# febrianrachmadi/dep-gan-im

Hardware: AMD Instinct MI355X
Metric: 2D slices/sec (G+2D+GP train step), 256x256x1 fp32 (higher is better)
Workload: dtype f32; 1 GPU; DEP-GAN-IM twoCritics canonical train step (critic-Y2 + critic-DEM + G update, WGAN-GP), batch 32 per GPU, 256x256x1; per_gpu_batch=32, global_batch=32, parallelism=dp1

## Files before the change

dep_gan_im_amd/csrc/common.h:

```cpp
#pragma once
#include <hip/hip_runtime.h>
#include <stdint.h>
#include <stddef.h>

typedef float f32x2 __attribute__((ext_vector_type(2)));
typedef float f32x4 __attribute__((ext_vector_type(4)));
typedef float f32x16 __attribute__((ext_vector_type(16)));

struct TView {
  float* p;
  long sB, sY, sX;
};

static inline TView make_view(float* p, int H, int W, int C) {
  TView v;
  v.p = p;
  v.sX = C;
  v.sY = (long)W * C;
  v.sB = (long)H * W * C;
  return v;
}
static inline TView make_view_slice(float* p, int H, int W, int Ctot, int c0) {
  TView v = make_view(p, H, W, Ctot);
  v.p = p + c0;
  return v;
}
static inline TView null_view() {
  TView v;
  v.p = nullptr;
  v.sB = v.sY = v.sX = 0;
  return v;
}

struct TViewH {
  __bf16* p;
  long sB, sY, sX;
};

static inline TViewH make_view_h(__bf16* p, int H, int W, int C) {
  TViewH v;
  v.p = p;
  v.sX = C;
  v.sY = (long)W * C;
  v.sB = (long)H * W * C;
  return v;
}
static inline TViewH make_view_slice_h(__bf16* p, int H, int W, int Ctot, int c0) {
  TViewH v = make_view_h(p, H, W, Ctot);
  v.p = p + c0;
  return v;
}
static inline TViewH null_view_h() {
  TViewH v;
  v.p = nullptr;
  v.sB = v.sY = v.sX = 0;
  return v;
}

struct Epilogue {
  const float* bias;
  const float* scale;
  const float* shift;
  const float* film_mul;
  const float* film_add;
  int film_ld;
  TView out_pre;
  TView res;
  TView mask;
  int relu;
  int accumulate;
  TView pool;
  const float* head_w;
  const float* head_b;
  float* head_out;
  int head_tanh, head_skip_out;
};

struct ConvArgs {
  TView in;
  TView out;
  const float* w;
  int B, H, W, Cin, Cout;
  Epilogue ep;
  long wsT, wsI, wsO;
  int flip;
  int vec4;
  unsigned long long* dbg;
  int groups;
  int lgx, lgy;
  const float* w_group[4];
  long out_group_off[4];
  int cpt;
  long in_run_off[4];
};

struct WgradArgs {
  TView x;
  TView dy;
  float* part;
  int B, H, W, Cin, Cout;
  int nTiles, tilesPerChunk;
  float* colpart;
  int colB;
};

#ifdef __HIPCC__
static __device__ __forceinline__ float dg_vmax(float a, float b) {
  float o;
  asm("v_max_f32 %0, %1, %2" : "=v"(o) : "v"(a), "v"(b));
  return o;
}
#endif

#define DG_OK 0
#define DG_ERR_ARG 1
#define DG_ERR_HIP 2
#define DG_ERR_UNSUPPORTED 3

void dg_set_error(const char* fmt, ...);

#define HIPCHECK(expr)                                                              \
  do {                                                                              \
    hipError_t _e = (expr);                                                         \
    if (_e != hipSuccess) {                                                         \
      dg_set_error("%s:%d: %s -> %s", __FILE__, __LINE__, #expr, hipGetErrorString(_e)); \
      return DG_ERR_HIP;                                                            \
    }                                                                               \
  } while (0)
// ... 51 lines not shown
  int planes;
  int ntaps() const { return family == CONV_WINO ? 16 : KS * KS; }
  int tapg() const { return KS == 5 ? 5 : KS * KS; }
};
static inline bool dg_plan_mfma(const ConvPlan& pl) { return pl.family != CONV_DIRECT; }
static inline bool dg_plan_bf16(const ConvPlan& pl) { return pl.family == CONV_BF16; }
static inline bool dg_plan_split(const ConvPlan& pl) { return pl.family == CONV_SPLIT; }
static inline bool dg_plan_wino(const ConvPlan& pl) { return pl.family == CONV_WINO; }
static inline bool dg_plan_tile3_ck8(const ConvPlan& pl) { return pl.family == CONV_TILE && pl.KS == 3 && pl.CK == 8; }
static inline bool dg_plan_tile5(const ConvPlan& pl) { return pl.family == CONV_TILE && pl.KS == 5; }
static inline ConvPlan dg_plan_direct() {
  ConvPlan p = {};
  p.family = CONV_DIRECT;
  return p;
}
ConvPlan dg_plan_conv(int KS, int Cin, int Cout);
ConvPlan dg_plan_conv_items(int KS, int Cin, int Cout, long items);
ConvPlan dg_plan_conv_bf16(int KS, int Cin, int Cout);
ConvPlan dg_plan_conv_bf16_n16(int KS, int Cin, int Cout);
const char* dg_conv_igemm_bf16_name(const ConvPlan& pl);
ConvPlan dg_plan_conv_split(int KS, int Cin, int Cout, int planes);
int dg_conv_igemm_bf16(const ConvPlan& pl, const ConvArgs& a, hipStream_t st);
static inline size_t dg_plan_elem_bytes(const ConvPlan& pl) { return pl.planes ? 2 * (size_t)pl.planes : 4; }

struct PackJob {
  const float* src;
  float* dst;
  const float* kscale;
  int ntaps, srcI, srcO, io, transpose, flip;
  int NT, CK, nCC, Kdim, Ndim;
  int bf16;
  int tapg;
  int wino;
  unsigned total;
  unsigned per_nt;
  unsigned nt_stride;
  unsigned blk0, nblk;
};
int dg_pack_job(const ConvPlan& pl, const float* src, int srcI, int srcO, int io, int transpose, int flip,
                const float* kscale, float* dst, size_t nt_stride, PackJob* job);
unsigned dg_pack_layout(PackJob* jobs_host, int njobs);
int dg_pack_weights_batch(const PackJob* jobs_dev, int njobs, unsigned nblocks, hipStream_t st);

int dg_pack_weights(const ConvPlan& pl, const float* src, int srcI, int srcO, int io, int transpose, int flip,
                    const float* kscale, float* dst, hipStream_t st);

int dg_conv_igemm(const ConvPlan& pl, const ConvArgs& a, hipStream_t st);
int dg_conv_igemm_check(const ConvPlan& pl, const ConvArgs& a);
bool dg_conv_igemm_wp_supported(const ConvPlan& pl, const ConvArgs& a, bool force);
int dg_conv_igemm_wp(const ConvPlan& pl, const ConvArgs& a, hipStream_t st);
bool dg_conv_igemm_ws5_supported(const ConvPlan& pl, const ConvArgs& a, bool force);
int dg_conv_igemm_ws5(const ConvPlan& pl, const ConvArgs& a, hipStream_t st);
const char* dg_conv_igemm_ws5_name(const ConvPlan& pl);
int dg_conv_igemm_tile(const ConvPlan& pl, const ConvArgs& a, hipStream_t st);
bool dg_conv_igemm_head_supported(const ConvPlan& pl, const ConvArgs& a);
ConvPlan dg_plan_conv_wino(int Cin, int Cout);
bool dg_conv_wino_supported(const ConvPlan& pl, const ConvArgs& a);
const char* dg_conv_wino_name(const ConvArgs& a);
int dg_conv_wino(const ConvPlan& pl, const ConvArgs& a, hipStream_t st);
enum { DG_EPF_BIAS = 1, DG_EPF_AFFINE = 2, DG_EPF_FILM = 4, DG_EPF_RELU = 8, DG_EPF_PRE = 16, DG_EPF_RES = 32,
       DG_EPF_MASK = 64, DG_EPF_POOL = 128, DG_EPF_ACCUM = 256, DG_EPF_HEAD = 512, DG_EPF_ALL = 1023 };
unsigned dg_epilogue_flags(const Epilogue& e);
int dg_wino_epi_class(unsigned flags, int form);
void dg_set_epi_classes(int on);
int dg_get_epi_classes();
void dg_conv_igemm_name(const ConvPlan& pl, const ConvArgs& a, char* buf, size_t cap);
int dg_conv_direct(int KS, const ConvArgs& a, hipStream_t st);

int dg_wgrad(int KS, const WgradArgs& a, int* nchunks, hipStream_t st);
int dg_wgrad_finish(const float* part, int nchunks, int ntaps, int Cin, int Cout, const float* scale, float* out,
                    float* raw, int accumulate, int oi, const float* colpart, int colC, const float* colscale,
                    float* colout, float* colraw, hipStream_t st);
int dg_wgrad_finish_rows(const float* part, int nchunks, int ntaps, int Cin, int Cout, const float* scale, float* out,
                         float* raw, int accumulate, int oi, const float* colpart, int colrows, int colC,
                         const float* colscale, float* colout, float* colraw, hipStream_t st);

bool dg_wgrad_bf16_supported(int KS, int Cin, int Cout);
int dg_wgrad_bf16(int KS, const WgradArgs& a, int* nchunks, hipStream_t st);

int dg_wgrad_small(int KS, const WgradArgs& a, int* nchunks, hipStream_t st);

int dg_wgrad_plan(int KS, int B, int H, int W, int Cin, int Cout, int out[4]);
int dg_wgrad_small_plan(int KS, int B, int H, int W, int Cin, int Cout, int out[4]);
int dg_wgrad_bf16_plan(int KS, int B, int H, int W, int Cin, int Cout, int out[4]);

enum DgWgradKernel { DG_WG_F32 = 0, DG_WG_EDGE = 1, DG_WG_BF16 = 2, DG_WG_BF16S = 3, DG_WG_DECONV = 4 };
struct DgWgradChoice {
  int kernel, nchunks;
  size_t part_floats;
  int col_rows;
};
int dg_wgrad_choose(int KS, int B, int H, int W, int Cin, int Cout, bool bf16_pipe, bool x_bf16, DgWgradChoice* out);
int dg_wgrad_plan_of(int kernel, int KS, int B, int H, int W, int Cin, int Cout, int out[4]);
```

dep_gan_im_amd/csrc/direct.hip:

```cpp
#include "common.h"
#include "epilogue.h"

template <int KS, int COG, int G>
__global__ __launch_bounds__(256) void conv_direct_kernel(const ConvArgs a) {
  constexpr int PAD = KS / 2;
  constexpr int TW = 16 + KS - 1;
  constexpr int PIXT = TW * TW;
  constexpr int NTAPS = KS * KS;
  constexpr int CT = COG * G;
  constexpr int CIK = 8;
  constexpr int PPP = 256 / G;
  constexpr int NPASS = G;

  extern __shared__ __attribute__((aligned(16))) float smem[];
  float* xs = smem;
  float* ws = smem + CIK * PIXT;

  const int tid = threadIdx.x;
  const int tilesX = (a.W + 15) >> 4, tilesY = (a.H + 15) >> 4;
  int t = blockIdx.x;
  const int tx0 = (t % tilesX) * 16;
  t /= tilesX;
  const int ty0 = (t % tilesY) * 16;
  const int b = t / tilesY;
// ... 221 lines not shown
    const int iy = ty0 + ly - PAD, ix = tx0 + lx - PAD;
    float v = 0.f;
    if (lx < TWX && iy >= 0 && iy < a.H && ix >= 0 && ix < a.W) v = inb[(long)iy * a.in.sY + (long)ix * a.in.sX + c];
    xs[q] = v;
  }
  for (int q = tid; q < a.Cin * KS * KS * CT; q += 256) {
    const int n = q % CT, tap = (q / CT) % (KS * KS), c = q / (CT * KS * KS);
    const int ts = a.flip ? (KS * KS - 1 - tap) : tap;
    ws[q] = (n < a.Cout) ? a.w[(long)ts * a.wsT + (long)c * a.wsI + (long)n * a.wsO] : 0.f;
  }
  __syncthreads();

  f32x4 acc[4];
#pragma unroll
  for (int j = 0; j < 4; ++j) acc[j] = f32x4{0.f, 0.f, 0.f, 0.f};
  for (int c = 0; c < a.Cin; ++c) {
#pragma unroll
    for (int ty = 0; ty < KS; ++ty) {
      const float* row = xs + (c * TWY + py + ty) * RS + qx;
      const f32x4 x0 = *reinterpret_cast<const f32x4*>(row);
      const f32x4 x1 = *reinterpret_cast<const f32x4*>(row + 4);
      const float xv[8] = {x0[0], x0[1], x0[2], x0[3], x1[0], x1[1], x1[2], x1[3]};
#pragma unroll
      for (int tx = 0; tx < KS; ++tx) {
        const f32x4 w4 = *reinterpret_cast<const f32x4*>(ws + ((c * KS + ty) * KS + tx) * CT + 4 * g);
#pragma unroll
        for (int j = 0; j < 4; ++j)
#pragma unroll
          for (int k = 0; k < 4; ++k) acc[j][k] = fmaf(xv[j + tx], w4[k], acc[j][k]);
      }
    }
  }
  const int co = 4 * g;
  if (co < a.Cout) {
#pragma unroll
    for (int j = 0; j < 4; ++j) {
      const int oy = ty0 + py, ox = tx0 + qx + j;
      if (oy < a.H && ox < a.W) epi_store4(a, b, oy, ox, co, acc[j]);
    }
  }
}

template <int KS, int G>
static int launch_cin12(const ConvArgs& a, hipStream_t st) {
  constexpr int ROWS = 256 / G / 4;
  dim3 grid((unsigned)(cdiv(a.W, 16) * cdiv(a.H, ROWS) * a.B));
  hipLaunchKernelGGL((conv_cin12_kernel<KS, G>), grid, dim3(256), 0, st, a);
  HIPCHECK(hipGetLastError());
  return DG_OK;
}

int dg_conv_direct(int KS, const ConvArgs& a_in, hipStream_t st) {
  ConvArgs a = a_in;
  if (a.ep.pool.p || a.ep.head_out || a.ep.head_skip_out || a.groups > 1 || a.cpt > 0) {
    dg_set_error("dg_conv_direct: no fused pool, fused head, grouped launch or gathered K on the direct kernels");
    return DG_ERR_UNSUPPORTED;
  }
  auto aligned = [](const TView& v) {
    return !v.p || (!(v.sX % 4) && !(v.sY % 4) && !(v.sB % 4) && !(((uintptr_t)v.p) & 15));
  };
  a.vec4 = (a.Cout % 4 == 0) && aligned(a.out) && aligned(a.ep.res) && aligned(a.ep.mask) && aligned(a.ep.out_pre) &&
           (!a.ep.film_mul || a.ep.film_ld % 4 == 0);
  const int sel = (a.Cout == 1) ? 0 : ((a.Cout <= 16) ? 1 : 2);
  if (a.Cin <= 2 && a.vec4 && (a.Cout == 16 || a.Cout == 32) && (KS == 3 || KS == 5)) {
    if (KS == 3) return (a.Cout == 16) ? launch_cin12<3, 4>(a, st) : launch_cin12<3, 8>(a, st);
    return (a.Cout == 16) ? launch_cin12<5, 4>(a, st) : launch_cin12<5, 8>(a, st);
  }
  if (KS == 3) {
    if (sel == 0) return (a.Cin >= 4) ? launch_cout1<3>(a, st) : launch_direct<3, 1, 1>(a, st);
    if (sel == 1) return launch_direct<3, 4, 4>(a, st);
    return launch_direct<3, 4, 8>(a, st);
  }
  if (KS == 5) {
    if (sel == 0) return (a.Cin >= 4) ? launch_cout1<5>(a, st) : launch_direct<5, 1, 1>(a, st);
    if (sel == 1) return launch_direct<5, 4, 4>(a, st);
    return launch_direct<5, 4, 8>(a, st);
  }
  if (KS == 1) {
    if (sel == 0) return launch_direct<1, 1, 1>(a, st);
    if (sel == 1) return launch_direct<1, 4, 4>(a, st);
    return launch_direct<1, 4, 8>(a, st);
  }
  dg_set_error("dg_conv_direct: unsupported kernel size %d", KS);
  return DG_ERR_UNSUPPORTED;
}

template <int KS>
__global__ __launch_bounds__(256) void wgrad_small_kernel(const WgradArgs a) {
  constexpr int PAD = KS / 2;
  constexpr int TW = 16 + KS - 1;
  constexpr int PIXT = TW * TW;
  constexpr int NTAPS = KS * KS;
  constexpr int NOUT = 4;
  extern __shared__ __attribute__((aligned(16))) float smem[];
  float* xs = smem;
  float* ds = smem + a.Cin * PIXT;
  const int tid = threadIdx.x;
  const int nout = NTAPS * a.Cin * a.Cout;
  const int tilesX = (a.W + 15) >> 4, tilesY = (a.H + 15) >> 4;
  const int t0 = blockIdx.x * a.tilesPerChunk, t1 = min(t0 + a.tilesPerChunk, a.nTiles);
  float acc[NOUT];
  int xoff[NOUT], co_[NOUT];
#pragma unroll
  for (int k = 0; k < NOUT; ++k) {
    acc[k] = 0.f;
    const int o = tid + k * 256;
    const int oo = (o < nout) ? o : 0;
    const int co = oo % a.Cout, ci = (oo / a.Cout) % a.Cin, tap = oo / (a.Cout * a.Cin);
// ... 197 lines not shown
```

dep_gan_im_amd/csrc/epilogue.h:

```cpp
#pragma once
#include "common.h"

struct EpiChan {
  float bias, scale, shift, fmul, fadd;
};

__device__ __forceinline__ EpiChan epi_load_chan(const Epilogue& e, int b, int co, int Cout) {
  EpiChan c;
  c.bias = e.bias ? e.bias[co] : 0.f;
  c.scale = e.scale ? e.scale[co] : 1.f;
  c.shift = e.shift ? e.shift[co] : 0.f;
  c.fmul = e.film_mul ? e.film_mul[(long)b * e.film_ld + co] : 1.f;
  c.fadd = e.film_add ? e.film_add[(long)b * e.film_ld + co] : 0.f;
  return c;
}

__device__ __forceinline__ long view_off(const TView& v, int b, int y, int x) {
  return (long)b * v.sB + (long)y * v.sY + (long)x * v.sX;
}

__device__ __forceinline__ float film_preact(float u, float fmul, float fadd) {
#pragma clang fp contract(off)
  const float p = u * fmul;
  return p + fadd;
}

__device__ __forceinline__ void epi_store(const ConvArgs& a, const EpiChan& c, int b, int oy, int ox, int co,
                                          float acc) {
  const Epilogue& e = a.ep;
  float v = acc + c.bias;
  if (e.scale) v = __fadd_rn(__fmul_rn(v, c.scale), c.shift);
  if (e.out_pre.p) e.out_pre.p[view_off(e.out_pre, b, oy, ox) + co] = v;
  if (e.film_mul) v = film_preact(v, c.fmul, c.fadd);
  if (e.relu) v = fmaxf(v, 0.f);
  if (e.res.p) v += e.res.p[view_off(e.res, b, oy, ox) + co];
  if (e.mask.p) v = (e.mask.p[view_off(e.mask, b, oy, ox) + co] > 0.f) ? v : 0.f;
  float* o = a.out.p + view_off(a.out, b, oy, ox) + co;
  if (e.accumulate) v += *o;
  *o = v;
}

__device__ __forceinline__ void epi_store4(const ConvArgs& a, int b, int oy, int ox, int co, f32x4 v) {
  const Epilogue& e = a.ep;
  if (e.bias) {
    const f32x4 t = *reinterpret_cast<const f32x4*>(e.bias + co);
#pragma unroll
    for (int k = 0; k < 4; ++k) v[k] += t[k];
  }
  if (e.scale) {
    const f32x4 sc = *reinterpret_cast<const f32x4*>(e.scale + co);
    const f32x4 sh = *reinterpret_cast<const f32x4*>(e.shift + co);
#pragma unroll
    for (int k = 0; k < 4; ++k) v[k] = __fadd_rn(__fmul_rn(v[k], sc[k]), sh[k]);
  }
  if (e.out_pre.p) *reinterpret_cast<f32x4*>(e.out_pre.p + view_off(e.out_pre, b, oy, ox) + co) = v;
  if (e.film_mul) {
    const f32x4 fm = *reinterpret_cast<const f32x4*>(e.film_mul + (long)b * e.film_ld + co);
    const f32x4 fa = *reinterpret_cast<const f32x4*>(e.film_add + (long)b * e.film_ld + co);
#pragma unroll
    for (int k = 0; k < 4; ++k) v[k] = film_preact(v[k], fm[k], fa[k]);
  }
  if (e.relu) {
#pragma unroll
    for (int k = 0; k < 4; ++k) v[k] = fmaxf(v[k], 0.f);
  }
  if (e.res.p) {
    const f32x4 r = *reinterpret_cast<const f32x4*>(e.res.p + view_off(e.res, b, oy, ox) + co);
#pragma unroll
    for (int k = 0; k < 4; ++k) v[k] += r[k];
  }
  if (e.mask.p) {
    const f32x4 m = *reinterpret_cast<const f32x4*>(e.mask.p + view_off(e.mask, b, oy, ox) + co);
// ... 12 lines not shown
```

dep_gan_im_amd/csrc/igemm_conv.hip:

```cpp
#include <stdlib.h>

#include "common.h"
#include "epilogue.h"

__device__ __forceinline__ void store_packed(float* dst, size_t i, float v, int bf16) {
  if (bf16) reinterpret_cast<__bf16*>(dst)[i] = (__bf16)v;
  else dst[i] = v;
}
__device__ __forceinline__ void store_split(float* dst, size_t nt_base, int cc, int tap, int n, int k, float v, int planes,
                                            int tapg, int ntaps, int NT, int CK) {
  const int ng = ntaps / tapg, tg = tap / tapg, tl = tap - tg * tapg;
  __bf16* d = reinterpret_cast<__bf16*>(dst) + nt_base + ((size_t)cc * ng + tg) * (size_t)(planes * tapg * NT * CK);
  float rem = v;
  for (int p = 0; p < planes; ++p) {
    const __bf16 hb = (__bf16)rem;
    d[((size_t)p * tapg + tl) * (NT * CK) + (size_t)n * CK + k] = hb;
    rem -= (float)hb;
  }
}

template <int MF>
struct Mfma;
template <>
struct Mfma<32> {
  typedef f32x16 acc_t;
  static constexpr int NREG = 16;
  static __device__ __forceinline__ acc_t run(float a, float b, acc_t c) {
    return __builtin_amdgcn_mfma_f32_32x32x2f32(a, b, c, 0, 0, 0);
  }
  static __device__ __forceinline__ int row(int j, int h) { return (j & 3) + 8 * (j >> 2) + 4 * h; }
};
template <>
struct Mfma<16> {
  typedef f32x4 acc_t;
  static constexpr int NREG = 4;
  static __device__ __forceinline__ acc_t run(float a, float b, acc_t c) {
    return __builtin_amdgcn_mfma_f32_16x16x4f32(a, b, c, 0, 0, 0);
  }
  static __device__ __forceinline__ int row(int j, int h) { return 4 * h + j; }
};

template <int MF, int KS, int CK, int TAPG, bool PERS, bool HEAD>
static __device__ __forceinline__ void igemm_conv_body(const ConvArgs& a) {
  constexpr int NT = MF;
  constexpr int PAD = KS / 2;
  constexpr int TW = 16 + KS - 1;
  constexpr int PIXT = TW * TW;
  constexpr int CKP = CK + 4;
  constexpr int NTAPS = KS * KS;
  constexpr int NG = NTAPS / TAPG;
  constexpr int KB = 256 / MF;
  constexpr int NSUB = CK / KB;
  constexpr int MT = 64 / MF;
  constexpr int XV = CK / 4;
  constexpr int XTOT = PIXT * XV;
  constexpr int XPIECES = (XTOT + 255) / 256;
  constexpr int WTOT = TAPG * NT * XV;
  constexpr int WPIECES = (WTOT + 255) / 256;
  static_assert(NTAPS % TAPG == 0 && (TAPG == NTAPS || TAPG == KS), "tap grouping");
  static_assert(CK % KB == 0, "chunk must hold whole fragment reads");
  typedef typename Mfma<MF>::acc_t acc_t;

  extern __shared__ __attribute__((aligned(16))) float smem[];
  float* xs = smem;
  float* ws = smem + PIXT * CKP;

  const int tid = threadIdx.x;
  unsigned long long* dbg = a.dbg ? a.dbg + (size_t)blockIdx.x * 16 : nullptr;
  if (dbg && tid == 0) {
    dbg[0] = __builtin_amdgcn_s_memtime();
    dbg[6] = __builtin_amdgcn_s_memrealtime();
    dbg[7] = __builtin_amdgcn_s_getreg((4 << 0) | (0 << 6) | (31 << 11));
  }
  const int tilesX = (a.W + 15) >> 4, tilesY = (a.H + 15) >> 4;
  const unsigned nNTall = (unsigned)a.lgy, nPix = (unsigned)a.lgx;
  constexpr int XFULL = XTOT / 256, WFULL = WTOT / 256;
  constexpr bool XPART = (XTOT % 256) != 0, WPART = (WTOT % 256) != 0;
  unsigned xgb[XPIECES], xlb[XPIECES], wlb[WPIECES];
  int xyx[XPIECES];
  if (PERS) {
#pragma unroll
    for (int i = 0; i < XPIECES; ++i) {
      const int q = min(tid + i * 256, XTOT - 1);
      const int pix = q / XV, part = q - pix * XV;
      const int ly = pix / TW, lx = pix - ly * TW;
      xgb[i] = 4u * (unsigned)(ly * (int)a.in.sY + lx * (int)a.in.sX + part * 4);
      xlb[i] = 4u * (unsigned)(pix * CKP + part * 4);
      xyx[i] = (ly << 16) | (lx << 8) | (part * 4);
    }
#pragma unroll
    for (int i = 0; i < WPIECES; ++i) {
      const int q = min(tid + i * 256, WTOT - 1);
      const int row = q / XV, part = q - row * XV;
      wlb[i] = 4u * (unsigned)(row * CKP + part * 4);
    }
// ... 150 lines not shown
    if (MF == 32) {
      py = 4 * wv + 2 * mt + (r >> 4);
      px = r & 15;
    } else {
      py = 4 * wv + mt;
      px = r;
    }
    apix[mt] = (py * TW + px) * CKP + 4 * h;
  }
  const int boff = r * CKP + 4 * h;

  acc_t acc[MT];
#pragma unroll
  for (int mt = 0; mt < MT; ++mt)
#pragma unroll
    for (int j = 0; j < Mfma<MF>::NREG; ++j) acc[mt][j] = 0.f;

  prefetch(0);
  if (dbg && tid == 0) dbg[1] = __builtin_amdgcn_s_memtime();
  for (int s = 0; s < NS; ++s) {
    __syncthreads();
    commit(s);
    __syncthreads();
    if (dbg && tid == 0 && s == 0) dbg[2] = __builtin_amdgcn_s_memtime();
    if (dbg && tid == 0 && s == 1) dbg[3] = __builtin_amdgcn_s_memtime();
    if (s + 1 < NS) prefetch(s + 1);
    const int tg = s % NG;
    constexpr int NSTEP = TAPG * NSUB;
    f32x4 av[2][MT], bv[2];
    auto load_frag = [&](int q, f32x4* a_, f32x4& b_) {
      const int tl = q / NSUB, sub = q - tl * NSUB;
      const int tap = (TAPG == NTAPS) ? tl : (tg * TAPG + tl);
      const int ty = tap / KS, tx = tap - ty * KS;
      const int tapoff = (ty * TW + tx) * CKP;
#pragma unroll
      for (int mt = 0; mt < MT; ++mt) a_[mt] = *reinterpret_cast<const f32x4*>(xs + apix[mt] + tapoff + sub * KB);
      b_ = *reinterpret_cast<const f32x4*>(ws + tl * (NT * CKP) + boff + sub * KB);
    };
    load_frag(0, av[0], bv[0]);
#pragma unroll
    for (int q = 0; q < NSTEP; ++q) {
      if (q + 1 < NSTEP) load_frag(q + 1, av[(q + 1) & 1], bv[(q + 1) & 1]);
      __builtin_amdgcn_sched_barrier(0);
#pragma unroll
      for (int j = 0; j < 4; ++j)
#pragma unroll
        for (int mt = 0; mt < MT; ++mt) acc[mt] = Mfma<MF>::run(bv[q & 1][j], av[q & 1][mt][j], acc[mt]);
      __builtin_amdgcn_sched_barrier(0);
    }
  }

  if (dbg && tid == 0) dbg[4] = __builtin_amdgcn_s_memtime();
#define EPI_HEAD HEAD
#include "igemm_epilogue.inc"
#undef EPI_HEAD
  if (dbg && tid == 0) {
    dbg[5] = __builtin_amdgcn_s_memtime();
    dbg[6] = __builtin_amdgcn_s_memrealtime() - dbg[6];
  }
  dbg = nullptr;
  } while (PERS && (id += gridDim.x) < nPix * nNTall);
}

template <int MF, int KS, int CK, int TAPG, bool PERS>
__global__ __launch_bounds__(256, (PERS && KS == 3) ? (CK == 8 ? 4 : 3) : 1) void igemm_conv_kernel(const ConvArgs a) {
  igemm_conv_body<MF, KS, CK, TAPG, PERS, false>(a);
}

template <bool PERS>
__global__ __launch_bounds__(256, PERS ? 4 : 1) void igemm_conv_head_kernel(const ConvArgs a) {
  igemm_conv_body<32, 3, 8, 9, PERS, true>(a);
}

ConvPlan dg_plan_conv(int KS, int Cin, int Cout) {
  ConvPlan p = dg_plan_direct();
  p.KS = KS;
  p.Cin = Cin;
  p.Cout = Cout;
  p.MF = (Cout % 32 == 0) ? 32 : 16;
  p.NT = p.MF;
  p.CK = 16;
  if (Cin < 8 || (Cin % 4) != 0 || Cout < 8) return p;
  if (KS != 1 && KS != 3 && KS != 5) return p;
  if (p.MF == 32 && KS == 5) p.CK = 8;
  if (p.MF == 32 && KS == 1) p.CK = 32;
  p.family = CONV_TILE;
  p.nNT = cdiv(Cout, p.NT);
  p.nCC = cdiv(Cin, p.CK);
  p.packedFloats = (size_t)p.nNT * p.nCC * KS * KS * p.NT * p.CK;
  return p;
}

ConvPlan dg_plan_conv_items(int KS, int Cin, int Cout, long items) {
  ConvPlan p = dg_plan_conv(KS, Cin, Cout);
  const char* e = getenv("DEPGAN_IGEMM_CK8");
  const bool on = !(e && atoi(e) == 0);
  if (on && p.family == CONV_TILE && KS == 3 && p.MF == 32 && (Cin % 8) == 0 && items >= 1536) {
    p.CK = 8;
    p.nCC = cdiv(Cin, p.CK);
    p.packedFloats = (size_t)p.nNT * p.nCC * KS * KS * p.NT * p.CK;
  }
  return p;
}

ConvPlan dg_plan_conv_wino(int Cin, int Cout) {
  ConvPlan p = dg_plan_conv(3, Cin, Cout);
  if (p.family != CONV_TILE || (Cin % 8) != 0 || (Cout % 32) != 0) { p.family = CONV_DIRECT; return p; }
  p.family = CONV_WINO;
  p.CK = 8;
  p.nCC = Cin / 8;
  p.packedFloats = (size_t)p.nNT * p.nCC * 16 * p.NT * p.CK;
  return p;
}

static long igemm_grid(int KS, int CK, size_t lds, long total) {
  const char* e = getenv("DEPGAN_IGEMM_PERSIST");
  int per_cu = (int)((160 * 1024) / lds);
  if (per_cu > (KS == 3 ? (CK == 8 ? 4 : 3) : 2)) per_cu = (KS == 3 ? (CK == 8 ? 4 : 3) : 2);
  if (KS == 1) per_cu = 0;
  if (e) per_cu = atoi(e) < per_cu ? atoi(e) : per_cu;
  const long cap = 256L * per_cu;
  return (per_cu > 0 && total > cap) ? cap : total;
}

template <int MF, int KS, int CK, int TAPG>
static int launch_tile(const ConvArgs& a, hipStream_t st, char* name_out = nullptr, size_t name_cap = 0) {
  constexpr int TW = 16 + KS - 1;
  constexpr size_t lds_k = (size_t)(TW * TW * (CK + 4) + TAPG * MF * (CK + 4)) * sizeof(float);
  constexpr size_t lds_e = (size_t)4 * 64 * (MF + 4) * sizeof(float);
  constexpr size_t lds = lds_k > lds_e ? lds_k : lds_e;
  ConvArgs b = a;
  b.lgx = cdiv(a.W, 16) * cdiv(a.H, 16) * a.B;
  b.lgy = cdiv(a.Cout, MF) * (a.groups > 1 ? a.groups : 1);
  const long total = (long)b.lgx * b.lgy;
  const long G = igemm_grid(KS, CK, lds, total);
  constexpr bool CAN_HEAD = (MF == 32 && KS == 3 && CK == 8 && TAPG == 9);
  const bool head = a.ep.head_out != nullptr;
  if (head && (!CAN_HEAD || a.Cout != 32 || a.groups > 1 || a.ep.pool.p != nullptr)) {
    dg_set_error("dg_conv_igemm: the fused head needs the 8-channel-chunk 3x3 kernel and 32 output channels");
    return DG_ERR_ARG;
  }
  if (name_out) {
    if (head) snprintf(name_out, name_cap, "igemm_conv_head_kernel<%s>", G < total ? "true" : "false");
    else snprintf(name_out, name_cap, "igemm_conv_kernel<%d,%d,%d,%d,%s>", MF, KS, CK, TAPG, G < total ? "true" : "false");
    return DG_OK;
  }
  if constexpr (CAN_HEAD) {
    if (head) {
      static DgOncePerDevice once_h;
      if (once_h.need()) {
        HIPCHECK(hipFuncSetAttribute(reinterpret_cast<const void*>(&igemm_conv_head_kernel<false>),
                                     hipFuncAttributeMaxDynamicSharedMemorySize, (int)lds));
        HIPCHECK(hipFuncSetAttribute(reinterpret_cast<const void*>(&igemm_conv_head_kernel<true>),
                                     hipFuncAttributeMaxDynamicSharedMemorySize, (int)lds));
      }
      if (G < total) hipLaunchKernelGGL((igemm_conv_head_kernel<true>), dim3((unsigned)G), dim3(256), lds, st, b);
      else hipLaunchKernelGGL((igemm_conv_head_kernel<false>), dim3((unsigned)G), dim3(256), lds, st, b);
      HIPCHECK(hipGetLastError());
      return DG_OK;
    }
  }
  static DgOncePerDevice once;
  if (once.need()) {
    HIPCHECK(hipFuncSetAttribute(reinterpret_cast<const void*>(&igemm_conv_kernel<MF, KS, CK, TAPG, false>),
                                 hipFuncAttributeMaxDynamicSharedMemorySize, (int)lds));
    HIPCHECK(hipFuncSetAttribute(reinterpret_cast<const void*>(&igemm_conv_kernel<MF, KS, CK, TAPG, true>),
                                 hipFuncAttributeMaxDynamicSharedMemorySize, (int)lds));
  }
  if (G < total)
    hipLaunchKernelGGL((igemm_conv_kernel<MF, KS, CK, TAPG, true>), dim3((unsigned)G), dim3(256), lds, st, b);
  else
    hipLaunchKernelGGL((igemm_conv_kernel<MF, KS, CK, TAPG, false>), dim3((unsigned)G), dim3(256), lds, st, b);
  HIPCHECK(hipGetLastError());
  return DG_OK;
}

static int dispatch_tile(const ConvPlan& pl, const ConvArgs& a, hipStream_t st, char* name_out, size_t name_cap) {
  const bool wide = pl.MF == 32;
  if (pl.family == CONV_TILE && pl.KS == 3 && !dg_plan_tile3_ck8(pl))
    return wide ? launch_tile<32, 3, 16, 9>(a, st, name_out, name_cap) : launch_tile<16, 3, 16, 9>(a, st, name_out, name_cap);
  if (pl.family == CONV_TILE && pl.KS == 5)
    return wide ? launch_tile<32, 5, 8, 25>(a, st, name_out, name_cap) : launch_tile<16, 5, 16, 25>(a, st, name_out, name_cap);
  if (pl.family == CONV_TILE && pl.KS == 1)
    return wide ? launch_tile<32, 1, 32, 1>(a, st, name_out, name_cap) : launch_tile<16, 1, 16, 1>(a, st, name_out, name_cap);
  if (dg_plan_tile3_ck8(pl)) return launch_tile<32, 3, 8, 9>(a, st, name_out, name_cap);
  dg_set_error("dg_conv_igemm: no tile kernel for family %d MF=%d KS=%d CK=%d", (int)pl.family, pl.MF, pl.KS, pl.CK);
  return DG_ERR_ARG;
}

bool dg_conv_igemm_head_supported(const ConvPlan& pl, const ConvArgs& a) {
  return (dg_plan_tile3_ck8(pl) || dg_plan_wino(pl)) && a.Cout == 32 && a.groups <= 1 && a.ep.pool.p == nullptr && a.cpt <= 0 &&
         !a.ep.accumulate;
}

void dg_conv_igemm_name(const ConvPlan& pl, const ConvArgs& a, char* buf, size_t cap) {
  if (cap) buf[0] = 0;
  if (!dg_plan_mfma(pl)) { snprintf(buf, cap, "conv_direct"); return; }
  if (dg_plan_split(pl)) { snprintf(buf, cap, "igemm_split_kernel"); return; }
  if (dg_plan_bf16(pl)) { snprintf(buf, cap, "%s", dg_conv_igemm_bf16_name(pl)); return; }
  if (dg_plan_wino(pl)) { snprintf(buf, cap, "%s", dg_conv_wino_name(a)); return; }
  if (dg_conv_igemm_wp_supported(pl, a, false)) { snprintf(buf, cap, "igemm_wp_kernel<0>"); return; }
  if (dg_conv_igemm_ws5_supported(pl, a, false)) { snprintf(buf, cap, "%s", dg_conv_igemm_ws5_name(pl)); return; }
  dispatch_tile(pl, a, nullptr, buf, cap);
}

int dg_conv_igemm_check(const ConvPlan& pl, const ConvArgs& a) {
  if (!dg_plan_mfma(pl)) {
    dg_set_error("dg_conv_igemm: no MFMA variant for KS=%d Cin=%d Cout=%d", pl.KS, pl.Cin, pl.Cout);
    return DG_ERR_UNSUPPORTED;
  }
  auto misaligned = [](const TView& v) {
    return v.p && ((v.sX % 4) || (v.sY % 4) || (v.sB % 4) || (((uintptr_t)v.p) & 15));
  };
  if (misaligned(a.in) || misaligned(a.out) || misaligned(a.ep.res) || misaligned(a.ep.mask) ||
      misaligned(a.ep.out_pre) || (a.Cout % 4) || (a.ep.film_mul && (a.ep.film_ld % 4))) {
    dg_set_error("dg_conv_igemm: views must be 16-byte aligned (pointers, strides and Cout multiples of 4 floats)");
    return DG_ERR_ARG;
  }
  if (a.ep.pool.p && ((a.H | a.W) & 1 || misaligned(a.ep.pool) || a.groups > 1)) {
    dg_set_error("dg_conv_igemm: fused max-pool needs even H, W and a 16-byte aligned pooled view");
    return DG_ERR_ARG;
  }
  if (a.cpt > 0) {
    const int run = a.cpt * pl.CK;
    bool bad = a.groups > 1 || (a.Cin % run) != 0 || a.Cin / run > 4;
    for (int r = 0; !bad && r < a.Cin / run; ++r) bad = (a.in_run_off[r] % 4) != 0;
    if (bad) {
      dg_set_error("dg_conv_igemm: gathered K needs Cin = runs (<= 4) x cpt x %d channels and 16-byte run offsets", pl.CK);
      return DG_ERR_ARG;
    }
  }
  if (a.ep.head_out && !dg_conv_igemm_head_supported(pl, a)) {
    dg_set_error("dg_conv_igemm: the fused head needs the fp32 8-channel-chunk 3x3 kernel, 32 output channels, no pool");
    return DG_ERR_ARG;
  }
  return DG_OK;
}

static int conv_igemm_impl(const ConvPlan& pl, const ConvArgs& a_in, hipStream_t st, bool allow_wp) {
  ConvArgs a = a_in;
  DGCHECK(dg_conv_igemm_check(pl, a));
  if (dg_plan_bf16(pl) || dg_plan_split(pl)) return dg_conv_igemm_bf16(pl, a, st);
  if (dg_plan_wino(pl)) return dg_conv_wino(pl, a, st);
  if (allow_wp && dg_conv_igemm_wp_supported(pl, a, false)) return dg_conv_igemm_wp(pl, a, st);
  if (allow_wp && dg_conv_igemm_ws5_supported(pl, a, false)) return dg_conv_igemm_ws5(pl, a, st);
  return dispatch_tile(pl, a, st, nullptr, 0);
}

int dg_conv_igemm(const ConvPlan& pl, const ConvArgs& a, hipStream_t st) { return conv_igemm_impl(pl, a, st, true); }
int dg_conv_igemm_tile(const ConvPlan& pl, const ConvArgs& a, hipStream_t st) { return conv_igemm_impl(pl, a, st, false); }

__global__ __launch_bounds__(256) void pack_weights_batch_kernel(const PackJob* __restrict__ jobs, int njobs) {
  int lo = 0, hi = njobs - 1;
  while (lo < hi) {
    const int mid = (lo + hi + 1) >> 1;
    if (jobs[mid].blk0 <= blockIdx.x) lo = mid; else hi = mid - 1;
  }
  const PackJob J = jobs[lo];
  const unsigned b = blockIdx.x - J.blk0;
  if (J.wino) {
    const unsigned cols = J.total / 16u, plane = (unsigned)(J.NT * J.CK);
    for (unsigned i = b * 256u + threadIdx.x; i < cols; i += J.nblk * 256u) {
      unsigned q = i;
      const int k = (int)(q % J.CK);
      q /= J.CK;
      const int n = (int)(q % J.NT);
      q /= J.NT;
      const int cc = (int)(q % J.nCC);
      const int nt = (int)(q / J.nCC);
      const int kk = cc * J.CK + k, nn = nt * J.NT + n;
      double g[3][3];
#pragma unroll
      for (int t = 0; t < 9; ++t) g[t / 3][t % 3] = 0.0;
      if (kk < J.Kdim && nn < J.Ndim) {
        const int ci = J.transpose ? nn : kk;
        const int co = J.transpose ? kk : nn;
        const float* e0 = J.src + (J.io ? ((size_t)co * J.srcI + ci) : ((size_t)ci * J.srcO + co));
        const size_t ts_stride = (size_t)J.srcI * J.srcO;
        const float ks = J.kscale ? J.kscale[kk] : 1.f;
#pragma unroll
        for (int t = 0; t < 9; ++t) {
          float v = e0[(size_t)(J.flip ? 8 - t : t) * ts_stride];
// ... 110 lines not shown
```

dep_gan_im_amd/csrc/igemm_epilogue.inc:

```
#ifndef EPI_PRE_SYNC
#define EPI_PRE_SYNC __syncthreads()
#define EPI_PRE_SYNC_DEFAULTED
#endif
  EPI_PRE_SYNC;
  constexpr int CP = NT + 4;
#ifdef EPI_ES_BASE
  float* es = EPI_ES_BASE;
#else
  float* es = smem + wv * (64 * CP);
#endif
  constexpr int NQ = (MF == 32) ? 4 : 1, CSTEP = (MF == 32) ? 8 : 4;
#if defined(EPI_STAGE)
  EPI_STAGE;
  (void)es;
#elif !defined(EPI_PHASED)
#pragma unroll
  for (int mt = 0; mt < MT; ++mt)
#pragma unroll
    for (int g = 0; g < NQ; ++g) {
      f32x4 q4;
#pragma unroll
      for (int k = 0; k < 4; ++k) q4[k] = acc[mt][4 * g + k];
      *reinterpret_cast<f32x4*>(es + (MF * mt + r) * CP + CSTEP * g + 4 * h) = q4;
    }
#endif
  constexpr int LPP = NT / 4;
  constexpr int PPP = 64 / LPP;
#ifdef EPI_NPASS
  constexpr int NPASS = EPI_NPASS;
#else
  constexpr int NPASS = 64 / PPP;
#endif
  const int c4 = (lane % LPP) * 4, pl0 = lane / LPP;
  const int co = n0 + c4;
#ifndef EPI_OYW
  const int wvu = __builtin_amdgcn_readfirstlane(wv);
#endif
  const Epilogue& e = a.ep;
#ifdef EPI_CLASS
  typedef EPI_CLASS EpiC;
  constexpr bool EPI_CT = EpiC::fixed;
  const bool affine = EPI_CT ? EpiC::affine : (e.scale != nullptr), film = EPI_CT ? EpiC::film : (e.film_mul != nullptr),
             relu = EPI_CT ? EpiC::relu : (e.relu != 0), accum = EPI_CT ? false : (e.accumulate != 0);
  const bool has_bias = EPI_CT ? EpiC::bias : (e.bias != nullptr), has_pre = EPI_CT ? EpiC::pre : (e.out_pre.p != nullptr),
             has_res = EPI_CT ? EpiC::res : (e.res.p != nullptr), has_msk = EPI_CT ? EpiC::msk : (e.mask.p != nullptr),
             has_pool = EPI_CT ? EpiC::pool : (e.pool.p != nullptr);
#else
  const bool affine = e.scale != nullptr, film = e.film_mul != nullptr, relu = e.relu != 0, accum = e.accumulate != 0;
  const bool has_bias = e.bias != nullptr, has_pre = e.out_pre.p != nullptr, has_res = e.res.p != nullptr,
             has_msk = e.mask.p != nullptr, has_pool = e.pool.p != nullptr;
#endif
#ifdef EPI_OYW
  const int oyw = EPI_OYW;
#else
  const int oyw = ty0 + 4 * wvu;
#endif
#ifdef EPI_HEAD
  float hkeep_out = 0.f;
#endif
#ifdef EPI_FULL
  const bool full = EPI_FULL;
#else
  const bool full = (ty0 + 16 <= a.H) && (tx0 + 16 <= a.W);
#endif
  if (co < a.Cout) {
    f32x4 bias4 = {0.f, 0.f, 0.f, 0.f}, sc4 = {1.f, 1.f, 1.f, 1.f}, sh4 = {0.f, 0.f, 0.f, 0.f};
    f32x4 fm4 = {1.f, 1.f, 1.f, 1.f}, fa4 = {0.f, 0.f, 0.f, 0.f};
    if (has_bias) bias4 = *reinterpret_cast<const f32x4*>(e.bias + co);
    if (affine) {
      sc4 = *reinterpret_cast<const f32x4*>(e.scale + co);
      sh4 = *reinterpret_cast<const f32x4*>(e.shift + co);
    }
#pragma unroll
    for (int k = 0; k < 4; ++k) sh4[k] = fmaf(bias4[k], sc4[k], sh4[k]);
    if (film) {
      fm4 = *reinterpret_cast<const f32x4*>(e.film_mul + (long)b * e.film_ld + co);
      fa4 = *reinterpret_cast<const f32x4*>(e.film_add + (long)b * e.film_ld + co);
    }
    auto mk = [&](const float* p) {
      const unsigned long long u = (unsigned long long)p;
      const unsigned lo = __builtin_amdgcn_readfirstlane((unsigned)u), hi = __builtin_amdgcn_readfirstlane((unsigned)(u >> 32));
      return __builtin_amdgcn_make_buffer_rsrc((void*)(((unsigned long long)hi << 32) | lo), 0, 0x7FFFFFFF, 0x00020000);
    };
    const int lo_out = 4 * (pl0 * (int)a.out.sX + co);
    const int lo_pre = has_pre ? 4 * (pl0 * (int)e.out_pre.sX + co) : 0;
    const int lo_res = has_res ? 4 * (pl0 * (int)e.res.sX + co) : 0;
    const int lo_msk = has_msk ? 4 * (pl0 * (int)e.mask.sX + co) : 0;
    const __amdgpu_buffer_rsrc_t r_out = mk(a.out.p + out_goff + view_off(a.out, b, oyw, tx0));
    const __amdgpu_buffer_rsrc_t r_pre = mk(has_pre ? e.out_pre.p + view_off(e.out_pre, b, oyw, tx0) : a.out.p);
    const __amdgpu_buffer_rsrc_t r_res = mk(has_res ? e.res.p + view_off(e.res, b, oyw, tx0) : a.out.p);
    const __amdgpu_buffer_rsrc_t r_msk = mk(has_msk ? e.mask.p + view_off(e.mask, b, oyw, tx0) : a.out.p);
    const __amdgpu_buffer_rsrc_t r_pool =
        mk(has_pool ? e.pool.p + view_off(e.pool, b, oyw >> 1, tx0 >> 1) : a.out.p);
    const int lo_pool = has_pool ? 4 * ((pl0 >> 1) * (int)e.pool.sX + co) : 0;
    const int sY_pool = 4 * (int)e.pool.sY, sX_pool = 4 * (int)e.pool.sX;
    f32x4 vrow = {0.f, 0.f, 0.f, 0.f};
#ifdef EPI_HEAD
#ifdef EPI_CLASS
    const bool has_head = EPI_HEAD && (EPI_CT ? EpiC::head : (e.head_out != nullptr));
#else
    const bool has_head = EPI_HEAD && e.head_out != nullptr;
#endif
    f32x4 hw4 = {0.f, 0.f, 0.f, 0.f};
    if (has_head) hw4 = *reinterpret_cast<const f32x4*>(e.head_w + co);
    const bool skip_out = has_head && e.head_skip_out != 0;
#else
    constexpr bool has_head = false, skip_out = false;
#endif
    typedef int i32x4 __attribute__((ext_vector_type(4)));
    auto ld = [&](const __amdgpu_buffer_rsrc_t& r, int voff, int soff) {
      const i32x4 t = __builtin_amdgcn_raw_buffer_load_b128(r, voff, soff, 0);
      return __builtin_bit_cast(f32x4, t);
    };
    auto st = [&](const __amdgpu_buffer_rsrc_t& r, int voff, int soff, f32x4 v) {
      __builtin_amdgcn_raw_buffer_store_b128(__builtin_bit_cast(i32x4, v), r, voff, soff, 0);
    };
    const int sY_out = 4 * (int)a.out.sY, sX_out = 4 * (int)a.out.sX;
    const int sY_pre = 4 * (int)e.out_pre.sY, sX_pre = 4 * (int)e.out_pre.sX;
    const int sY_res = 4 * (int)e.res.sY, sX_res = 4 * (int)e.res.sX;
    const int sY_msk = 4 * (int)e.mask.sY, sX_msk = 4 * (int)e.mask.sX;
#ifdef EPI_STAGE_LATE
    EPI_STAGE_LATE;
#endif
#pragma unroll
    for (int p = 0; p < NPASS; ++p) {
      constexpr int RP = 16 / PPP;
      const int py = (p & 1) + 2 * (p / (2 * RP)), px0 = ((p >> 1) % RP) * PPP;
      const bool ok = full || (oyw + py < a.H && tx0 + px0 + pl0 < a.W);
#if defined(EPI_FETCH)
      f32x4 v;
      EPI_FETCH(v, py, (px0 + pl0));
#elif defined(EPI_PHASED)
      static_assert(MF == 32, "phased epilogue: 32-pixel tiles");
      if (p % (NPASS / MT) == 0) {
        const int mtp = p / (NPASS / MT);
#pragma unroll
        for (int g = 0; g < NQ; ++g) {
          f32x4 q4;
#pragma unroll
          for (int k = 0; k < 4; ++k) q4[k] = acc[mtp][4 * g + k];
          *reinterpret_cast<f32x4*>(es + r * CP + CSTEP * g + 4 * h) = q4;
        }
      }
      f32x4 v = *reinterpret_cast<const f32x4*>(es + ((py & 1) * 16 + px0 + pl0) * CP + c4);
#else
      f32x4 v = *reinterpret_cast<const f32x4*>(es + (py * 16 + px0 + pl0) * CP + c4);
#endif
#pragma unroll
      for (int k = 0; k < 4; ++k) v[k] = fmaf(v[k], sc4[k], sh4[k]);
      if (has_pre) {
        if (ok) st(r_pre, lo_pre, py * sY_pre + px0 * sX_pre, v);
      }
      if (film) {
#pragma unroll
        for (int k = 0; k < 4; ++k) v[k] = film_preact(v[k], fm4[k], fa4[k]);
      }
      if (relu) {
#pragma unroll
        for (int k = 0; k < 4; ++k) v[k] = dg_vmax(v[k], 0.f);
      }
      if (has_res) {
        f32x4 rr = {0.f, 0.f, 0.f, 0.f};
        if (ok) rr = ld(r_res, lo_res, py * sY_res + px0 * sX_res);
#pragma unroll
        for (int k = 0; k < 4; ++k) v[k] += rr[k];
      }
      if (has_msk) {
        f32x4 mm = {1.f, 1.f, 1.f, 1.f};
        if (ok) mm = ld(r_msk, lo_msk, py * sY_msk + px0 * sX_msk);
#pragma unroll
        for (int k = 0; k < 4; ++k) v[k] = (mm[k] > 0.f) ? v[k] : 0.f;
      }
      const int so = py * sY_out + px0 * sX_out;
      if (accum) {
        f32x4 old = {0.f, 0.f, 0.f, 0.f};
        if (ok) old = ld(r_out, lo_out, so);
#pragma unroll
        for (int k = 0; k < 4; ++k) v[k] += old[k];
      }
      if (ok && !skip_out) st(r_out, lo_out, so, v);
#ifdef EPI_HEAD
      if (has_head) {
        static_assert(!EPI_HEAD || (NT == 32 && NPASS == 8), "fused head: 32-channel tiles, eight passes");
        float d = v[0] * hw4[0];
        d = fmaf(v[1], hw4[1], d);
        d = fmaf(v[2], hw4[2], d);
        d = fmaf(v[3], hw4[3], d);
#define EPI_DPP(x, ctrl) \
  __builtin_bit_cast(float, __builtin_amdgcn_update_dpp(0, __builtin_bit_cast(int, (x)), (ctrl), 0xF, 0xF, false))
        d += EPI_DPP(d, 0xB1);
        d += EPI_DPP(d, 0x4E);
        d += EPI_DPP(d, 0x141);
#undef EPI_DPP
        hkeep_out = ((lane & 7) == p) ? d : hkeep_out;
      }
#endif
      if (has_pool) {
        if ((py & 1) == 0) {
          vrow = v;
        } else {
          f32x4 m;
#pragma unroll
          for (int k = 0; k < 4; ++k) {
            const float t = dg_vmax(vrow[k], v[k]);
            m[k] = dg_vmax(t, __shfl_xor(t, LPP, 64));
          }
          if (ok && (pl0 & 1) == 0) st(r_pool, lo_pool, (py >> 1) * sY_pool + (px0 >> 1) * sX_pool, m);
        }
      }
    }
  }
#ifdef EPI_HEAD
  if (EPI_HEAD && a.ep.head_out != nullptr && n0 < a.Cout) {
    const int ph = lane & 7, plh = lane >> 3;
    const int pyh = (ph & 1) + 2 * (ph >> 2), pxh = ((ph >> 1) & 1) * 8 + plh;
    const int yh = oyw + pyh, xh = tx0 + pxh;
    if (yh < a.H && xh < a.W) {
      const float t = hkeep_out + a.ep.head_b[0];
      a.ep.head_out[((long)b * a.H + yh) * a.W + xh] = a.ep.head_tanh ? tanhf(t) : t;
    }
  }
#endif
#ifdef EPI_PRE_SYNC_DEFAULTED
#undef EPI_PRE_SYNC
#undef EPI_PRE_SYNC_DEFAULTED
#endif
```

dep_gan_im_amd/csrc/igemm_wino.hip:

```cpp
#include <stdlib.h>

#include <type_traits>

#include "common.h"
#include "epilogue.h"

namespace {

constexpr int WN_CK = 8;
constexpr int WN_TW = 18;
constexpr int WN_CP = 36;
constexpr int WN_XV = WN_CK / 4;

template <int MT>
struct WnCfg {
  static constexpr int TH = 8 * MT;
  static constexpr int NTILE = 32 * MT;
  static constexpr int PIXT = (TH + 2) * WN_TW;
  static constexpr int XTOT = PIXT * WN_XV;
  static constexpr int NXP = (XTOT + 255) / 256;
  static constexpr int RAW = NXP * 256 * 4;
  static_assert(XTOT % 4 == 0 && WN_TW % 2 == 0, "rslot permutes inside aligned groups of four slots: halo and padding stay apart");
  static constexpr int ZPLANE = NTILE * WN_CP + 32;
  static constexpr int Z = 8 * ZPLANE;
  static constexpr int NBUF = 2;
  static_assert(NBUF >= 2 && NBUF * RAW <= Z, "the raw ring must fit under the Z exchange: LDS and workgroups per CU unchanged");
  static_assert((NBUF - 1) * NXP + 4 < 64, "counted waits: vmcnt is a 6-bit field");
  static constexpr size_t LDS = sizeof(float) * (size_t)Z;
  static constexpr int WGS_PER_CU = (MT == 2) ? 2 : 3;
};

template <int N>
static __device__ __forceinline__ void wn_wait_vm() {
  asm volatile("s_waitcnt vmcnt(%0)" ::"n"(N) : "memory");
}
template <int S>
using WnSlot = std::integral_constant<int, S>;

static __device__ __forceinline__ int rslot(int pix, int half) { return (2 * pix + half) ^ (((pix % WN_TW) >> 2) & 3); }
static __device__ __forceinline__ int rslot_inv(int q) { return q ^ ((((q >> 1) % WN_TW) >> 2) & 3); }

constexpr unsigned WN_BAR = DG_EPF_BIAS | DG_EPF_AFFINE | DG_EPF_RELU;
constexpr unsigned WN_FILM = WN_BAR | DG_EPF_FILM | DG_EPF_RES;
constexpr int WN_NCLASS = 11, WN_HEAD_CLASS = 10;
constexpr unsigned kWnClassMask[WN_NCLASS] = {
    0,
    WN_BAR,
    WN_BAR | DG_EPF_POOL,
    WN_FILM,
    WN_FILM | DG_EPF_PRE,
    DG_EPF_RES | DG_EPF_MASK,
    DG_EPF_MASK,
    0,
    DG_EPF_BIAS | DG_EPF_RELU,
    DG_EPF_BIAS | DG_EPF_RELU | DG_EPF_POOL,
    WN_BAR | DG_EPF_HEAD,
};
#define WN_CLASSES8(X) X(1) X(2) X(3) X(4) X(5) X(6) X(7) X(8) X(9)
template <int EC>
struct WnEpi {
  static_assert(EC >= 0 && EC < WN_NCLASS, "epilogue class");
  static constexpr unsigned M = kWnClassMask[EC];
  static constexpr bool fixed = EC != 0;
  static constexpr bool bias = M & DG_EPF_BIAS, affine = M & DG_EPF_AFFINE, film = M & DG_EPF_FILM, relu = M & DG_EPF_RELU,
                        pre = M & DG_EPF_PRE, res = M & DG_EPF_RES, msk = M & DG_EPF_MASK, pool = M & DG_EPF_POOL,
                        head = M & DG_EPF_HEAD;
};

template <int MT, bool PERS, bool HEAD, bool GATH = false, int ABL = 0, int EC = 0>
static __device__ __forceinline__ void wino_body(const ConvArgs& a) {
  typedef WnCfg<MT> C;
  constexpr int MF = 32, NT = 32;
  constexpr int WN_RAW = C::RAW, WN_ZPLANE = C::ZPLANE, WN_XTOT = C::XTOT, NXP = C::NXP, NBUF = C::NBUF;
  constexpr int NXI = (ABL & 8) ? 0 : NXP;
  typedef f32x16 acc_t;
  extern __shared__ __attribute__((aligned(16))) float smem[];

  const int tid = threadIdx.x;
  const int lane = tid & 63, wv = tid >> 6;
  const int r = lane & 31, h = lane >> 5;
  const int tilesX = (a.W + 15) >> 4, tilesY = (a.H + C::TH - 1) / C::TH;
  const unsigned nNTall = (unsigned)a.lgy, nPix = (unsigned)a.lgx;
  const int nCC = a.Cin / WN_CK;

  constexpr int SENT = (int)0x80000000;
  int xvo[NXP], xyx[NXP];
#pragma unroll
  for (int i = 0; i < NXP; ++i) {
    const int q = tid + i * 256;
    const int lq = rslot_inv(q);
    const int pix = lq >> 1, part = lq & 1;
    const int ly = pix / WN_TW, lx = pix - ly * WN_TW;
    xvo[i] = (q < WN_XTOT) ? 4 * (ly * (int)a.in.sY + lx * (int)a.in.sX + part * 4) : SENT;
    xyx[i] = (ly << 8) | lx;
  }
  int tA[MT][4], tB[MT][4];
  float tS[MT];
#pragma unroll
  for (int i = 0; i < MT; ++i) {
    const int cg = h, aa = wv, T = 32 * i + r;
    const int tyi = T >> 3, txi = T & 7;
    const int rA = (aa == 0) ? 0 : (aa == 2 ? 2 : 1), rB = (aa == 3) ? 3 : (aa == 2 ? 1 : 2);
#pragma unroll
    for (int j = 0; j < 4; ++j) {
      tA[i][j] = 16 * rslot((2 * tyi + rA) * WN_TW + 2 * txi + j, cg);
      tB[i][j] = 16 * rslot((2 * tyi + rB) * WN_TW + 2 * txi + j, cg);
    }
    tS[i] = (aa == 1) ? 1.f : -1.f;
  }
  const int wbase = __builtin_amdgcn_readfirstlane(wv * 256);
  const int wvo = 4 * ((4 * wv * 32 + r) * WN_CK + 4 * h);

  unsigned id = blockIdx.x;
  do {
    int t, ntile;
    if ((nPix & 7u) == 0) {
      const unsigned x = id & 7u, sl = id >> 3;
      ntile = (int)(sl % nNTall);
      t = (int)(x * (nPix >> 3) + sl / nNTall);
// ... 166 lines not shown
        chunk(no, rt, last);
      }
    }

    if (ABL & 1) {
      float sacc = 0.f;
#pragma unroll
      for (int f = 0; f < 4; ++f)
#pragma unroll
        for (int mt = 0; mt < MT; ++mt)
#pragma unroll
          for (int j = 0; j < 16; ++j) sacc += acc[f][mt][j];
      if (sacc == 12345.678f) a.out.p[tid] = sacc;
      __syncthreads();
      continue;
    }
    auto zstage = [&]() {
      __syncthreads();
      float* zw = smem + (2 * wv) * WN_ZPLANE + r * WN_CP + 4 * h;
#pragma unroll
      for (int mt = 0; mt < MT; ++mt)
#pragma unroll
        for (int g = 0; g < 4; ++g) {
          f32x4 z0, z1;
#pragma unroll
          for (int k = 0; k < 4; ++k) {
            const float m0 = acc[0][mt][4 * g + k], m1 = acc[1][mt][4 * g + k], m2 = acc[2][mt][4 * g + k],
                        m3 = acc[3][mt][4 * g + k];
            z0[k] = (m0 + m1) + m2;
            z1[k] = (m1 - m2) - m3;
          }
          *reinterpret_cast<f32x4*>(zw + mt * (32 * WN_CP) + 8 * g) = z0;
          *reinterpret_cast<f32x4*>(zw + WN_ZPLANE + mt * (32 * WN_CP) + 8 * g) = z1;
        }
      __syncthreads();
    };
#define EPI_PRE_SYNC
#define EPI_STAGE
#define EPI_STAGE_LATE zstage()
#define EPI_NPASS (4 * MT)
#define EPI_OYW (ty0 + 2 * MT * __builtin_amdgcn_readfirstlane(wv))
#define EPI_FULL ((ty0 + C::TH <= a.H) && (tx0 + 16 <= a.W))
#define EPI_FETCH(v, py, px)                                                                                         \
  {                                                                                                                  \
    const float* zb = smem + ((px)&1) * WN_ZPLANE +                                                                  \
                      ((MT * __builtin_amdgcn_readfirstlane(wv) + ((py) >> 1)) * 8 + ((px) >> 1)) * WN_CP + c4;       \
    const f32x4 za = *reinterpret_cast<const f32x4*>(zb + (((py)&1) ? 2 : 0) * WN_ZPLANE);                           \
    const f32x4 zb1 = *reinterpret_cast<const f32x4*>(zb + (((py)&1) ? 4 : 2) * WN_ZPLANE);                          \
    const f32x4 zc = *reinterpret_cast<const f32x4*>(zb + (((py)&1) ? 6 : 4) * WN_ZPLANE);                           \
    _Pragma("unroll") for (int k_ = 0; k_ < 4; ++k_) v[k_] = ((py)&1) ? (za[k_] - zb1[k_]) - zc[k_] : (za[k_] + zb1[k_]) + zc[k_]; \
  }
#define EPI_HEAD HEAD
#define EPI_CLASS WnEpi<EC>
#include "igemm_epilogue.inc"
#undef EPI_CLASS
#undef EPI_HEAD
#undef EPI_FETCH
#undef EPI_FULL
#undef EPI_OYW
#undef EPI_NPASS
#undef EPI_STAGE_LATE
#undef EPI_STAGE
#undef EPI_PRE_SYNC
    if (PERS) __syncthreads();
  } while (PERS && (id += gridDim.x) < nPix * nNTall);
}

template <int MT, bool PERS, int EC>
__global__ __launch_bounds__(256, WnCfg<MT>::WGS_PER_CU) void wino_conv_kernel(const ConvArgs a) {
  wino_body<MT, PERS, false, false, 0, EC>(a);
}
template <bool PERS, int EC>
__global__ __launch_bounds__(256, 2) void wino_conv_head_kernel(const ConvArgs a) {
  wino_body<2, PERS, true, false, 0, EC>(a);
}
template <int MT, bool PERS>
__global__ __launch_bounds__(256, WnCfg<MT>::WGS_PER_CU) void wino_conv_gathered_kernel(const ConvArgs a) {
  wino_body<MT, PERS, false, true>(a);
}
#ifdef DEPGAN_WINO_ABLATIONS
template <int MT, int ABL>
__global__ __launch_bounds__(256, WnCfg<MT>::WGS_PER_CU) void wino_conv_abl_kernel(const ConvArgs a) {
  wino_body<MT, true, false, false, ABL>(a);
}
#endif

struct WnKern {
  const void* fn;
  const char* name;
};
#define WN_K8(EC)                                                                                       \
  {{reinterpret_cast<const void*>(&wino_conv_kernel<1, false, EC>), "wino_conv_kernel<1,false," #EC ">"}, \
   {reinterpret_cast<const void*>(&wino_conv_kernel<1, true, EC>), "wino_conv_kernel<1,true," #EC ">"}},
const WnKern kWn8[WN_HEAD_CLASS][2] = {WN_K8(0) WN_CLASSES8(WN_K8)};
#undef WN_K8
const WnKern kWn16[2] = {{reinterpret_cast<const void*>(&wino_conv_kernel<2, false, 0>), "wino_conv_kernel<2,false,0>"},
                         {reinterpret_cast<const void*>(&wino_conv_kernel<2, true, 0>), "wino_conv_kernel<2,true,0>"}};
const WnKern kWnHead[2][2] = {
    {{reinterpret_cast<const void*>(&wino_conv_head_kernel<false, 0>), "wino_conv_head_kernel<false,0>"},
     {reinterpret_cast<const void*>(&wino_conv_head_kernel<true, 0>), "wino_conv_head_kernel<true,0>"}},
    {{reinterpret_cast<const void*>(&wino_conv_head_kernel<false, WN_HEAD_CLASS>), "wino_conv_head_kernel<false,10>"},
     {reinterpret_cast<const void*>(&wino_conv_head_kernel<true, WN_HEAD_CLASS>), "wino_conv_head_kernel<true,10>"}}};
static_assert(WN_HEAD_CLASS == 10, "the names above");
const WnKern kWnGath[2][2] = {
    {{reinterpret_cast<const void*>(&wino_conv_gathered_kernel<1, false>), "wino_conv_gathered_kernel<1,false>"},
     {reinterpret_cast<const void*>(&wino_conv_gathered_kernel<1, true>), "wino_conv_gathered_kernel<1,true>"}},
    {{reinterpret_cast<const void*>(&wino_conv_gathered_kernel<2, false>), "wino_conv_gathered_kernel<2,false>"},
     {reinterpret_cast<const void*>(&wino_conv_gathered_kernel<2, true>), "wino_conv_gathered_kernel<2,true>"}}};

int g_epi_classes = -1;

}

void dg_set_epi_classes(int on) { g_epi_classes = on ? 1 : 0; }
int dg_get_epi_classes() {
  if (g_epi_classes < 0) {
    const char* e = getenv("DEPGAN_EPI_CLASSES");
    g_epi_classes = (e && atoi(e) == 0) ? 0 : 1;
  }
  return g_epi_classes;
}

unsigned dg_epilogue_flags(const Epilogue& e) {
  return (e.bias ? DG_EPF_BIAS : 0u) | (e.scale ? DG_EPF_AFFINE : 0u) | (e.film_mul ? DG_EPF_FILM : 0u) |
         (e.relu ? DG_EPF_RELU : 0u) | (e.out_pre.p ? DG_EPF_PRE : 0u) | (e.res.p ? DG_EPF_RES : 0u) |
         (e.mask.p ? DG_EPF_MASK : 0u) | (e.pool.p ? DG_EPF_POOL : 0u) | (e.accumulate ? DG_EPF_ACCUM : 0u) |
         (e.head_out ? DG_EPF_HEAD : 0u);
}

int dg_wino_epi_class(unsigned flags, int form) {
  if (!dg_get_epi_classes()) return 0;
  if (form == 1) return flags == kWnClassMask[WN_HEAD_CLASS] ? WN_HEAD_CLASS : 0;
  if (form != 0) return 0;
  for (int i = 1; i < WN_HEAD_CLASS; ++i)
    if (kWnClassMask[i] == flags) return i;
  return 0;
}

bool dg_conv_wino_supported(const ConvPlan& pl, const ConvArgs& a) {
  if (!dg_plan_wino(pl)) return false;
  if (a.Cin != pl.Cin || (a.Cin % WN_CK) || (a.Cout % 32) || a.groups > 1 || a.dbg || ((a.H | a.W) & 1)) return false;
  if (a.cpt > 0 && ((a.Cin % (a.cpt * WN_CK)) != 0 || a.Cin / (a.cpt * WN_CK) > 4)) return false;
  long run = 0;
  for (int t = 0; a.cpt > 0 && t < a.Cin / (a.cpt * WN_CK); ++t) {
    if (a.in_run_off[t] < 0) return false;
    run = a.in_run_off[t] > run ? a.in_run_off[t] : run;
  }
  constexpr long lim = 1L << 29;
  if (a.in.sY < 0 || a.in.sX < 0 || a.in.sY >= lim || a.in.sX >= lim || run >= lim) return false;
  if ((WnCfg<2>::TH + 2) * a.in.sY + WN_TW * a.in.sX + a.Cin + run >= lim) return false;
  return true;
}

static int wino_mt(const ConvArgs& a) {
  static int forced = -1;
  if (forced < 0) {
    const char* e = getenv("DEPGAN_WINO_MT");
    forced = e ? atoi(e) : 0;
  }
  if (a.ep.head_out) return 2;
  if (forced == 1 || forced == 2) return forced;
  return 1;
}

template <int MT>
static void wino_geometry(ConvArgs& a, long* total, long* G, bool* pers) {
  a.lgx = cdiv(a.W, 16) * cdiv(a.H, WnCfg<MT>::TH) * a.B;
  a.lgy = a.Cout / 32;
  *total = (long)a.lgx * a.lgy;
  const long cap = (long)WnCfg<MT>::WGS_PER_CU * dg_cu_count();
  *pers = *total > cap;
  *G = *pers ? cap : *total;
}

static const WnKern* wino_pick(const ConvArgs& a, int mt, bool pers) {
  const int form = a.ep.head_out ? 1 : (a.cpt > 0 ? 3 : (mt == 2 ? 2 : 0));
  const int ec = dg_wino_epi_class(dg_epilogue_flags(a.ep), form);
  if (form == 1) return &kWnHead[ec ? 1 : 0][pers];
  if (form == 3) return &kWnGath[mt - 1][pers];
  if (form == 2) return &kWn16[pers];
  return &kWn8[ec][pers];
}

const char* dg_conv_wino_name(const ConvArgs& a_in) {
  ConvArgs a = a_in;
  long total, G;
  bool pers;
  const int mt = wino_mt(a);
  if (mt == 2) wino_geometry<2>(a, &total, &G, &pers); else wino_geometry<1>(a, &total, &G, &pers);
  return wino_pick(a, mt, pers)->name;
}

template <int MT>
static int wino_launch(ConvArgs a, hipStream_t st) {
  long total, G;
  bool pers;
  wino_geometry<MT>(a, &total, &G, &pers);
  constexpr size_t LDS = WnCfg<MT>::LDS;
  static DgOncePerDevice once;
  if (once.need()) {
    const WnKern* const own = (MT == 2) ? &kWn16[0] : &kWn8[0][0];
    const int nown = (MT == 2) ? 2 : 2 * WN_HEAD_CLASS;
    for (int i = 0; i < nown; ++i)
      HIPCHECK(hipFuncSetAttribute(own[i].fn, hipFuncAttributeMaxDynamicSharedMemorySize, (int)LDS));
    for (int i = 0; i < 2; ++i)
      HIPCHECK(hipFuncSetAttribute(kWnGath[MT - 1][i].fn, hipFuncAttributeMaxDynamicSharedMemorySize, (int)LDS));
    for (int i = 0; MT == 2 && i < 4; ++i)
      HIPCHECK(hipFuncSetAttribute(kWnHead[i >> 1][i & 1].fn, hipFuncAttributeMaxDynamicSharedMemorySize, (int)LDS));
  }
#ifdef DEPGAN_WINO_ABLATIONS
  if (const char* e = getenv("DEPGAN_WINO_ABL")) {
    const int abl = atoi(e);
    if (abl && pers && !a.ep.head_out && a.cpt <= 0) {
#define WN_ABL_CASE(N)                                                                                              \
  case N:                                                                                                           \
    HIPCHECK(hipFuncSetAttribute(reinterpret_cast<const void*>(&wino_conv_abl_kernel<MT, N>),                       \
                                 hipFuncAttributeMaxDynamicSharedMemorySize, (int)LDS));                            \
    hipLaunchKernelGGL((wino_conv_abl_kernel<MT, N>), dim3((unsigned)G), dim3(256), LDS, st, a);                    \
    break;
      switch (abl) {
        WN_ABL_CASE(1) WN_ABL_CASE(2) WN_ABL_CASE(3) WN_ABL_CASE(4) WN_ABL_CASE(8) WN_ABL_CASE(10) WN_ABL_CASE(11)
        default: dg_set_error("DEPGAN_WINO_ABL=%d not instantiated", abl); return DG_ERR_ARG;
      }
      HIPCHECK(hipGetLastError());
      return DG_OK;
    }
  }
#endif
  if (a.ep.head_out) {
    if (MT != 2 || a.Cout != 32 || a.ep.pool.p || a.cpt > 0) {
      dg_set_error("dg_conv_wino: the fused head needs 32 output channels, no fused pool and no gathered K");
      return DG_ERR_ARG;
    }
  }
  void* kargs[] = {&a};
  HIPCHECK(hipLaunchKernel(wino_pick(a, MT, pers)->fn, dim3((unsigned)G), dim3(256), kargs, LDS, st));
  HIPCHECK(hipGetLastError());
  return DG_OK;
}

int dg_conv_wino(const ConvPlan& pl, const ConvArgs& a, hipStream_t st) {
  if (!dg_conv_wino_supported(pl, a)) {
    dg_set_error("dg_conv_wino: shape not covered (3x3, Cin %% 8, Cout %% 32, even H and W, no groups, a halo tile of the input view within 2 GiB)");
    return DG_ERR_UNSUPPORTED;
  }
  return wino_mt(a) == 2 ? wino_launch<2>(a, st) : wino_launch<1>(a, st);
}
```

dep_gan_im_amd/csrc/igemm_wp.hip:

```cpp
#include <stdlib.h>

#include "common.h"
#include "epilogue.h"

namespace {

constexpr int WP_NW = 16;

template <int MF, int KS, int CK>
struct WpGeo {
  static constexpr int NT = MF, MT = 64 / MF, PAD = KS / 2, NTAPS = KS * KS;
  static constexpr int TWX = 16 + KS - 1, TWY = 4 + KS - 1;
  static constexpr int PIX = TWX * TWY;
  static constexpr int XV = CK / 4;
  static constexpr int CKP = (KS == 3) ? CK + 4 : CK;
  static constexpr int EPI_FLOATS = (MF == 32 ? 32 : 64) * (NT + 4);
  static constexpr int WAVE_FLOATS = PIX * CKP > EPI_FLOATS ? PIX * CKP : EPI_FLOATS;
  static constexpr int SLOTS = PIX * XV;
  static constexpr int PIECES = (SLOTS + 63) / 64;
  static __device__ __forceinline__ int panel_sw(int n) {
    if (MF == 32) return (n >> (KS == 3 ? 2 : 4)) & 1;
    return (0x78 >> (2 * (n >> 2))) & 3;
  }
  static __device__ __forceinline__ int halo_off(int pix, int part) {
    if (CK == 16) return pix * CKP + 4 * (part ^ (((pix >> 2) & 1) << 1));
    return pix * CKP + 4 * part;
  }
};

template <int MF> struct WpMfma;
template <> struct WpMfma<32> {
  typedef f32x16 acc_t;
  static constexpr int NREG = 16;
  static __device__ __forceinline__ acc_t run(float w, float x, acc_t c) { return __builtin_amdgcn_mfma_f32_32x32x2f32(w, x, c, 0, 0, 0); }
};
template <> struct WpMfma<16> {
  typedef f32x4 acc_t;
  static constexpr int NREG = 4;
  static __device__ __forceinline__ acc_t run(float w, float x, acc_t c) { return __builtin_amdgcn_mfma_f32_16x16x4f32(w, x, c, 0, 0, 0); }
};

template <int MF, int KS, int CK, int ABL>
static __device__ __forceinline__ void igemm_wp_body(const ConvArgs& a) {
  typedef WpGeo<MF, KS, CK> G;
  constexpr int NT = G::NT, MT = G::MT, TW = G::TWX, PAD = G::PAD, NTAPS = G::NTAPS, CKP = G::CKP;
  constexpr int PIECES = G::PIECES, SLOTS = G::SLOTS, XV = G::XV;
  typedef typename WpMfma<MF>::acc_t acc_t;
  extern __shared__ __attribute__((aligned(16))) float smem[];
  const int tid = threadIdx.x;
  const int lane = tid & 63, wv = tid >> 6;
  const int NW = (int)(blockDim.x >> 6);
  const int r = lane % MF, h = lane / MF;
  const int nCC = a.Cin / CK;
  const int panelFloats = nCC * NTAPS * NT * CK;
  float* panel = smem;
  float* wbuf = smem + panelFloats + wv * G::WAVE_FLOATS;

  const unsigned nNT = (unsigned)a.lgy, nSup = (unsigned)a.lgx;
  const int bxN = (a.W + 15) >> 4, bandsY = (a.H + 15) >> 4;
  const int nItems = a.B * bandsY * bxN * 4;
  unsigned id = blockIdx.x;
  auto decode = [&](unsigned i, int& st, int& nt) {
    if ((nSup & 7u) == 0) {
      const unsigned x = i & 7u, sl = i >> 3;
      nt = (int)(sl % nNT);
      st = (int)(x * (nSup >> 3) + sl / nNT);
    } else {
      st = (int)(i % nSup);
      nt = (int)(i / nSup);
    }
  };
  int st0, ntile;
  decode(id, st0, ntile);

  {
    const float* src = a.w + (size_t)ntile * panelFloats;
    const int nq = panelFloats / 4;
    for (int q = tid; q < nq; q += (int)blockDim.x) {
      const int row = q / XV, part = q % XV;
      const f32x4 v = *reinterpret_cast<const f32x4*>(src + (size_t)q * 4);
      *reinterpret_cast<f32x4*>(panel + row * CK + 4 * (part ^ G::panel_sw(row % NT))) = v;
    }
  }
  __syncthreads();

  unsigned xgb[PIECES];
  constexpr int PSTEP = 64 / XV;
  static_assert(PSTEP % 8 == 0, "the halo swizzle must repeat from piece to piece");
  const int xpart = lane % XV, xpix0 = lane / XV;
#pragma unroll
  for (int i = 0; i < PIECES; ++i) {
    const int pix = min(xpix0 + PSTEP * i, G::PIX - 1);
    const int ly = pix / TW, lx = pix - ly * TW;
    xgb[i] = 4u * (unsigned)(ly * (int)a.in.sY + lx * (int)a.in.sX + xpart * 4);
  }
// ... 64 lines not shown
        for (int i = 0; i < PIECES - 1; ++i)
          *reinterpret_cast<__attribute__((address_space(3))) f32x4*>((size_t)(wb0 + xlb0 + 4u * PSTEP * CKP * i)) = xr[i];
        if (in_last)
          *reinterpret_cast<__attribute__((address_space(3))) f32x4*>((size_t)(wb0 + xlb0 + 4u * PSTEP * CKP * (PIECES - 1))) =
              xr[PIECES - 1];
      };

      acc_t acc[MT];
#pragma unroll
      for (int mt = 0; mt < MT; ++mt)
#pragma unroll
        for (int j = 0; j < WpMfma<MF>::NREG; ++j) acc[mt][j] = 0.f;

      prefetch(0);
      commit();
      for (int cc = 0; cc < nCC; ++cc) {
        if (!(ABL & 2) && cc + 1 < nCC) prefetch(cc + 1);
        const float* wp = panel + (size_t)cc * (NTAPS * NT * CK) + boff;
        f32x4 av[2][MT], bv[2];
        auto load_frag = [&](int tap, f32x4* a_, f32x4& b_) {
          const int ty = tap / KS, tx = tap - ty * KS;
#pragma unroll
          for (int mt = 0; mt < MT; ++mt) {
            if (CK == 16) a_[mt] = *reinterpret_cast<const f32x4*>(wbuf + asw[tx][(mt + ty) & 1] + (mt + ty) * TW * CKP);
            else a_[mt] = *reinterpret_cast<const f32x4*>(wbuf + apix[mt] + (ty * TW + tx) * CKP);
          }
          b_ = *reinterpret_cast<const f32x4*>(wp + tap * (NT * CK));
        };
        load_frag(0, av[0], bv[0]);
#pragma unroll
        for (int q = 0; q < NTAPS; ++q) {
          if (q + 1 < NTAPS) load_frag(q + 1, av[(q + 1) & 1], bv[(q + 1) & 1]);
          __builtin_amdgcn_sched_barrier(0);
#pragma unroll
          for (int j = 0; j < 4; ++j)
#pragma unroll
            for (int mt = 0; mt < MT; ++mt) {
              if (ABL & 4) acc[mt][j] += bv[q & 1][j] * av[q & 1][mt][j];
              else acc[mt] = WpMfma<MF>::run(bv[q & 1][j], av[q & 1][mt][j], acc[mt]);
            }
          __builtin_amdgcn_sched_barrier(0);
        }
        if (!(ABL & 2) && cc + 1 < nCC) commit();
      }

      const long out_goff = 0;
      if (ABL & 1) {
        if (acc[0][0] + acc[1][0] == 123.456f) a.out.p[0] = 1.f;
      } else {
#define EPI_PRE_SYNC ((void)0)
#define EPI_ES_BASE wbuf
#define EPI_OYW ty0
#define EPI_FULL ((ty0 + 4 <= a.H) && (tx0 + 16 <= a.W))
        if constexpr (MF == 32) {
#define EPI_PHASED
#include "igemm_epilogue.inc"
#undef EPI_PHASED
        } else {
#include "igemm_epilogue.inc"
        }
#undef EPI_PRE_SYNC
#undef EPI_ES_BASE
#undef EPI_OYW
#undef EPI_FULL
      }
    }
    id += gridDim.x;
    if (id >= nSup * nNT) break;
  }
}

template <int ABL>
__global__ __launch_bounds__(WP_NW * 64, 1) void igemm_wp_kernel(const ConvArgs a) {
  igemm_wp_body<32, 3, 8, ABL>(a);
}

constexpr int ws5_nwmax(int MF) { return MF == 32 ? 16 : 12; }
template <int MF, int CK>
__global__ __launch_bounds__(ws5_nwmax(MF) * 64, 1) void igemm_ws5_kernel(const ConvArgs a) {
  igemm_wp_body<MF, 5, CK, 0>(a);
}

}

typedef WpGeo<32, 3, 8> Wp3;
static long wp_groups(const ConvArgs& a, int nw) { return cdiv((long)a.B * cdiv(a.H, 16) * cdiv(a.W, 16) * 4, nw); }

bool dg_conv_igemm_wp_supported(const ConvPlan& pl, const ConvArgs& a, bool force) {
  if (!dg_plan_tile3_ck8(pl)) return false;
  if (a.Cin != pl.Cin || (a.Cin % 8) || a.Cin > 64 || (a.Cout % 32) || a.groups > 1 || a.cpt > 0 || a.dbg) return false;
  if (a.ep.head_out) return false;
  const size_t lds = ((size_t)a.Cin * 9 * 32 + (size_t)WP_NW * Wp3::WAVE_FLOATS) * sizeof(float);
  if (lds > 160 * 1024) return false;
  if (force) return true;
  static int on = -1;
  if (on < 0) {
    const char* e = getenv("DEPGAN_IGEMM_WP");
    on = (e && atoi(e) != 0) ? 1 : 0;
  }
  if (!on) return false;
  const long sup = wp_groups(a, WP_NW);
  return (sup & 7) == 0 && sup * (a.Cout / 32) >= 256;
}

int dg_conv_igemm_wp(const ConvPlan& pl, const ConvArgs& a_in, hipStream_t st) {
  ConvArgs a = a_in;
  DGCHECK(dg_conv_igemm_check(pl, a));
  const size_t lds = ((size_t)a.Cin * 9 * 32 + (size_t)WP_NW * Wp3::WAVE_FLOATS) * sizeof(float);
  static DgOncePerDevice once;
  if (once.need())
    HIPCHECK(hipFuncSetAttribute(reinterpret_cast<const void*>(&igemm_wp_kernel<0>),
                                 hipFuncAttributeMaxDynamicSharedMemorySize, 160 * 1024));
  const int nNT = a.Cout / 32;
  a.lgx = (int)wp_groups(a, WP_NW);
  a.lgy = nNT;
  const long total = (long)a.lgx * nNT;
  long G = dg_cu_count();
  G -= G % (8L * nNT);
  if (G < 8L * nNT) G = 8L * nNT;
  if (G > total || (a.lgx & 7) != 0) G = total;
#ifdef DEPGAN_WP_ABLATIONS
  static int abl = -1;
  if (abl < 0) {
    const char* e = getenv("DEPGAN_WP_ABL");
    abl = e ? atoi(e) : 0;
  }
  if (abl) {
    static DgOncePerDevice once2;
    if (once2.need()) {
      HIPCHECK(hipFuncSetAttribute(reinterpret_cast<const void*>(&igemm_wp_kernel<1>), hipFuncAttributeMaxDynamicSharedMemorySize, 160 * 1024));
      HIPCHECK(hipFuncSetAttribute(reinterpret_cast<const void*>(&igemm_wp_kernel<2>), hipFuncAttributeMaxDynamicSharedMemorySize, 160 * 1024));
      HIPCHECK(hipFuncSetAttribute(reinterpret_cast<const void*>(&igemm_wp_kernel<3>), hipFuncAttributeMaxDynamicSharedMemorySize, 160 * 1024));
      HIPCHECK(hipFuncSetAttribute(reinterpret_cast<const void*>(&igemm_wp_kernel<4>), hipFuncAttributeMaxDynamicSharedMemorySize, 160 * 1024));
    }
    switch (abl) {
      case 1: hipLaunchKernelGGL((igemm_wp_kernel<1>), dim3((unsigned)G), dim3(WP_NW * 64), lds, st, a); break;
      case 2: hipLaunchKernelGGL((igemm_wp_kernel<2>), dim3((unsigned)G), dim3(WP_NW * 64), lds, st, a); break;
      case 3: hipLaunchKernelGGL((igemm_wp_kernel<3>), dim3((unsigned)G), dim3(WP_NW * 64), lds, st, a); break;
      default: hipLaunchKernelGGL((igemm_wp_kernel<4>), dim3((unsigned)G), dim3(WP_NW * 64), lds, st, a); break;
    }
    HIPCHECK(hipGetLastError());
    return DG_OK;
  }
#endif
  hipLaunchKernelGGL((igemm_wp_kernel<0>), dim3((unsigned)G), dim3(WP_NW * 64), lds, st, a);
  HIPCHECK(hipGetLastError());
  return DG_OK;
}

template <int MF, int CK>
static int ws5_waves(int Cin) {
  const long panel = (long)Cin * 25 * MF, wave = WpGeo<MF, 5, CK>::WAVE_FLOATS;
  long nw = (160L * 1024 / 4 - panel) / wave;
  static int cap = -1;
  if (cap < 0) {
    const char* e = getenv("DEPGAN_IGEMM_WS5_WAVES");
    cap = (e && atoi(e) >= 4) ? atoi(e) : 16;
  }
  if (nw > cap) nw = cap;
  return (int)(nw < ws5_nwmax(MF) ? nw : ws5_nwmax(MF));
}
static int ws5_waves_of(const ConvPlan& pl, int Cin) { return pl.MF == 32 ? ws5_waves<32, 8>(Cin) : ws5_waves<16, 16>(Cin); }

bool dg_conv_igemm_ws5_supported(const ConvPlan& pl, const ConvArgs& a, bool force) {
  if (!dg_plan_tile5(pl)) return false;
  if (pl.CK != (pl.MF == 32 ? 8 : 16)) return false;
  if (a.Cin != pl.Cin || a.Cout != pl.Cout || a.Cout != pl.MF || (a.Cin != 16 && a.Cin != 32)) return false;
  if (a.groups > 1 || a.cpt > 0 || a.dbg || a.ep.head_out) return false;
  if (force) return true;
  static int mode = -2;
  if (mode == -2) {
    const char* e = getenv("DEPGAN_IGEMM_WS5");
    mode = e ? (atoi(e) != 0 ? 1 : 0) : -1;
  }
  if (mode == 0) return false;
  const long items = (long)a.B * cdiv(a.H, 4) * cdiv(a.W, 16);
  const long slots = (long)dg_cu_count() * ws5_waves_of(pl, a.Cin);
  if (items < 2 * slots) return false;
  if (mode == 1) return true;
  if (a.Cin == 32 && a.Cout == 16) return false;
  if (a.Cin == 32 && a.Cout == 32) return items >= 4 * slots;
  return true;
}

const char* dg_conv_igemm_ws5_name(const ConvPlan& pl) { return pl.MF == 32 ? "igemm_ws5_kernel<32,8>" : "igemm_ws5_kernel<16,16>"; }

template <int MF, int CK>
static int ws5_launch(ConvArgs& a, hipStream_t st) {
  const int nw = ws5_waves<MF, CK>(a.Cin);
  const size_t lds = ((size_t)a.Cin * 25 * MF + (size_t)nw * WpGeo<MF, 5, CK>::WAVE_FLOATS) * sizeof(float);
  static DgOncePerDevice once;
  if (once.need())
    HIPCHECK(hipFuncSetAttribute(reinterpret_cast<const void*>(&igemm_ws5_kernel<MF, CK>),
                                 hipFuncAttributeMaxDynamicSharedMemorySize, 160 * 1024));
  a.lgx = (int)wp_groups(a, nw);
  a.lgy = 1;
  long G = dg_cu_count();
  if ((a.lgx & 7) == 0) G -= G % 8;
  if (G > a.lgx || G < 1) G = a.lgx;
  hipLaunchKernelGGL((igemm_ws5_kernel<MF, CK>), dim3((unsigned)G), dim3(nw * 64), lds, st, a);
  HIPCHECK(hipGetLastError());
  return DG_OK;
}

int dg_conv_igemm_ws5(const ConvPlan& pl, const ConvArgs& a_in, hipStream_t st) {
  ConvArgs a = a_in;
  DGCHECK(dg_conv_igemm_check(pl, a));
  return pl.MF == 32 ? ws5_launch<32, 8>(a, st) : ws5_launch<16, 16>(a, st);
}
```

dep_gan_im_amd/csrc/model.h:

```cpp
#pragma once
#include <string.h>

#include <map>
#include <string>
#include <type_traits>
#include <vector>

#include "../../include/depgan.h"
#include "common.h"
#include "bf16s.h"
#include "bf16s_train.h"
#include "deconv_fwd.h"
#include "noise.h"
#include "ops.h"
#include "train_ops.h"

struct PInfo {
  std::string name;
  int shape[4];
  int ndim;
  size_t off, size;
  bool trainable;
};

// ... 83 lines not shown
  double flops;
  double bytes;
  char label[56];
  char kernel[48];
};

struct depgan_ctx {
  depgan_config cfg;
  hipStream_t st = nullptr;
  std::vector<void*> allocs;

  Net g;
  std::vector<GLayer> gl;
  NoiseParams np;
  NoiseGrads ng;
  NoiseActs na;
  float* derived = nullptr;
  PackJob* g_pack_jobs = nullptr;
  int g_n_pack = 0;
  unsigned g_pack_blocks = 0;
  BnJob* g_bn_jobs = nullptr;
  int g_n_bn = 0;
  float* raw_all = nullptr;
  GammaJob* g_gamma_jobs = nullptr;
  int g_n_gamma = 0, g_gamma_blocks = 0;
  float* heads_mean = nullptr;
  float* dheads = nullptr;
  Tn attr;
  Tn du_tmp;
  float* dpre = nullptr;
  float* zbuf = nullptr;

  DNet d[2];
  std::vector<DLayer> dl;
  int NB3 = 0;
  float* d_in = nullptr;
  Tn d_act[11];
  Tn d_pool[11];
  Tn d_dz[11];
  Tn d_dpool[11];
  Tn d_ufull;
  float *d_t9 = nullptr, *d_out = nullptr;
  float* g0 = nullptr;
  float* coefs = nullptr;
  float *norms = nullptr, *gp = nullptr;

  depgan_allreduce_fn ar_fn = nullptr;
  void* ar_user = nullptr;
  int world = 1;
  void* rccl_comm = nullptr;
  long rccl_issued = 0;
  int device = 0;
  bool winograd = true;
  bool head_fused = true;
  bool wgrad_bf16 = true;
  float* host_stats = nullptr;
  int* best_dev = nullptr;
  int* best_host = nullptr;
  float* z_best = nullptr;

  float* part = nullptr;
  size_t partFloats = 0;
  float* raw = nullptr;
  float* Sraw = nullptr;
  float* scratch = nullptr;
  size_t scratchFloats = 0;
  float* scal = nullptr;
  float* scal_multi = nullptr;
  float* fake_y2 = nullptr;
  float last_sums[8];

  bool infer_only = false;

  bool train_bn = false;
  unsigned last_drop_seed = 0;
  Tn draw_tmp;
  float *logits = nullptr, *dz = nullptr, *loss_dev = nullptr;
  struct {
    DgCeSetting ce;
    DgDiceSetting dice;
    DgBoundarySetting boundary;
  } loss;
  float* bl_phi = nullptr;
  void* bl_rows = nullptr;
  size_t bl_rows_bytes = 0;
  double* bl_part = nullptr;
  struct {
    bool census_valid = false, counts_valid = false, dice_valid = false;
    long long census[DEPGAN_MAX_HEAD_CLASSES * DEPGAN_MAX_HEAD_CLASSES];
    long long counts[DEPGAN_LABEL_NCOUNT];
    double dice_sums[3 * DEPGAN_MAX_HEAD_CLASSES];
    float dice_loss = 0.f;
    bool boundary_valid = false;
    double boundary_loss = 0.0, boundary_M = 0.0;
  } last;
  float *ones1k = nullptr, *zeros1k = nullptr;
  float *n_mean0 = nullptr, *n_rstd0 = nullptr, *n_mean1 = nullptr, *n_rstd1 = nullptr, *n_meanh = nullptr,
        *n_rstdh = nullptr;
  float *n_dl = nullptr, *n_dflat = nullptr, *n_dl1 = nullptr, *n_da0 = nullptr, *n_dl0 = nullptr;

  bool dbg_capture = false;
  float* dbg_mixed[11] = {nullptr, nullptr, nullptr, nullptr, nullptr, nullptr, nullptr, nullptr, nullptr, nullptr, nullptr};
  bool dbg_mixed_valid = false;

  bool h_ready = false, h_valid = false;
  bool fwd_only_bf16 = false;
// ... 206 lines not shown
```

dep_gan_im_amd/csrc/model.hip:

```cpp
#include "model.h"

#include <dlfcn.h>
#include <float.h>
#include <math.h>
#include <stdlib.h>
#include <stdarg.h>
#include <stdio.h>
#include <string.h>

static thread_local char g_err[1024] = "";
void dg_set_error(const char* fmt, ...) {
  va_list ap;
  va_start(ap, fmt);
  vsnprintf(g_err, sizeof(g_err), fmt, ap);
  va_end(ap);
}
const char* dg_get_error() { return g_err; }

void Net::add(const std::string& name, std::vector<int> shape, bool trainable) {
  PInfo pi;
  pi.name = name;
  pi.ndim = (int)shape.size();
  pi.size = 1;
  for (int i = 0; i < 4; ++i) {
// ... 39 lines not shown
}
#define STATS_TAIL 8
static int net_alloc(depgan_ctx* c, Net* n) {
  DGCHECK(dmalloc(c, &n->P, n->nTrain));
  DGCHECK(dmalloc(c, &n->G, n->nTrain + STATS_TAIL));
  DGCHECK(dmalloc(c, &n->M, n->nTrain));
  DGCHECK(dmalloc(c, &n->V, n->nTrain));
  DGCHECK(dmalloc(c, &n->NT, n->nNon));
  if (c->cfg.bf16_weights) {
    DGCHECK(dmalloc(c, &n->Pq, n->nTrain));
    std::vector<unsigned char> m(n->nTrain ? n->nTrain : 4, 0);
    for (const PInfo& pi : n->params) {
      const std::string& nm = pi.name;
      if (pi.trainable && nm.size() > 7 && nm.compare(nm.size() - 7, 7, "/kernel") == 0)
        for (size_t i = 0; i < pi.size; ++i) m[pi.off + i] = 1;
    }
    void* q = nullptr;
    HIPCHECK(hipMalloc(&q, m.size()));
    c->allocs.push_back(q);
    HIPCHECK(hipMemcpy(q, m.data(), m.size(), hipMemcpyHostToDevice));
    n->qmask = (unsigned char*)q;
  }
  return DG_OK;
}

static int net_requantize(depgan_ctx* c, Net& n) {
  if (!n.Pq || n.nTrain == 0) return DG_OK;
  ProfScope ps(c, 2, 0.0, "bf16 round");
  return dg_round_bf16_masked(n.P, n.qmask, n.Pq, n.nTrain, c->st);
}

static ConvPlan plan_conv(const depgan_ctx* c, int KS, int Cin, int Cout, int N = 0, int H = 0, int W = 0) {
  if (c->cfg.f32_split) return dg_plan_conv_split(KS, Cin, Cout, c->cfg.f32_split == 6 ? 3 : 2);
  if (c->cfg.bf16_mfma) return dg_plan_conv_bf16(KS, Cin, Cout);
  const long items = (long)N * cdiv(H, 16) * cdiv(W, 16) * cdiv(Cout, 32);
  if (c->winograd && KS == 3 && H > 0 && W > 0 && !((H | W) & 1)) {
    const ConvPlan w = dg_plan_conv_wino(Cin, Cout);
    if (dg_plan_wino(w)) return w;
  }
  return dg_plan_conv_items(KS, Cin, Cout, items);
}


int conv_launch(depgan_ctx* c, const ConvPlan& pl, const ConvArgs& a, int KS) {
  const int ng = a.groups > 1 ? a.groups : 1;
  const double fl = 2.0 * a.B * a.H * a.W * (double)a.Cin * a.Cout * KS * KS * ng;
  char lb[56], pipe[12] = "";
  if (dg_plan_split(pl)) snprintf(pipe, sizeof(pipe), "(bf16x%d)", pl.planes * (pl.planes + 1) / 2);
  else if (dg_plan_bf16(pl)) snprintf(pipe, sizeof(pipe), "(bf16)");
  snprintf(lb, sizeof(lb), "conv%s k%d b%d %dx%d %d->%d%s", pipe, KS, a.B, a.H, a.W, a.Cin, a.Cout, ng > 1 ? " x4" : "");
  const double px = 4.0 * a.B * a.H * a.W;
  const double by = px * a.Cin + ng * (px * a.Cout * (1 + (a.ep.res.p ? 1 : 0) + (a.ep.mask.p ? 1 : 0) +
                                                      (a.ep.out_pre.p ? 1 : 0) + (a.ep.accumulate ? 1 : 0) +
                                                      (a.ep.pool.p ? 0.25 : 0) - (a.ep.head_skip_out ? 1 : 0)) +
                                          4.0 * KS * KS * a.Cin * a.Cout) +
                    (a.ep.head_out ? px + 4.0 * a.Cout : 0.0);
  if (dg_plan_mfma(pl)) {
    char kn[48] = "";
    if (c->prof_on) dg_conv_igemm_name(pl, a, kn, sizeof(kn));
    ProfScope ps(c, 0, fl, lb, by, kn);
    return dg_conv_igemm(pl, a, c->st);
  }
  ProfScope ps(c, 2, fl, lb);
  return dg_conv_direct(KS, a, c->st);
}

bool deconv_fused(const depgan_ctx* c, const GLayer& L, int n) {
  if (c->cfg.bf16_mfma || c->cfg.f32_split) return false;
  return dg_deconv_fwd_supported(n, L.H, L.W, L.Cin, L.Cout, L.in, L.out);
}
int deconv_fwd_launch(depgan_ctx* c, const GLayer& L, TView out, const float* bias, const float* scale,
                      const float* shift, int relu, int n) {
  DeconvArgs d;
  memset(&d, 0, sizeof(d));
  d.in = L.in.p;
  d.w = L.Wt;
  d.out = out;
  d.bias = bias; d.scale = scale; d.shift = shift; d.relu = relu;
  d.H = L.H; d.W = L.W; d.Cin = L.Cin; d.Cout = L.Cout;
  char lb[56];
  snprintf(lb, sizeof(lb), "conv k1 b%d %dx%d %d->%d x4", n, L.H, L.W, L.Cin, L.Cout);
  const double px = 4.0 * n * L.H * L.W;
  ProfScope ps(c, 0, 2.0 * n * L.H * L.W * (double)L.Cin * L.Cout * 4, lb,
               px * L.Cin + 4 * (px * L.Cout + 4.0 * L.Cin * L.Cout), "deconv_fwd_kernel");
  return dg_deconv_fwd(d, n, c->st);
}

template <typename XV>
int deconv_wgrad_all(depgan_ctx* c, const GLayer& L, XV x, TView dsrc, int n, const float* scale, float* raw,
                     const float* colscale, float* colout, float* colraw) {
  if constexpr (std::is_same<XV, TView>::value) {
    if (!c->cfg.bf16_mfma && !c->cfg.f32_split && dg_deconv_wgrad_supported(n, L.H, L.W, L.Cin, L.Cout, x, dsrc) &&
        dg_deconv_wgrad_part_floats(n, L.H, L.W, L.Cin, L.Cout) <= c->partFloats) {
      DeconvWgradArgs d;
      memset(&d, 0, sizeof(d));
      d.in = x.p;
      d.dout = dsrc;
      d.part = c->part;
      d.colpart = c->scratch;
      d.H = L.H; d.W = L.W; d.Cin = L.Cin; d.Cout = L.Cout;
      int nch = 0;
      {
        char lb[56];
        snprintf(lb, sizeof(lb), "wgrad k1 b%d %dx%d %d->%d x4", n, L.H, L.W, L.Cin, L.Cout);
        ProfScope ps(c, 1, 2.0 * n * L.H * L.W * (double)L.Cin * L.Cout * 4, lb);
        DGCHECK(dg_deconv_wgrad(d, n, &nch, c->st));
      }
      ProfScope ps(c, 2, 0.0, "slab reduce");
      return dg_wgrad_finish_rows(c->part, nch, 4, L.Cin, L.Cout, scale, L.dW, raw, 0, 1, c->scratch, 4 * nch, L.Cout,
                                  colscale, colout, colraw, c->st);
    }
  }
  {
    ProfScope ps(c, 2, 0.0, "colsum");
    DGCHECK(dg_colsum(dsrc, n, 2 * L.H, 2 * L.W, L.Cout, colscale, colout, colraw, 0, c->scratch, c->scratchFloats,
                      c->st));
  }
  for (int t = 0; t < 4; ++t) {
    const size_t o = (size_t)t * L.Cout * L.Cin;
    DGCHECK(wgrad_full(c, 1, x, strided2(dsrc, t / 2, t % 2), n, L.H, L.W, L.Cin, L.Cout, scale, L.dW + o,
                       raw ? raw + o : nullptr, 0, 1));
  }
  return DG_OK;
}
template int deconv_wgrad_all<TView>(depgan_ctx*, const GLayer&, TView, TView, int, const float*, float*, const float*,
                                     float*, float*);
template int deconv_wgrad_all<TViewH>(depgan_ctx*, const GLayer&, TViewH, TView, int, const float*, float*,
                                      const float*, float*, float*);

int deconv_bwd_data(depgan_ctx* c, GLayer& L, TView dsrc, int n) {
  ConvArgs a = conv_args(null_view(), L.din, n, L.H, L.W, L.Cout, L.Cin);
  a.ep.mask = L.in_mask;
  if (L.wpb_all) {
    deconv_gather_k(&a, dsrc, L.Cout, L.pb.CK);
    a.w = L.wpb_all;
    return conv_launch(c, L.pbf, a, 1);
  }
  for (int t = 0; t < 4; ++t) {
    a.in = strided2(dsrc, t / 2, t % 2);
    a.w = L.wpb[t];
    a.ep.accumulate = (t > 0);
    DGCHECK(conv_launch(c, L.pb, a, 1));
  }
  return DG_OK;
}

void zero_ep(Epilogue* e) {
  memset(e, 0, sizeof(*e));
  e->out_pre = e->res = e->mask = e->pool = null_view();
}

TView view_offset(TView v, long samples) {
  v.p += samples * v.sB;
  return v;
}
void deconv_gather_k(ConvArgs* a, TView d, int Cout, int CK) {
  a->in = strided2(d, 0, 0);
  a->Cin = 4 * Cout;
  a->cpt = Cout / CK;
  for (int t = 0; t < 4; ++t) a->in_run_off[t] = (long)(t / 2) * d.sY + (long)(t % 2) * d.sX;
}

static int wgrad_launch(int kernel, int KS, const WgradArgs& a, int* nch, hipStream_t st) {
  if (kernel == DG_WG_F32) return dg_wgrad(KS, a, nch, st);
  if (kernel == DG_WG_EDGE) return dg_wgrad_small(KS, a, nch, st);
  return dg_wgrad_bf16(KS, a, nch, st);
}
static int wgrad_launch(int, int KS, const WgradArgsH& a, int* nch, hipStream_t st) { return dg_wgrad_bf16s(KS, a, nch, st); }

template <typename XV>
int wgrad_run(const WgradWs& ws, int KS, XV x, TView dy, int N, int H, int W, int Cin, int Cout, const float* scale,
              float* out, float* raw, int accumulate, int oi, const ColSum* cs) {
  constexpr bool x_bf16 = std::is_same<XV, TViewH>::value;
  typedef typename std::conditional<x_bf16, WgradArgsH, WgradArgs>::type Args;
  depgan_ctx* c = ws.prof;
  float* const scratch = ws.scratch;
  const size_t cap = ws.scratchFloats;
  DgWgradChoice ch;
  DGCHECK(dg_wgrad_choose(KS, N, H, W, Cin, Cout, ws.bf16, x_bf16, &ch));
  if (ch.part_floats > ws.partFloats) {
    dg_set_error("wgrad slab workspace too small");
    return DG_ERR_ARG;
  }
  const bool rows = cs && ch.col_rows;
  if (rows && (size_t)ch.col_rows * Cout > cap) {
    dg_set_error("wgrad column-sum workspace too small (%d rows of %d floats, capacity %zu)", ch.col_rows, Cout, cap);
    return DG_ERR_ARG;
  }
  if (cs && !rows) {
    ProfScope ps(c, 2, 0.0, "colsum");
    DGCHECK(dg_colsum(dy, cs->B, H, W, Cout, cs->scale, cs->out, cs->raw, 0, scratch, cap, ws.st));
  }
  Args a = wgrad_args_of<Args>(x, dy, ws.part, N, H, W, Cin, Cout);
  if (rows) {
    a.colpart = scratch;
    a.colB = cs->B;
  }
  int nch = 0;
  {
    static const char* const tag[] = {"wgrad", "wgrad", "wgrad(bf16)", "wgrad(bf16s)"};
    char lb[56];
    snprintf(lb, sizeof(lb), "%s k%d b%d %dx%d %d->%d", tag[ch.kernel], KS, N, H, W, Cin, Cout);
// ... 462 lines not shown
  }
  ProfScope ps(c, 2, 0.0, "pack weights");
  return dg_pack_weights_batch(D.pack_jobs, D.n_pack, D.pack_blocks, c->st);
}

int g_forward(depgan_ctx* c, const float* x, const float* z, int n, bool store_u) {
  {
    ProfScope ps(c, 2, 0.0, "noise mlp fwd");
    DGCHECK(dg_noise_fwd(c->np, z, c->na, n, c->st));
  }
  bool pooled_by_conv = false, head_by_conv = false;
  for (size_t i = 0; i < c->gl.size(); ++i) {
    GLayer& L = c->gl[i];
    if (L.kind == G_CONV || L.kind == G_FILM) {
      ConvArgs a = conv_args((i == 0) ? make_view(const_cast<float*>(x), L.H, L.W, L.Cin) : L.in, L.out,
                             n, L.H, L.W, L.Cin, L.Cout);
      g_layer_epilogue(&a.ep, L, c->na.heads, L.in);
      if (L.kind == G_FILM && store_u) a.ep.out_pre = L.u.view();
      conv_set_weights(&a, L.pf, L.wpf[0], L.Wt, L.Cin, L.Cout);
      if (dg_plan_mfma(L.pf) && g_pool_follows(c->gl, i)) a.ep.pool = c->gl[i + 1].out;
      pooled_by_conv = a.ep.pool.p != nullptr;
      head_by_conv = false;
      if (L.kind == G_CONV && i + 1 < c->gl.size() && c->gl[i + 1].kind == G_HEAD && c->cfg.nc_out == 1 &&
          c->head_fused && dg_conv_igemm_head_supported(L.pf, a)) {
        const GLayer& Hd = c->gl[i + 1];
        a.ep.head_w = Hd.Wt; a.ep.head_b = Hd.b; a.ep.head_out = c->attr.p;
        a.ep.head_tanh = 1;
        a.ep.head_skip_out = (!store_u && !c->dbg_capture) ? 1 : 0;
        head_by_conv = true;
      }
      DGCHECK(conv_launch(c, L.pf, a, 3));
    } else if (L.kind == G_POOL) {
      if (pooled_by_conv && L.skip_of == (int)i - 1) continue;
      ProfScope ps(c, 2, 0.0, "maxpool");
      DGCHECK(dg_maxpool(c->gl[L.skip_of].out, L.out, n, L.H / 2, L.W / 2, L.Cout, c->st));
    } else if (L.kind == G_DECONV) {
      if (deconv_fused(c, L, n)) {
        DGCHECK(deconv_fwd_launch(c, L, L.out, L.b, L.s, L.t, 1, n));
        continue;
      }
      ConvArgs a = conv_args(L.in, L.out, n, L.H, L.W, L.Cin, L.Cout);
      g_layer_epilogue(&a.ep, L, c->na.heads, L.in);
      deconv_groups(&a, L.out, L.wpf);
      DGCHECK(conv_launch(c, L.pf, a, 1));
    } else if (L.kind == G_HEAD && c->cfg.nc_out == 1) {
      if (head_by_conv) continue;
      ProfScope ps(c, 2, 0.0, "head fwd");
      DGCHECK(dg_head_fwd(L.in.p, L.Wt, L.b, c->attr.p, (long)n * L.H * L.W, L.Cin, 1, c->st));
    }
  }
  return DG_OK;
}

static int g_conv_bn_bwd(depgan_ctx* c, GLayer& L, size_t li, const float* x_user, TView dy, TView res, int n) {
  TView xin = (li == 0) ? make_view(const_cast<float*>(x_user), L.H, L.W, L.Cin) : L.in;
  const ColSum cs = {n, L.s, L.db, L.dbeta};
  DGCHECK(wgrad_full(c, 3, xin, dy, n, L.H, L.W, L.Cin, L.Cout, L.s, L.dW, c->raw_all + (L.dW - c->g.G), 0, 0, &cs));
  if (li == 0) return DG_OK;
  ConvArgs a = conv_args(dy, L.din, n, L.H, L.W, L.Cout, L.Cin);
  a.w = L.wpb[0];
  a.ep.res = res;
  a.ep.mask = L.in_mask;
  return conv_launch(c, L.pb, a, 3);
}

int g_backward(depgan_ctx* c, const float* x, const float* z, int n) {
  for (int i = (int)c->gl.size() - 1; i >= 0; --i) {
    GLayer& L = c->gl[i];
    if (L.kind == G_HEAD) {
      ProfScope ps(c, 2, 0.0, "head bwd");
      const long P = (long)n * L.H * L.W;
      DGCHECK(dg_colsum_rowmul(L.in, n, L.H, L.W, L.Cin, c->dpre, L.dW, c->scratch, c->scratchFloats, c->st));
      DGCHECK(dg_sum(c->dpre, (size_t)P, L.db, c->scratch, c->scratchFloats, c->st));
      DGCHECK(dg_head_bwd(c->dpre, L.Wt, L.in.p, L.din.p, P, L.Cin, c->st));
    } else if (L.kind == G_CONV) {
      DGCHECK(g_conv_bn_bwd(c, L, (size_t)i, x, L.dout, null_view(), n));
    } else if (L.kind == G_FILM) {
      TView du = make_view(c->du_tmp.p, L.H, L.W, L.Cout);
      {
        ProfScope ps(c, 2, 0.0, "film bwd");
        DGCHECK(dg_film_bwd(L.dout.p, L.u.p, c->na.heads + L.col_mul, c->na.heads + L.col_add, 1024, du.p,
                            c->dheads + L.col_mul, c->dheads + L.col_add, n, (long)L.H * L.W, L.Cout, c->scratch,
                            c->scratchFloats, c->st));
      }
      DGCHECK(g_conv_bn_bwd(c, L, (size_t)i, x, du, L.dout, n));
    } else if (L.kind == G_POOL) {
      ProfScope ps(c, 2, 0.0, "unpool+mask");
      DGCHECK(dg_unpool_mask(L.pool_dsrc, c->gl[L.skip_of].out, L.pool_skipgrad, L.pool_dst, n, L.H / 2, L.W / 2,
                             L.Cout, c->st));
    } else if (L.kind == G_DECONV) {
      DGCHECK(deconv_wgrad_all(c, L, L.in, L.dout, n, L.s, c->raw_all + (L.dW - c->g.G), L.s, L.db, L.dbeta));
      DGCHECK(deconv_bwd_data(c, L, L.dout, n));
    }
  }
  return g_backward_finish(c, z, n);
}

int g_backward_finish(depgan_ctx* c, const float* z, int n) {
  {
    if (!c->g_gamma_jobs) {
      std::vector<GammaJob> jobs;
      int blk = 0;
      for (size_t i = 0; i < c->gl.size(); ++i) {
        const GLayer& L = c->gl[i];
        if (L.kind != G_CONV && L.kind != G_FILM && L.kind != G_DECONV) continue;
        const bool de = L.kind == G_DECONV;
        jobs.push_back({L.Wt, c->raw_all + (L.dW - c->g.G), L.b, L.mean, L.rstd, L.dbeta, L.dgamma,
                        (de ? 4 : 9) * L.Cin, L.Cout, de ? 1 : 0, L.Cin, blk});
        blk += L.Cout;
      }
      c->g_n_gamma = (int)jobs.size();
      c->g_gamma_blocks = blk;
      DGCHECK(upload_table(c, jobs, &c->g_gamma_jobs));
    }
    ProfScope ps(c, 2, 0.0, "bn gamma grad");
    DGCHECK(dg_bn_gamma_grad_batch(c->g_gamma_jobs, c->g_n_gamma, c->g_gamma_blocks, c->st));
  }
  ProfScope ps(c, 2, 0.0, "noise mlp bwd");
  return dg_noise_bwd(c->np, c->ng, z, c->na, c->dheads, c->scratch, c->scratchFloats, n, c->st);
}

static TView d_in_view(depgan_ctx* c, int l, long s0) {
  const Tn& t = c->dl[l - 1].pool ? c->d_pool[l - 1] : c->d_act[l - 1];
  return view_offset(t.view(), s0);
}

static const ConvPlan& d_plan_f(const depgan_ctx* c, int l) {
  return (c->critic16_bf16 && c->dl[l].has16f) ? c->dl[l].pf16 : c->dl[l].pf;
}
static const float* d_panel_f(const depgan_ctx* c, const DNet& D, int l) {
  return (c->critic16_bf16 && c->dl[l].has16f) ? D.wpf16[l] : D.wpf[l];
}
static const ConvPlan& d_plan_b(const depgan_ctx* c, int l) {
  return (c->critic16_bf16 && c->dl[l].has16b) ? c->dl[l].pb16 : c->dl[l].pb;
}
static const float* d_panel_b(const depgan_ctx* c, const DNet& D, int l) {
  return (c->critic16_bf16 && c->dl[l].has16b) ? D.wpb16[l] : D.wpb[l];
}

static int d_forward(depgan_ctx* c, DNet& D, const float* img, long s0, int N) {
  const int H0 = c->cfg.height, W0 = c->cfg.width;
  for (int l = 0; l < 11; ++l) {
    const DLayer& L = c->dl[l];
    ConvArgs a = conv_args((l == 0) ? make_view(const_cast<float*>(img), H0, W0, 1) : d_in_view(c, l, s0),
                           view_offset(c->d_act[l].view(), s0), N, L.H, L.W, L.Cin, L.Cout);
    a.ep.bias = D.b[l];
    a.ep.relu = 1;
    const ConvPlan& pf = d_plan_f(c, l);
    conv_set_weights(&a, pf, d_panel_f(c, D, l), D.W[l], L.Cin, L.Cout);
    if (dg_plan_mfma(pf) && L.pool && !((L.H | L.W) & 1))
      a.ep.pool = view_offset(c->d_pool[l].view(), s0);
    DGCHECK(conv_launch(c, pf, a, L.KS));
    if (L.pool && !a.ep.pool.p) {
      ProfScope ps(c, 2, 0.0, "maxpool");
      DGCHECK(dg_maxpool(a.out, view_offset(c->d_pool[l].view(), s0), N, L.H / 2, L.W / 2, L.Cout, c->st));
    }
  }
  const DLayer& T = c->dl[10];
  const int HW = T.H * T.W;
  ProfScope ps(c, 2, 0.0, "critic tail fwd");
  return dg_critic_tail_fwd(c->d_act[10].p + s0 * c->d_act[10].per_sample(), D.w9, D.b9, D.wd, D.bd,
                            c->d_t9 + s0 * HW, c->d_out + s0, N, HW, 256, c->st);
}

static int d_backward_chain(depgan_ctx* c, DNet& D, long s0, int N, const float* coefs, int per, long img_s0,
                            int img_n, float* g0_out) {
  const DLayer& T = c->dl[10];
  const int HW = T.H * T.W;
  {
    ProfScope ps(c, 2, 0.0, "critic tail bwd");
    DGCHECK(dg_critic_tail_bwd(c->d_act[10].p + s0 * c->d_act[10].per_sample(), D.w9, D.wd, coefs, per,
                               c->d_dz[10].p + s0 * c->d_dz[10].per_sample(), N, HW, 256, c->st));
  }
  for (int l = 10; l >= 1; --l) {
    const DLayer& L = c->dl[l];
    const DLayer& Pv = c->dl[l - 1];
    ConvArgs a = conv_args(view_offset(c->d_dz[l].view(), s0), null_view(), N, L.H, L.W, L.Cout, L.Cin);
    a.w = d_panel_b(c, D, l);
    if (Pv.pool) {
      a.out = view_offset(c->d_dpool[l - 1].view(), s0);
    } else {
      a.out = view_offset(c->d_dz[l - 1].view(), s0);
      a.ep.mask = view_offset(c->d_act[l - 1].view(), s0);
    }
    DGCHECK(conv_launch(c, d_plan_b(c, l), a, L.KS));
    if (Pv.pool) {
      ProfScope ps(c, 2, 0.0, "unpool+mask");
      DGCHECK(dg_unpool_mask(a.out, view_offset(c->d_act[l - 1].view(), s0), null_view(),
                             view_offset(c->d_dz[l - 1].view(), s0), N, Pv.H / 2, Pv.W / 2, Pv.Cout, c->st));
    }
  }
  if (img_n > 0) {
    const DLayer& L = c->dl[0];
    ConvArgs a = conv_args(view_offset(c->d_dz[0].view(), s0 + img_s0), make_view(g0_out, L.H, L.W, 1),
                           img_n, L.H, L.W, L.Cout, 1);
    conv_set_weights_bwd(&a, dg_plan_direct(), nullptr, D.W[0], L.Cin, L.Cout);
    DGCHECK(conv_launch(c, dg_plan_direct(), a, L.KS));
  }
  return DG_OK;
}

int net_adam(depgan_ctx* c, Net& n, float gscale) {
  n.adam_t += 1;
  const double b1 = c->cfg.beta1, b2 = c->cfg.beta2;
  const double t = (double)n.adam_t;
  const double lr_t = n.lr * sqrt(1.0 - pow(b2, t)) / (1.0 - pow(b1, t));
  if (n.clipnorm == 0.f && n.clipvalue == 0.f && n.weight_decay == 0.f) {
    ProfScope ps(c, 2, 0.0, "adam");
    return dg_adam(n.P, n.G, n.M, n.V, n.nTrain, (float)lr_t, (float)b1, (float)b2, c->cfg.adam_eps, gscale, c->st);
  }
  if (n.clipnorm > 0.f) {
    ProfScope ps(c, 2, 0.0, "grad sqnorm");
    DGCHECK(dg_grad_sqnorm(n.G, n.nTrain, gscale, c->scratch, c->scratchFloats, n.gnorm, c->st));
    n.gnorm_valid = true;
  }
  ProfScope ps(c, 2, 0.0, "adam opts");
  return dg_adam_opts(n.P, n.G, n.M, n.V, n.nTrain, (float)lr_t, n.lr, (float)b1, (float)b2, c->cfg.adam_eps, gscale,
                      n.clipnorm, n.clipvalue, n.weight_decay, n.decay_bits, n.gnorm, c->st);
}

static int net_opt_alloc(depgan_ctx* c, Net& n) {
  if (n.gnorm) return DG_OK;
  const size_t words = (n.nTrain + 31) / 32 + 1;
  std::vector<unsigned> bits(words, 0u);
  for (const PInfo& pi : n.params) {
    const std::string& nm = pi.name;
    if (pi.trainable && nm.size() > 7 && nm.compare(nm.size() - 7, 7, "/kernel") == 0)
      for (size_t i = pi.off; i < pi.off + pi.size; ++i) bits[i >> 5] |= 1u << (i & 31);
  }
  void* b = nullptr;
  HIPCHECK(dalloc_bytes(c, &b, words * sizeof(unsigned)));
  HIPCHECK(hipMemcpy(b, bits.data(), words * sizeof(unsigned), hipMemcpyHostToDevice));
  void* g = nullptr;
  HIPCHECK(dalloc_bytes(c, &g, 4 * sizeof(double)));
  n.decay_bits = (unsigned*)b;
  n.gnorm = (double*)g;
  return dalloc_fills_done();
}

// ... 224 lines not shown
  return DG_OK;
}

static Net* pick_net(depgan_ctx* c, int net) {
  if (net == DEPGAN_NET_G) return &c->g;
  if (net == DEPGAN_NET_D_Y2) return &c->d[0].net;
  if (net == DEPGAN_NET_D_DEM) return &c->d[1].net;
  dg_set_error("unknown net id %d", net);
  return nullptr;
}

extern "C" {

const char* depgan_last_error(void) { return dg_get_error(); }

int depgan_abi_version(void) { return DEPGAN_ABI_VERSION; }
size_t depgan_config_size(void) { return sizeof(depgan_config); }

int depgan_create(const depgan_config* cfg, depgan_ctx** out) {
  if (!cfg || !out) { dg_set_error("depgan_create: null argument"); return DG_ERR_ARG; }
  if (cfg->struct_size != (int)sizeof(depgan_config)) {
    dg_set_error("depgan_create: depgan_config.struct_size is %d, this library (ABI %d) expects %d -- the caller was "
                 "built against another include/depgan.h", cfg->struct_size, DEPGAN_ABI_VERSION,
                 (int)sizeof(depgan_config));
    return DG_ERR_ARG;
  }
  if (cfg->f32_split != 0 && ((cfg->f32_split != 3 && cfg->f32_split != 6) || cfg->bf16_weights || cfg->bf16_mfma ||
                               (cfg->nc_out != 0 && cfg->nc_out != 1))) {
    dg_set_error("depgan_create: f32_split must be 0, 3 or 6, without bf16_weights / bf16_mfma, nc_out = 1");
    return DG_ERR_ARG;
  }
  if (cfg->bf16_mfma && !cfg->bf16_weights) {
    dg_set_error("depgan_create: bf16_mfma needs bf16_weights = 1 and nc_out = 1 (the DEP-GAN generator) or nc_out in "
                 "[2, %d] (the DEP-UResNet as a predict-only inference context)", DEPGAN_MAX_HEAD_CLASSES);
    return DG_ERR_ARG;
  }
  if (cfg->batch < 1 || cfg->height % 16 || cfg->width % 16 || cfg->height < 16 || cfg->width < 16 || cfg->nicg < 1 ||
      cfg->nicg > 2) {
    dg_set_error("depgan_create: need batch >= 1, height/width multiples of 16, nicg in {1,2}");
    return DG_ERR_ARG;
  }
  depgan_ctx* c = new depgan_ctx();
  c->cfg = *cfg;
  if (hipGetDevice(&c->device) != hipSuccess) c->device = 0;
  {
    const char* e = getenv("DEPGAN_WGRAD_BF16");
    c->wgrad_bf16 = !(e && atoi(e) == 0);
    const char* hf = getenv("DEPGAN_HEAD_FUSED");
    c->head_fused = !(hf && atoi(hf) == 0);
    const char* hfs = getenv("DEPGAN_BF16S_HEAD_FUSED");
    c->bf16s_head_fused = !(hfs && atoi(hfs) == 0);
    const char* wn = getenv("DEPGAN_WINOGRAD");
    c->winograd = !(wn && atoi(wn) == 0);
  }
  if (c->cfg.nc_out == 0) c->cfg.nc_out = 1;
  if (c->cfg.nc_out < 1 || c->cfg.nc_out > DEPGAN_MAX_HEAD_CLASSES) {
    dg_set_error("depgan_create: nc_out must be 1 (DEP-GAN) or in [2, %d] (DEP-UResNet classes), not %d",
                 DEPGAN_MAX_HEAD_CLASSES, c->cfg.nc_out);
    delete c;
    return DG_ERR_ARG;
  }
  c->infer_only = c->cfg.bf16_mfma && c->cfg.nc_out >= 2;
  c->train_bn = c->cfg.nc_out != 1 && !c->infer_only;
  memset(c->last_sums, 0, sizeof(c->last_sums));
  int rc = build_generator(c);
  if (rc == DG_OK && !c->train_bn && !c->infer_only) rc = build_critics(c);
  if (rc == DG_OK && c->train_bn) rc = uresnet_build(c);
  if (rc == DG_OK && c->infer_only)
    rc = dmalloc(c, &c->logits, (size_t)cfg->batch * cfg->height * cfg->width * c->cfg.nc_out);
  if (rc == DG_OK && !c->infer_only) {
    size_t mx = 0;
    const int B = cfg->batch;
    const bool pipe = cfg->bf16_mfma != 0, store = pipe && c->cfg.nc_out == 1;
    auto call = [&](int KS, int N, const auto& L, bool x_bf16) {
      auto form = [&](bool bf16_pipe, bool xh) {
        DgWgradChoice ch;
        if (dg_wgrad_choose(KS, N, L.H, L.W, L.Cin, L.Cout, bf16_pipe, xh, &ch) == DG_OK && ch.part_floats > mx)
          mx = ch.part_floats;
      };
      form(false, false);
      if (pipe) form(true, false);
      if (x_bf16) form(false, true);
    };
    for (size_t i = 0; i < c->gl.size(); ++i) {
      const GLayer& L = c->gl[i];
      if (L.kind == G_CONV || L.kind == G_FILM) call(3, B, L, store && i > 0);
      else if (L.kind == G_DECONV) call(1, B, L, store);
      else if (L.kind == G_HEAD && c->train_bn && L.Cout == 4) call(1, B, L, false);
      if (L.kind == G_DECONV && dg_deconv_wgrad_supported(B, L.H, L.W, L.Cin, L.Cout, L.in, L.dout)) {
        const size_t f4 = dg_deconv_wgrad_part_floats(B, L.H, L.W, L.Cin, L.Cout);
        if (f4 > mx) mx = f4;
      }
    }
    for (const DLayer& L : c->dl) call(L.KS, 3 * B, L, false);
    c->partFloats = mx;
    rc = dmalloc(c, &c->part, mx);
  }
  if (rc == DG_OK && !c->infer_only) rc = dmalloc(c, &c->raw, (size_t)9 * 256 * 256);
  if (rc == DG_OK && !c->train_bn && !c->infer_only) rc = dmalloc(c, &c->raw_all, c->g.nTrain);
  if (rc == DG_OK) rc = dmalloc(c, &c->Sraw, 256);
  c->scratchFloats = (size_t)(1 << 20) + (size_t)cfg->batch * 20000;
  if (rc == DG_OK) rc = dmalloc(c, &c->scratch, c->scratchFloats);
  if (rc == DG_OK) rc = dmalloc(c, &c->scal, 16);
  if (rc == DG_OK) rc = dmalloc(c, &c->scal_multi, 8 * DEPGAN_MAX_MULTI);
  if (rc == DG_OK) rc = dmalloc(c, &c->z_best, (size_t)cfg->batch * 32);
  if (rc == DG_OK) {
// ... 500 lines not shown
```

dep_gan_im_amd/csrc/op_entries.hip:

```cpp
#include "model.h"

#include <math.h>
#include <stdlib.h>
#include <stdio.h>
#include <string.h>

int op_pack_jobs(PackJob* jobs, int n, hipStream_t st) {
  const unsigned nb = dg_pack_layout(jobs, n);
  DevTmp jd(st);
  DGCHECK(jd.alloc(n * sizeof(PackJob)));
  hipError_t e = hipMemcpyAsync(jd.p, jobs, n * sizeof(PackJob), hipMemcpyHostToDevice, st);
  if (e != hipSuccess) { dg_set_error("op_pack_jobs: upload failed: %s", hipGetErrorString(e)); return DG_ERR_HIP; }
  return dg_pack_weights_batch(jd.as<PackJob>(), n, nb, st);
}

static int op_alloc(DevTmp* t, size_t floats, const char* who) {
  if (t->alloc((floats ? floats : 1) * sizeof(float)) != DG_OK) {
    dg_set_error("%s: out of device memory (%zu floats)", who, floats);
    return DG_ERR_HIP;
  }
  return DG_OK;
}

template <typename XV>
int op_wgrad(const char* who, int KS, XV x, TView dy, int B, int H, int W, int Cin, int Cout, bool bf16,
             const float* scale, float* dw, float* raw, int accumulate, int oi, const ColSum* cs, hipStream_t st) {
  DgWgradChoice ch;
  DGCHECK(dg_wgrad_choose(KS, B, H, W, Cin, Cout, bf16, std::is_same<XV, TViewH>::value, &ch));
  WgradWs ws;
  memset(&ws, 0, sizeof(ws));
  ws.partFloats = ch.part_floats;
  ws.scratchFloats = !cs ? 0 : ch.col_rows ? (size_t)ch.col_rows * Cout : dg_colsum_scratch(cs->B, H, W, Cout);
  ws.bf16 = bf16;
  ws.st = st;
  DevTmp part(st), scratch(st);
  DGCHECK(op_alloc(&part, ws.partFloats, who));
  DGCHECK(op_alloc(&scratch, ws.scratchFloats, who));
  ws.part = part.as<float>();
  ws.scratch = scratch.as<float>();
  return wgrad_run(ws, KS, x, dy, B, H, W, Cin, Cout, scale, dw, raw, accumulate, oi, cs);
}
template int op_wgrad<TViewH>(const char*, int, TViewH, TView, int, int, int, int, int, bool, const float*, float*, float*,
                              int, int, const ColSum*, hipStream_t);

extern "C" {

static int op_conv_run(ConvArgs a, const float* w_hwio, int Cin, int Cout, int KS, int path, int bwd, hipStream_t st) {
  const int ci = a.Cin, co = a.Cout;
  ConvPlan pl = (path == 3) ? dg_plan_conv_bf16(KS, ci, co)
                : (path == 4 || path == 5) ? dg_plan_conv_split(KS, ci, co, path == 5 ? 3 : 2)
                : (path == 6) ? dg_plan_conv_items(KS, ci, co, 1L << 30) : dg_plan_conv(KS, ci, co);
  if (path == 7) pl = dg_plan_conv_items(KS, ci, co, 1L << 30);
  if (path == 10) {
    if (KS != 5) { dg_set_error("op_conv: path 10 is the 16-channel 5x5 bf16 kernel, KS must be 5"); return DG_ERR_ARG; }
    if (!a.in.p || !a.out.p || !w_hwio) { dg_set_error("op_conv: null operand"); return DG_ERR_ARG; }
    if (a.ep.head_w || a.ep.head_b || a.ep.head_out) { dg_set_error("op_conv: path 10 has no fused head"); return DG_ERR_ARG; }
    pl = dg_plan_conv_bf16_n16(KS, ci, co);
    if (!dg_plan_bf16(pl) || pl.MF != 16) { dg_set_error("op_conv: the 16-channel bf16 kernel does not cover a launch of %d -> %d channels", ci, co); return DG_ERR_UNSUPPORTED; }
  }
  if (path == 8) {
    pl = (KS == 3) ? dg_plan_conv_wino(ci, co) : pl;
    if (!dg_plan_wino(pl) || !dg_conv_wino_supported(pl, a)) { dg_set_error("op_conv: the Winograd kernel does not cover this shape"); return DG_ERR_UNSUPPORTED; }
  }
  if ((path == 6 || path == 7) && pl.CK != 8) { dg_set_error("op_conv: the 8-channel-chunk variant does not cover this shape"); return DG_ERR_UNSUPPORTED; }
  if (path >= 3 && path <= 5 && !pl.planes) { dg_set_error("op_conv: the bf16 MFMA kernel does not cover this shape"); return DG_ERR_UNSUPPORTED; }
  if (path == 9 && KS != 5) { dg_set_error("op_conv: path 9 is the weight-stationary 5x5 kernel, KS must be 5"); return DG_ERR_ARG; }
  if (path == 9 && !dg_conv_igemm_ws5_supported(pl, a, true)) { dg_set_error("op_conv: the weight-stationary 5x5 kernel does not cover this shape"); return DG_ERR_UNSUPPORTED; }
  if (path == 1 && !dg_plan_mfma(pl)) { dg_set_error("op_conv: MFMA path not available for this shape"); return DG_ERR_UNSUPPORTED; }
  if (path != 2 && dg_plan_mfma(pl)) {
    DevTmp wp(st);
    DGCHECK(wp.alloc(pl.packedFloats * sizeof(float)));
    DGCHECK(dg_pack_weights(pl, w_hwio, Cin, Cout, 0, bwd, bwd, nullptr, wp.as<float>(), st));
    a.w = wp.as<float>();
    if (path == 7) {
      if (dg_conv_igemm_wp_supported(pl, a, true)) return dg_conv_igemm_wp(pl, a, st);
      dg_set_error("op_conv: the wave-private kernel does not cover this shape");
      return DG_ERR_UNSUPPORTED;
    }
    if (path == 9) return dg_conv_igemm_ws5(pl, a, st);
    if (path == 6 || path == 1) return dg_conv_igemm_tile(pl, a, st);
    return dg_conv_igemm(pl, a, st);
  }
  if (!bwd) conv_set_weights(&a, dg_plan_direct(), nullptr, w_hwio, Cin, Cout);
  else conv_set_weights_bwd(&a, dg_plan_direct(), nullptr, w_hwio, Cin, Cout);
  return dg_conv_direct(KS, a, st);
}

static int op_conv(const float* in, const float* w_hwio, const float* bias, float* out, int B, int H, int W, int Cin,
                   int Cout, int KS, int relu, int path, int bwd, hipStream_t st) {
  const int ci = bwd ? Cout : Cin, co = bwd ? Cin : Cout;
  ConvArgs a = conv_args(make_view(const_cast<float*>(in), H, W, ci), make_view(out, H, W, co), B, H, W, ci, co);
  a.ep.bias = bias;
  a.ep.relu = relu;
  return op_conv_run(a, w_hwio, Cin, Cout, KS, path, bwd, st);
}

int depgan_op_conv2d_stamps(const float* in, const float* w_hwio, float* out, int B, int H, int W, int Cin, int Cout,
                            int KS, unsigned long long* stamps, int reps, void* stream) {
  hipStream_t st = (hipStream_t)stream;
  ConvArgs a = conv_args(make_view(const_cast<float*>(in), H, W, Cin), make_view(out, H, W, Cout), B, H, W, Cin, Cout);
  a.ep.relu = 1;
  ConvPlan pl = dg_plan_conv(KS, Cin, Cout);
  if (!dg_plan_mfma(pl)) { dg_set_error("no MFMA variant"); return DG_ERR_UNSUPPORTED; }
  DevTmp wp(st);
  DGCHECK(wp.alloc(pl.packedFloats * sizeof(float)));
  DGCHECK(dg_pack_weights(pl, w_hwio, Cin, Cout, 0, 0, 0, nullptr, wp.as<float>(), st));
  a.w = wp.as<float>();
  for (int i = 0; i < reps; ++i) {
    a.dbg = (i == reps - 1) ? stamps : nullptr;
    DGCHECK(dg_conv_igemm(pl, a, st));
  }
  return DG_OK;
}

int depgan_op_conv2d(const float* in, const float* w_hwio, const float* bias, float* out, int B, int H, int W,
                     int Cin, int Cout, int KS, int relu, int path, void* stream) {
  return op_conv(in, w_hwio, bias, out, B, H, W, Cin, Cout, KS, relu, path, 0, (hipStream_t)stream);
}
int depgan_op_conv2d_bwd_data(const float* dy, const float* w_hwio, float* dx, int B, int H, int W, int Cin,
                              int Cout, int KS, int path, void* stream) {
  return op_conv(dy, w_hwio, nullptr, dx, B, H, W, Cin, Cout, KS, 0, path, 1, (hipStream_t)stream);
// ... 73 lines not shown
  DGCHECK(dev.alloc(DEPGAN_EVAL_NCOUNT * sizeof(unsigned long long)));
  DGCHECK(dg_eval_counts(x, nicg, pred, code_real, mask1, wmh1, mask2, wmh2, prob2, (size_t)npix, thr,
                         dev.as<unsigned long long>(), st));
  unsigned long long h[DEPGAN_EVAL_NCOUNT];
  if (hipMemcpyAsync(h, dev.p, sizeof(h), hipMemcpyDeviceToHost, st) != hipSuccess ||
      hipStreamSynchronize(st) != hipSuccess) {
    dg_set_error("eval_counts: copy back failed");
    return DG_ERR_HIP;
  }
  for (int k = 0; k < DEPGAN_EVAL_NCOUNT; ++k) out_host[k] = (long long)h[k];
  return DG_OK;
}


static size_t op_scratch(long scratch_floats, size_t need) { return scratch_floats > 0 ? (size_t)scratch_floats : need; }


int depgan_op_conv2d_fused(const float* in, long isB, long isY, long isX, const float* w_hwio, const float* bias,
                           const float* scale, const float* shift, const float* film_mul, const float* film_add,
                           int film_ld, float* out, long osB, long osY, long osX, float* out_pre, long psB, long psY,
                           long psX, const float* res, long rsB, long rsY, long rsX, const float* mask, long msB,
                           long msY, long msX, float* pool, long qsB, long qsY, long qsX, const float* head_w,
                           const float* head_b, float* head_out, int head_tanh, int head_skip_out, int B, int H, int W,
                           int Cin, int Cout, int KS, int relu, int accumulate, int path, int bwd, void* stream) {
  if (op_view_bad_batched(in, isB, isY, isX) || op_view_bad_batched(out, osB, osY, osX) || !w_hwio || B < 1 || H < 1 || W < 1 || Cin < 1 ||
      Cout < 1 || (KS != 1 && KS != 3 && KS != 5) || (out_pre && op_view_bad_batched(out_pre, psB, psY, psX)) ||
      (res && op_view_bad_batched(res, rsB, rsY, rsX)) || (mask && op_view_bad_batched(mask, msB, msY, msX)) ||
      (pool && op_view_bad_batched(pool, qsB, qsY, qsX))) {
    dg_set_error("op_conv2d_fused: null or non-positive argument");
    return DG_ERR_ARG;
  }
  const int co = bwd ? Cin : Cout;
  if (!scale != !shift || !film_mul != !film_add || (film_mul && film_ld < co)) {
    dg_set_error("op_conv2d_fused: scale / shift and film_mul / film_add come in pairs, film_ld >= output channels");
    return DG_ERR_ARG;
  }
  if ((head_w || head_b || head_out) && !(head_w && head_b && head_out)) { dg_set_error("op_conv2d_fused: null head argument"); return DG_ERR_ARG; }
  if (head_skip_out && !head_out) { dg_set_error("op_conv2d_fused: head_skip_out without a head"); return DG_ERR_ARG; }
  if (path < 1 || path > 10) { dg_set_error("op_conv2d_fused: path must be 1 ... 10"); return DG_ERR_ARG; }
  ConvArgs a = conv_args(op_view(in, isB, isY, isX), op_view(out, osB, osY, osX), B, H, W, bwd ? Cout : Cin, co);
  Epilogue& e = a.ep;
  e.bias = bias; e.scale = scale; e.shift = shift;
  e.film_mul = film_mul; e.film_add = film_add; e.film_ld = film_ld;
  e.out_pre = op_view_or_null(out_pre, psB, psY, psX);
  e.res = op_view_or_null(res, rsB, rsY, rsX);
  e.mask = op_view_or_null(mask, msB, msY, msX);
  e.pool = op_view_or_null(pool, qsB, qsY, qsX);
  e.relu = relu; e.accumulate = accumulate;
  e.head_w = head_w; e.head_b = head_b; e.head_out = head_out;
  e.head_tanh = head_tanh; e.head_skip_out = head_skip_out;
  return op_conv_run(a, w_hwio, Cin, Cout, KS, path, bwd ? 1 : 0, (hipStream_t)stream);
}


int depgan_op_conv3x3_wino_gathered(const float* in, long isB, long isY, long isX, const long* run_off, int runs,
                                    const float* w_hwio, const float* bias, float* out, long osB, long osY, long osX,
                                    int B, int H, int W, int Cin, int Cout, void* stream) {
  if (op_view_bad_batched(in, isB, isY, isX) || op_view_bad_batched(out, osB, osY, osX) || !w_hwio || !run_off || B < 1 || H < 1 ||
      W < 1 || Cin < 1 || Cout < 1 || runs < 1 || runs > 4) {
    dg_set_error("op_conv3x3_wino_gathered: null or non-positive argument, or not 1 ... 4 runs");
    return DG_ERR_ARG;
  }
  if (Cin % (runs * 8)) {
    dg_set_error("op_conv3x3_wino_gathered: %d channels are not %d runs of whole 8-channel chunks", Cin, runs);
    return DG_ERR_UNSUPPORTED;
  }
  ConvArgs a = conv_args(op_view(in, isB, isY, isX), op_view(out, osB, osY, osX), B, H, W, Cin, Cout);
  a.ep.bias = bias;
  a.cpt = Cin / (runs * 8);
  for (int t = 0; t < runs; ++t) a.in_run_off[t] = run_off[t];
  return op_conv_run(a, w_hwio, Cin, Cout, 3, 8, 0, (hipStream_t)stream);
}


static_assert(DEPGAN_EPF_BIAS == DG_EPF_BIAS && DEPGAN_EPF_AFFINE == DG_EPF_AFFINE && DEPGAN_EPF_FILM == DG_EPF_FILM &&
              DEPGAN_EPF_RELU == DG_EPF_RELU && DEPGAN_EPF_PRE == DG_EPF_PRE && DEPGAN_EPF_RES == DG_EPF_RES &&
              DEPGAN_EPF_MASK == DG_EPF_MASK && DEPGAN_EPF_POOL == DG_EPF_POOL && DEPGAN_EPF_ACCUM == DG_EPF_ACCUM &&
              DEPGAN_EPF_HEAD == DG_EPF_HEAD && DEPGAN_EPF_ALL == DG_EPF_ALL, "include/depgan.h and common.h");
int depgan_set_epilogue_classes(int on) {
  if (on != 0 && on != 1) { dg_set_error("set_epilogue_classes: 0 or 1, not %d", on); return DG_ERR_ARG; }
  dg_set_epi_classes(on);
  return DG_OK;
}
int depgan_get_epilogue_classes(void) { return dg_get_epi_classes(); }
int depgan_wino_epilogue_class(unsigned flags, int form) {
  if ((flags & ~(unsigned)DG_EPF_ALL) || form < 0 || form > 3) {
    dg_set_error("wino_epilogue_class: flags 0x%x outside DEPGAN_EPF_ALL or form %d outside 0 ... 3", flags, form);
    return -1;
  }
  return dg_wino_epi_class(flags, form);
}
int depgan_op_conv3x3_wino_kernel_name(unsigned flags, int B, int H, int W, int Cin, int Cout, char* buf, int cap) {
  if ((flags & ~(unsigned)DG_EPF_ALL) || B < 1 || H < 1 || W < 1 || Cin < 1 || Cout < 1 || !buf || cap < 1) {
    dg_set_error("op_conv3x3_wino_kernel_name: null or non-positive argument, or flags outside DEPGAN_EPF_ALL");
    return DG_ERR_ARG;
  }
  static float present;
  const TView pv = make_view(&present, H, W, Cout);
  ConvArgs a = conv_args(make_view(&present, H, W, Cin), pv, B, H, W, Cin, Cout);
  Epilogue& e = a.ep;
  if (flags & DG_EPF_BIAS) e.bias = &present;
  if (flags & DG_EPF_AFFINE) e.scale = e.shift = &present;
  if (flags & DG_EPF_FILM) { e.film_mul = e.film_add = &present; e.film_ld = Cout; }
  e.relu = (flags & DG_EPF_RELU) ? 1 : 0;
  if (flags & DG_EPF_PRE) e.out_pre = pv;
  if (flags & DG_EPF_RES) e.res = pv;
// ... 752 lines not shown
```

dep_gan_im_amd/csrc/ops.hip:

```cpp
#include "ops.h"
#include <float.h>
#include <hip/hip_bf16.h>
#include "epilogue.h"

__device__ __forceinline__ float wave_sum(float v) {
#pragma unroll
  for (int o = 32; o > 0; o >>= 1) v += __shfl_down(v, o, 64);
  return v;
}
__device__ __forceinline__ float block_sum(float v, float* sh4) {
  v = wave_sum(v);
  __syncthreads();
  if ((threadIdx.x & 63) == 0) sh4[threadIdx.x >> 6] = v;
  __syncthreads();
  return (sh4[0] + sh4[1]) + (sh4[2] + sh4[3]);
}

static inline int nblk(size_t n, int cap = 2048) {
  size_t b = (n + 255) / 256;
  return (int)(b > (size_t)cap ? cap : (b < 1 ? 1 : b));
}

static int scratch_ok(const char* who, size_t need, size_t have) {
  if (need <= have) return 1;
  dg_set_error("%s: scratch holds %zu floats, the launch needs %zu", who, have, need);
  return 0;
}

__device__ __forceinline__ int first_argmax4(float a0, float a1, float a2, float a3) {
  int k = 0;
  float m = a0;
  if (a1 > m) { m = a1; k = 1; }
  if (a2 > m) { m = a2; k = 2; }
  if (a3 > m) { m = a3; k = 3; }
  return k;
}

__global__ void maxpool_kernel(TView in, TView out, int B, int Ho, int Wo, int C4) {
  const size_t total = (size_t)B * Ho * Wo * C4;
  for (size_t i = blockIdx.x * (size_t)blockDim.x + threadIdx.x; i < total; i += (size_t)gridDim.x * blockDim.x) {
    size_t q = i;
    const int c = (int)(q % C4) * 4;
    q /= C4;
    const int x = (int)(q % Wo);
    q /= Wo;
    const int y = (int)(q % Ho);
    const int b = (int)(q / Ho);
    const float* p = in.p + view_off(in, b, 2 * y, 2 * x) + c;
    const f32x4 a0 = *reinterpret_cast<const f32x4*>(p);
    const f32x4 a1 = *reinterpret_cast<const f32x4*>(p + in.sX);
    const f32x4 a2 = *reinterpret_cast<const f32x4*>(p + in.sY);
    const f32x4 a3 = *reinterpret_cast<const f32x4*>(p + in.sY + in.sX);
    f32x4 m;
#pragma unroll
    for (int k = 0; k < 4; ++k) m[k] = fmaxf(fmaxf(a0[k], a1[k]), fmaxf(a2[k], a3[k]));
    *reinterpret_cast<f32x4*>(out.p + view_off(out, b, y, x) + c) = m;
  }
}

int dg_maxpool(TView in, TView out, int B, int Ho, int Wo, int C, hipStream_t st) {
  if (C % 4) { dg_set_error("dg_maxpool: C %% 4 != 0"); return DG_ERR_ARG; }
  const size_t total = (size_t)B * Ho * Wo * (C / 4);
  hipLaunchKernelGGL(maxpool_kernel, dim3(nblk(total, 8192)), dim3(256), 0, st, in, out, B, Ho, Wo, C / 4);
  HIPCHECK(hipGetLastError());
  return DG_OK;
}

template <int MODE>
__global__ void pool_bwd_kernel(TView d, TView a, TView skip, TView out, int B, int Ho, int Wo, int C4) {
  const size_t total = (size_t)B * Ho * Wo * C4;
  for (size_t i = blockIdx.x * (size_t)blockDim.x + threadIdx.x; i < total; i += (size_t)gridDim.x * blockDim.x) {
    size_t q = i;
    const int c = (int)(q % C4) * 4;
    q /= C4;
    const int x = (int)(q % Wo);
    q /= Wo;
    const int y = (int)(q % Ho);
    const int b = (int)(q / Ho);
    const float* pa = a.p + view_off(a, b, 2 * y, 2 * x) + c;
    f32x4 av[4];
    av[0] = *reinterpret_cast<const f32x4*>(pa);
    av[1] = *reinterpret_cast<const f32x4*>(pa + a.sX);
    av[2] = *reinterpret_cast<const f32x4*>(pa + a.sY);
    av[3] = *reinterpret_cast<const f32x4*>(pa + a.sY + a.sX);
    if (MODE == 0) {
      const f32x4 dv = *reinterpret_cast<const f32x4*>(d.p + view_off(d, b, y, x) + c);
      f32x4 o[4];
#pragma unroll
// ... 1029 lines not shown
```

include/depgan.h:

```cpp
#ifndef DEPGAN_H
#define DEPGAN_H
#include <stddef.h>
#ifdef __cplusplus
extern "C" {
#endif

typedef struct depgan_ctx depgan_ctx;

#define DEPGAN_ABI_VERSION 3
int depgan_abi_version(void);
size_t depgan_config_size(void);
const char* depgan_source_hash(void);

typedef struct depgan_config {
  int struct_size;
  int batch;
  int height;
  int width;
  int nicg;
  int first_fm;
  float im_thresh;
  float delta;
  float lrD, lrG;
  float beta1, beta2, adam_eps;
// ... 202 lines not shown
int depgan_op_head_bwd_bf16s(int backward, const void* a, long ld, const float* w, const float* dpre, float* out, long P,
                             int C, void* hip_stream);

int depgan_op_conv2d_bf16s(const void* in, long isB, long isY, long isX, const float* w_hwio, const float* bias,
                           const float* scale, const float* shift, const float* film_mul, const float* film_add,
                           int film_ld, const void* res, long rsB, long rsY, long rsX, void* out, long osB, long osY,
                           long osX, void* pool, int B, int H, int W, int Cin, int Cout, int KS, int relu,
                           void* hip_stream);
int depgan_op_conv2d_head_bf16s(const void* in, long isB, long isY, long isX, const float* w_hwio, const float* bias,
                                const float* scale, const float* shift, const float* film_mul, const float* film_add,
                                int film_ld, const void* res, long rsB, long rsY, long rsX, void* out, long osB,
                                long osY, long osX, void* pool, int B, int H, int W, int Cin, int Cout, int KS, int relu,
                                const float* head_w, const float* head_b, float* head_out, int tanh_act, int skip_out,
                                void* hip_stream);
int depgan_op_deconv2x2_bf16s(const void* in, long isB, long isY, long isX, const float* w_hwoi, const float* bias,
                              const float* scale, const float* shift, void* out, long osB, long osY, long osX, int B,
                              int H, int W, int Cin, int Cout, int relu, void* hip_stream);
int depgan_op_edge_conv_bf16s(const float* in, const float* w_hwio, const float* bias, const float* scale,
                              const float* shift, void* out, long osB, long osY, long osX, int B, int H, int W, int Cin,
                              int Cout, int relu, void* hip_stream);
int depgan_op_head_bf16s(const void* a, const float* w, const float* b, float* out, long P, int C, int tanh_act,
                         void* hip_stream);
int depgan_op_head_softmax_bf16s(const void* a, long ld, const float* w, const float* b, float* probs,
                                 float* logits_or_null, long P, int C, void* hip_stream);
int depgan_op_head_softmax_k_bf16s(const void* a, long ld, const float* w, const float* b, float* probs,
                                   float* logits_or_null, long P, int C, int K, void* hip_stream);

int depgan_op_conv2d(const float* in, const float* w_hwio, const float* bias, float* out, int B, int H, int W,
                     int Cin, int Cout, int KS, int relu, int path, void* hip_stream);
int depgan_op_conv2d_bwd_data(const float* dy, const float* w_hwio, float* dx, int B, int H, int W, int Cin,
                              int Cout, int KS, int path, void* hip_stream);
int depgan_op_conv2d_wgrad(const float* x, const float* dy, float* dw_hwio, int B, int H, int W, int Cin, int Cout,
                           int KS, void* hip_stream);
int depgan_op_conv2d_wgrad_bf16(const float* x, const float* dy, float* dw_hwio, int B, int H, int W, int Cin,
                                int Cout, int KS, void* hip_stream);

int depgan_op_conv2d_stamps(const float* in, const float* w_hwio, float* out, int B, int H, int W, int Cin, int Cout,
                            int KS, unsigned long long* stamps, int reps, void* hip_stream);
int depgan_op_maxpool(const float* in, float* out, int B, int Ho, int Wo, int C, void* hip_stream);
int depgan_op_deconv2x2(const float* in, const float* w_hwoi, const float* bias, const float* scale,
                        const float* shift, float* out, int B, int H, int W, int Cin, int Cout, int relu,
                        void* hip_stream);

int depgan_op_deconv2x2_wgrad(const float* in, const float* dout, float* dw_hwoi, float* colsum, int B, int H, int W,
                              int Cin, int Cout, void* hip_stream);

int depgan_op_conv2d_fused(const float* in, long isB, long isY, long isX, const float* w_hwio, const float* bias,
                           const float* scale, const float* shift, const float* film_mul, const float* film_add,
                           int film_ld, float* out, long osB, long osY, long osX, float* out_pre, long psB, long psY,
                           long psX, const float* res, long rsB, long rsY, long rsX, const float* mask, long msB,
                           long msY, long msX, float* pool, long qsB, long qsY, long qsX, const float* head_w,
                           const float* head_b, float* head_out, int head_tanh, int head_skip_out, int B, int H, int W,
                           int Cin, int Cout, int KS, int relu, int accumulate, int path, int bwd, void* hip_stream);
int depgan_op_conv3x3_wino_gathered(const float* in, long isB, long isY, long isX, const long* run_off, int runs,
                                    const float* w_hwio, const float* bias, float* out, long osB, long osY, long osX,
                                    int B, int H, int W, int Cin, int Cout, void* hip_stream);
#define DEPGAN_EPF_BIAS 1
#define DEPGAN_EPF_AFFINE 2
#define DEPGAN_EPF_FILM 4
#define DEPGAN_EPF_RELU 8
#define DEPGAN_EPF_PRE 16
#define DEPGAN_EPF_RES 32
#define DEPGAN_EPF_MASK 64
#define DEPGAN_EPF_POOL 128
#define DEPGAN_EPF_ACCUM 256
#define DEPGAN_EPF_HEAD 512
#define DEPGAN_EPF_ALL 1023
int depgan_set_epilogue_classes(int on);
int depgan_get_epilogue_classes(void);
int depgan_wino_epilogue_class(unsigned flags, int form);
int depgan_op_conv3x3_wino_kernel_name(unsigned flags, int B, int H, int W, int Cin, int Cout, char* buf, int cap);
int depgan_op_deconv2x2_igemm(int form, const float* in, long isB, long isY, long isX, const float* w_hwoi,
                              const float* bias, const float* scale, const float* shift, float* out, long osB, long osY,
                              long osX, const float* mask, long msB, long msY, long msX, int B, int H, int W, int Cin,
                              int Cout, int relu, int path, void* hip_stream);
int depgan_op_conv2d_wgrad_ex(const float* x, long xsB, long xsY, long xsX, const float* dy, long dsB, long dsY,
                              long dsX, const float* scale, float* dw, float* raw, int accumulate, int oi, int colB,
                              const float* colscale, float* colout, float* colraw, int B, int H, int W, int Cin,
                              int Cout, int KS, int bf16, void* hip_stream);
int depgan_debug_wgrad_plan(int kernel, int KS, int B, int H, int W, int Cin, int Cout, int out[4]);
int depgan_debug_wgrad_choice(int KS, int B, int H, int W, int Cin, int Cout, int bf16_pipe, int x_bf16, long out[4]);

int depgan_op_bn_moments(const float* x, long sB, long sY, long sX, int B, int H, int W, int C, float* mean, float* var,
                         long scratch_floats, void* hip_stream);
int depgan_op_bn_backward(const float* dy, const float* raw, float* draw, long sB, long sY, long sX, int B, int H, int W,
                          int C, const float* gamma, const float* mean, const float* var, float eps, float invN,
                          float dyscale, float* dgamma, float* dbeta, long scratch_floats, void* hip_stream);
int depgan_op_affine_act(const float* in, float* out, float* out_pre, const float* res, long sB, long sY, long sX,
                         const float* s, const float* t, const float* film_mul, const float* film_add, int film_ld,
                         int relu, int B, int H, int W, int C, unsigned drop_seed, float drop_rate, void* hip_stream);
int depgan_op_softmax_ce4(const float* logits, const float* onehot, float* probs, float* dz, float* loss_sum, long P,
                          void* hip_stream);
int depgan_op_softmax_ce(const float* logits, const float* onehot, const unsigned char* codes, float* probs, float* dz,
                         float* loss_sum, long P, int C, void* hip_stream);
int depgan_op_softmax_ce_census(const float* logits, const float* onehot, const unsigned char* codes, float* probs,
                                float* dz, float* loss_sum, long long* census_host, long P, int C, void* hip_stream);
int depgan_op_softmax_ce_weighted(const float* logits, const float* onehot, const unsigned char* codes,
                                  const float* w_host, int n, int ignore_code, float* probs, float* dz, float* loss_sum,
                                  long long* census_host, long long* counts_host, long P, int C, void* hip_stream);
int depgan_op_softmax_ce_focal(const float* logits, const float* onehot, const unsigned char* codes, const float* w_host,
                               int n, int ignore_code, float gamma, float label_smoothing, float* probs, float* dz,
                               float* loss_sum, long long* census_host, long long* counts_host, long P, int C,
                               void* hip_stream);
int depgan_op_label_counts(const float* onehot, const unsigned char* codes, long P, int C, int ignore_code,
                           long long* out_host, void* hip_stream);
int depgan_op_dice_loss(const float* probs, const float* onehot, const unsigned char* codes, int ignore_code, int form,
// ... 72 lines not shown
```

Baseline: 712.9 slices/s.

## Fuse max-unpool and mask into backward conv epilogues for generator and critics

```diff
diff --git a/dep_gan_im_amd/csrc/common.h b/dep_gan_im_amd/csrc/common.h
--- a/dep_gan_im_amd/csrc/common.h
+++ b/dep_gan_im_amd/csrc/common.h
@@ -74,6 +74,9 @@
   const float* head_b;
   float* head_out;
   int head_tanh, head_skip_out;
+  TView unpool_act;
+  TView unpool_out;
+  TView unpool_skip;
 };
 
 struct ConvArgs {
@@ -231,8 +234,11 @@
 bool dg_conv_igemm_ws5_supported(const ConvPlan& pl, const ConvArgs& a, bool force);
 int dg_conv_igemm_ws5(const ConvPlan& pl, const ConvArgs& a, hipStream_t st);
 const char* dg_conv_igemm_ws5_name(const ConvPlan& pl);
+const char* dg_conv_igemm_ws5_unpool_name(const ConvPlan& pl);
 int dg_conv_igemm_tile(const ConvPlan& pl, const ConvArgs& a, hipStream_t st);
 bool dg_conv_igemm_head_supported(const ConvPlan& pl, const ConvArgs& a);
+bool dg_conv_igemm_unpool_supported(const ConvPlan& pl, const ConvArgs& a);
+bool dg_conv_wino_unpool_supported(const ConvArgs& a);
 ConvPlan dg_plan_conv_wino(int Cin, int Cout);
 bool dg_conv_wino_supported(const ConvPlan& pl, const ConvArgs& a);
 const char* dg_conv_wino_name(const ConvArgs& a);
diff --git a/dep_gan_im_amd/csrc/direct.hip b/dep_gan_im_amd/csrc/direct.hip
--- a/dep_gan_im_amd/csrc/direct.hip
+++ b/dep_gan_im_amd/csrc/direct.hip
@@ -297,8 +297,8 @@
 
 int dg_conv_direct(int KS, const ConvArgs& a_in, hipStream_t st) {
   ConvArgs a = a_in;
-  if (a.ep.pool.p || a.ep.head_out || a.ep.head_skip_out || a.groups > 1 || a.cpt > 0) {
-    dg_set_error("dg_conv_direct: no fused pool, fused head, grouped launch or gathered K on the direct kernels");
+  if (a.ep.pool.p || a.ep.head_out || a.ep.head_skip_out || a.groups > 1 || a.cpt > 0 || a.ep.unpool_out.p) {
+    dg_set_error("dg_conv_direct: no fused pool, un-pool or head, grouped launch or gathered K on the direct kernels");
     return DG_ERR_UNSUPPORTED;
   }
   auto aligned = [](const TView& v) {
diff --git a/dep_gan_im_amd/csrc/epilogue.h b/dep_gan_im_amd/csrc/epilogue.h
--- a/dep_gan_im_amd/csrc/epilogue.h
+++ b/dep_gan_im_amd/csrc/epilogue.h
@@ -18,6 +18,26 @@
 __device__ __forceinline__ long view_off(const TView& v, int b, int y, int x) {
   return (long)b * v.sB + (long)y * v.sY + (long)x * v.sX;
 }
+
+__device__ __forceinline__ int first_argmax4(float a0, float a1, float a2, float a3) {
+  int k = 0;
+  float m = a0;
+  if (a1 > m) { m = a1; k = 1; }
+  if (a2 > m) { m = a2; k = 2; }
+  if (a3 > m) { m = a3; k = 3; }
+  return k;
+}
+
+struct EpiRunTime {
+  static constexpr bool fixed = false, bias = false, affine = false, film = false, relu = false, pre = false, res = false,
+                        msk = false, pool = false, head = false, unpool = false;
+  static constexpr int uskip = -1;
+};
+struct EpiUnpoolOnly {
+  static constexpr bool fixed = true, bias = false, affine = false, film = false, relu = false, pre = false, res = false,
+                        msk = false, pool = false, head = false, unpool = true;
+  static constexpr int uskip = -1;
+};
 
 __device__ __forceinline__ float film_preact(float u, float fmul, float fadd) {
 #pragma clang fp contract(off)
diff --git a/dep_gan_im_amd/csrc/igemm_conv.hip b/dep_gan_im_amd/csrc/igemm_conv.hip
--- a/dep_gan_im_amd/csrc/igemm_conv.hip
+++ b/dep_gan_im_amd/csrc/igemm_conv.hip
@@ -1,4 +1,6 @@
 #include <stdlib.h>
+
+#include <type_traits>
 
 #include "common.h"
 #include "epilogue.h"
@@ -40,7 +42,7 @@
   static __device__ __forceinline__ int row(int j, int h) { return 4 * h + j; }
 };
 
-template <int MF, int KS, int CK, int TAPG, bool PERS, bool HEAD>
+template <int MF, int KS, int CK, int TAPG, bool PERS, bool HEAD, bool UNP = false>
 static __device__ __forceinline__ void igemm_conv_body(const ConvArgs& a) {
   constexpr int NT = MF;
   constexpr int PAD = KS / 2;
@@ -297,7 +299,11 @@
 
   if (dbg && tid == 0) dbg[4] = __builtin_amdgcn_s_memtime();
 #define EPI_HEAD HEAD
+#define EPI_UNPOOL UNP
+#define EPI_CLASS std::conditional_t<UNP, EpiUnpoolOnly, EpiRunTime>
 #include "igemm_epilogue.inc"
+#undef EPI_CLASS
+#undef EPI_UNPOOL
 #undef EPI_HEAD
   if (dbg && tid == 0) {
     dbg[5] = __builtin_amdgcn_s_memtime();
@@ -310,6 +316,11 @@
 template <int MF, int KS, int CK, int TAPG, bool PERS>
 __global__ __launch_bounds__(256, (PERS && KS == 3) ? (CK == 8 ? 4 : 3) : 1) void igemm_conv_kernel(const ConvArgs a) {
   igemm_conv_body<MF, KS, CK, TAPG, PERS, false>(a);
+}
+
+template <int MF, int CK, bool PERS>
+__global__ __launch_bounds__(256, 1) void igemm_conv5_unpool_kernel(const ConvArgs a) {
+  igemm_conv_body<MF, 5, CK, 25, PERS, false, true>(a);
 }
 
 template <bool PERS>
@@ -385,8 +396,15 @@
     dg_set_error("dg_conv_igemm: the fused head needs the 8-channel-chunk 3x3 kernel and 32 output channels");
     return DG_ERR_ARG;
   }
+  constexpr bool CAN_UNPOOL = (KS == 5 && TAPG == 25);
+  const bool unp = a.ep.unpool_out.p != nullptr;
+  if (unp && !CAN_UNPOOL) {
+    dg_set_error("dg_conv_igemm: among the tile kernels the fused un-pool rides on the 5x5 forms only");
+    return DG_ERR_UNSUPPORTED;
+  }
   if (name_out) {
-    if (head) snprintf(name_out, name_cap, "igemm_conv_head_kernel<%s>", G < total ? "true" : "false");
+    if (unp) snprintf(name_out, name_cap, "igemm_conv5_unpool_kernel<%d,%d,%s>", MF, CK, G < total ? "true" : "false");
+    else if (head) snprintf(name_out, name_cap, "igemm_conv_head_kernel<%s>", G < total ? "true" : "false");
     else snprintf(name_out, name_cap, "igemm_conv_kernel<%d,%d,%d,%d,%s>", MF, KS, CK, TAPG, G < total ? "true" : "false");
     return DG_OK;
   }
@@ -401,6 +419,21 @@
       }
       if (G < total) hipLaunchKernelGGL((igemm_conv_head_kernel<true>), dim3((unsigned)G), dim3(256), lds, st, b);
       else hipLaunchKernelGGL((igemm_conv_head_kernel<false>), dim3((unsigned)G), dim3(256), lds, st, b);
+      HIPCHECK(hipGetLastError());
+      return DG_OK;
+    }
+  }
+  if constexpr (CAN_UNPOOL) {
+    if (unp) {
+      static DgOncePerDevice once_u;
+      if (once_u.need()) {
+        HIPCHECK(hipFuncSetAttribute(reinterpret_cast<const void*>(&igemm_conv5_unpool_kernel<MF, CK, false>),
+                                     hipFuncAttributeMaxDynamicSharedMemorySize, (int)lds));
+        HIPCHECK(hipFuncSetAttribute(reinterpret_cast<const void*>(&igemm_conv5_unpool_kernel<MF, CK, true>),
+                                     hipFuncAttributeMaxDynamicSharedMemorySize, (int)lds));
+      }
+      if (G < total) hipLaunchKernelGGL((igemm_conv5_unpool_kernel<MF, CK, true>), dim3((unsigned)G), dim3(256), lds, st, b);
+      else hipLaunchKernelGGL((igemm_conv5_unpool_kernel<MF, CK, false>), dim3((unsigned)G), dim3(256), lds, st, b);
       HIPCHECK(hipGetLastError());
       return DG_OK;
     }
@@ -438,6 +471,13 @@
          !a.ep.accumulate;
 }
 
+bool dg_conv_igemm_unpool_supported(const ConvPlan& pl, const ConvArgs& a) {
+  if (!dg_plan_mfma(pl) || dg_plan_bf16(pl) || dg_plan_split(pl) || a.groups > 1 || a.cpt > 0 || a.dbg) return false;
+  if (dg_epilogue_flags(a.ep) != 0) return false;
+  if (dg_plan_wino(pl)) return dg_conv_wino_unpool_supported(a);
+  return dg_plan_tile5(pl);
+}
+
 void dg_conv_igemm_name(const ConvPlan& pl, const ConvArgs& a, char* buf, size_t cap) {
   if (cap) buf[0] = 0;
   if (!dg_plan_mfma(pl)) { snprintf(buf, cap, "conv_direct"); return; }
@@ -445,7 +485,10 @@
   if (dg_plan_bf16(pl)) { snprintf(buf, cap, "%s", dg_conv_igemm_bf16_name(pl)); return; }
   if (dg_plan_wino(pl)) { snprintf(buf, cap, "%s", dg_conv_wino_name(a)); return; }
   if (dg_conv_igemm_wp_supported(pl, a, false)) { snprintf(buf, cap, "igemm_wp_kernel<0>"); return; }
-  if (dg_conv_igemm_ws5_supported(pl, a, false)) { snprintf(buf, cap, "%s", dg_conv_igemm_ws5_name(pl)); return; }
+  if (dg_conv_igemm_ws5_supported(pl, a, false)) {
+    snprintf(buf, cap, "%s", a.ep.unpool_out.p ? dg_conv_igemm_ws5_unpool_name(pl) : dg_conv_igemm_ws5_name(pl));
+    return;
+  }
   dispatch_tile(pl, a, nullptr, buf, cap);
 }
 
@@ -473,6 +516,25 @@
     if (bad) {
       dg_set_error("dg_conv_igemm: gathered K needs Cin = runs (<= 4) x cpt x %d channels and 16-byte run offsets", pl.CK);
       return DG_ERR_ARG;
+    }
+  }
+  if (a.ep.unpool_out.p || a.ep.unpool_act.p || a.ep.unpool_skip.p) {
+    const Epilogue& e = a.ep;
+    if (!e.unpool_out.p || !e.unpool_act.p) {
+      dg_set_error("dg_conv_igemm: the fused un-pool needs its destination and its activation view");
+      return DG_ERR_ARG;
+    }
+    if (e.pool.p || e.head_out || e.accumulate || e.out_pre.p || a.groups > 1) {
+      dg_set_error("dg_conv_igemm: the fused un-pool excludes pool, head, accumulate, out_pre and grouped launches");
+      return DG_ERR_ARG;
+    }
+    if (misaligned(e.unpool_out) || misaligned(e.unpool_act) || misaligned(e.unpool_skip)) {
+      dg_set_error("dg_conv_igemm: the un-pool views must be 16-byte aligned");
+      return DG_ERR_ARG;
+    }
+    if (!dg_conv_igemm_unpool_supported(pl, a)) {
+      dg_set_error("dg_conv_igemm: no kernel of this plan carries the fused un-pool (plain launches on the fp32 5x5 tile and weight-stationary kernels and the Winograd 8-row kernel)");
+      return DG_ERR_UNSUPPORTED;
     }
   }
   if (a.ep.head_out && !dg_conv_igemm_head_supported(pl, a)) {
diff --git a/dep_gan_im_amd/csrc/igemm_epilogue.inc b/dep_gan_im_amd/csrc/igemm_epilogue.inc
--- a/dep_gan_im_amd/csrc/igemm_epilogue.inc
+++ b/dep_gan_im_amd/csrc/igemm_epilogue.inc
@@ -49,6 +49,17 @@
   const bool affine = e.scale != nullptr, film = e.film_mul != nullptr, relu = e.relu != 0, accum = e.accumulate != 0;
   const bool has_bias = e.bias != nullptr, has_pre = e.out_pre.p != nullptr, has_res = e.res.p != nullptr,
              has_msk = e.mask.p != nullptr, has_pool = e.pool.p != nullptr;
+#endif
+#ifdef EPI_UNPOOL
+#ifdef EPI_CLASS
+  const bool has_unp = EPI_UNPOOL && (EPI_CT ? EpiC::unpool : (e.unpool_out.p != nullptr));
+  const bool has_uskip = has_unp && ((EPI_CT && EpiC::uskip >= 0) ? EpiC::uskip != 0 : (e.unpool_skip.p != nullptr));
+#else
+  const bool has_unp = EPI_UNPOOL && e.unpool_out.p != nullptr;
+  const bool has_uskip = has_unp && e.unpool_skip.p != nullptr;
+#endif
+#else
+  constexpr bool has_unp = false;
 #endif
 #ifdef EPI_OYW
   const int oyw = EPI_OYW;
@@ -95,6 +106,20 @@
     const int lo_pool = has_pool ? 4 * ((pl0 >> 1) * (int)e.pool.sX + co) : 0;
     const int sY_pool = 4 * (int)e.pool.sY, sX_pool = 4 * (int)e.pool.sX;
     f32x4 vrow = {0.f, 0.f, 0.f, 0.f};
+#ifdef EPI_UNPOOL
+    const __amdgpu_buffer_rsrc_t r_ua =
+        mk(has_unp ? e.unpool_act.p + view_off(e.unpool_act, b, 2 * oyw, 2 * tx0) : a.out.p);
+    const __amdgpu_buffer_rsrc_t r_uo =
+        mk(has_unp ? e.unpool_out.p + view_off(e.unpool_out, b, 2 * oyw, 2 * tx0) : a.out.p);
+    const __amdgpu_buffer_rsrc_t r_us =
+        mk(has_uskip ? e.unpool_skip.p + view_off(e.unpool_skip, b, 2 * oyw, 2 * tx0) : a.out.p);
+    const int lo_ua = has_unp ? 4 * (2 * pl0 * (int)e.unpool_act.sX + co) : 0;
+    const int lo_uo = has_unp ? 4 * (2 * pl0 * (int)e.unpool_out.sX + co) : 0;
+    const int lo_us = has_uskip ? 4 * (2 * pl0 * (int)e.unpool_skip.sX + co) : 0;
+    const int sY_ua = 4 * (int)e.unpool_act.sY, sX_ua = 4 * (int)e.unpool_act.sX;
+    const int sY_uo = 4 * (int)e.unpool_out.sY, sX_uo = 4 * (int)e.unpool_out.sX;
+    const int sY_us = 4 * (int)e.unpool_skip.sY, sX_us = 4 * (int)e.unpool_skip.sX;
+#endif
 #ifdef EPI_HEAD
 #ifdef EPI_CLASS
     const bool has_head = EPI_HEAD && (EPI_CT ? EpiC::head : (e.head_out != nullptr));
@@ -119,6 +144,24 @@
     const int sY_pre = 4 * (int)e.out_pre.sY, sX_pre = 4 * (int)e.out_pre.sX;
     const int sY_res = 4 * (int)e.res.sY, sX_res = 4 * (int)e.res.sX;
     const int sY_msk = 4 * (int)e.mask.sY, sX_msk = 4 * (int)e.mask.sX;
+#ifdef EPI_UNPOOL
+    f32x4 ua[4];
+    auto unp_fetch = [&](int q) {
+      constexpr int RPq = 16 / PPP;
+      const int qy = (q & 1) + 2 * (q / (2 * RPq)), qx0 = ((q >> 1) % RPq) * PPP;
+      const bool okq = full || (oyw + qy < a.H && tx0 + qx0 + pl0 < a.W);
+      const int su_a = 2 * (qy * sY_ua + qx0 * sX_ua);
+#pragma unroll
+      for (int w = 0; w < 4; ++w) ua[w] = (f32x4){0.f, 0.f, 0.f, 0.f};
+      if (okq) {
+        ua[0] = ld(r_ua, lo_ua, su_a);
+        ua[1] = ld(r_ua, lo_ua, su_a + sX_ua);
+        ua[2] = ld(r_ua, lo_ua, su_a + sY_ua);
+        ua[3] = ld(r_ua, lo_ua, su_a + sY_ua + sX_ua);
+      }
+    };
+    if (has_unp) unp_fetch(0);
+#endif
 #ifdef EPI_STAGE_LATE
     EPI_STAGE_LATE;
 #endif
@@ -171,6 +214,62 @@
 #pragma unroll
         for (int k = 0; k < 4; ++k) v[k] = (mm[k] > 0.f) ? v[k] : 0.f;
       }
+#ifdef EPI_UNPOOL
+      if (has_unp) {
+        const int su_o = 2 * (py * sY_uo + px0 * sX_uo), su_s = 2 * (py * sY_us + px0 * sX_us);
+        f32x4 av[4], o[4];
+#pragma unroll
+        for (int w = 0; w < 4; ++w) {
+          av[w] = ua[w];
+          o[w] = (f32x4){0.f, 0.f, 0.f, 0.f};
+        }
+        if (has_uskip && ok) {
+          o[0] = ld(r_us, lo_us, su_s);
+          o[1] = ld(r_us, lo_us, su_s + sX_us);
+          o[2] = ld(r_us, lo_us, su_s + sY_us);
+          o[3] = ld(r_us, lo_us, su_s + sY_us + sX_us);
+        }
+        if (p + 1 < NPASS) unp_fetch(p + 1);
+#pragma unroll
+        for (int k = 0; k < 4; ++k) {
+          const float a0 = av[0][k], a1 = av[1][k], a2 = av[2][k], a3 = av[3][k];
+          const bool c1 = a1 > a0;
+          const float m1 = dg_vmax(a0, a1);
+          const bool c2 = a2 > m1;
+          const float m2 = dg_vmax(m1, a2);
+          const bool c3 = a3 > m2;
+          if (!has_uskip) {
+            const float m3 = dg_vmax(m2, a3);
+            const float t = 0.f + v[k];
+            float g = (m3 > 0.f) ? t : 0.f;
+            o[3][k] = c3 ? g : 0.f;
+            g = c3 ? 0.f : g;
+            o[2][k] = c2 ? g : 0.f;
+            g = c2 ? 0.f : g;
+            o[1][k] = c1 ? g : 0.f;
+            o[0][k] = c1 ? 0.f : g;
+          } else {
+            float g = v[k];
+            const float s3 = c3 ? g : 0.f;
+            g = c3 ? 0.f : g;
+            const float s2 = c2 ? g : 0.f;
+            g = c2 ? 0.f : g;
+            const float s1 = c1 ? g : 0.f, s0 = c1 ? 0.f : g;
+            const float t0 = o[0][k] + s0, t1 = o[1][k] + s1, t2 = o[2][k] + s2, t3 = o[3][k] + s3;
+            o[0][k] = (a0 > 0.f) ? t0 : 0.f;
+            o[1][k] = (a1 > 0.f) ? t1 : 0.f;
+            o[2][k] = (a2 > 0.f) ? t2 : 0.f;
+            o[3][k] = (a3 > 0.f) ? t3 : 0.f;
+          }
+        }
+        if (ok) {
+          st(r_uo, lo_uo, su_o, o[0]);
+          st(r_uo, lo_uo, su_o + sX_uo, o[1]);
+          st(r_uo, lo_uo, su_o + sY_uo, o[2]);
+          st(r_uo, lo_uo, su_o + sY_uo + sX_uo, o[3]);
+        }
+      }
+#endif
       const int so = py * sY_out + px0 * sX_out;
       if (accum) {
         f32x4 old = {0.f, 0.f, 0.f, 0.f};
@@ -178,7 +277,7 @@
 #pragma unroll
         for (int k = 0; k < 4; ++k) v[k] += old[k];
       }
-      if (ok && !skip_out) st(r_out, lo_out, so, v);
+      if (ok && !skip_out && !has_unp) st(r_out, lo_out, so, v);
 #ifdef EPI_HEAD
       if (has_head) {
         static_assert(!EPI_HEAD || (NT == 32 && NPASS == 8), "fused head: 32-channel tiles, eight passes");
diff --git a/dep_gan_im_amd/csrc/igemm_wino.hip b/dep_gan_im_amd/csrc/igemm_wino.hip
--- a/dep_gan_im_amd/csrc/igemm_wino.hip
+++ b/dep_gan_im_amd/csrc/igemm_wino.hip
@@ -42,7 +42,8 @@
 
 constexpr unsigned WN_BAR = DG_EPF_BIAS | DG_EPF_AFFINE | DG_EPF_RELU;
 constexpr unsigned WN_FILM = WN_BAR | DG_EPF_FILM | DG_EPF_RES;
-constexpr int WN_NCLASS = 11, WN_HEAD_CLASS = 10;
+constexpr int WN_NCLASS = 13, WN_HEAD_CLASS = 10;
+constexpr int WN_UNPOOL_CLASS = 11, WN_UNPOOL_SKIP_CLASS = 12;
 constexpr unsigned kWnClassMask[WN_NCLASS] = {
     0,
     WN_BAR,
@@ -55,6 +56,8 @@
     DG_EPF_BIAS | DG_EPF_RELU,
     DG_EPF_BIAS | DG_EPF_RELU | DG_EPF_POOL,
     WN_BAR | DG_EPF_HEAD,
+    0,
+    0,
 };
 #define WN_CLASSES8(X) X(1) X(2) X(3) X(4) X(5) X(6) X(7) X(8) X(9)
 template <int EC>
@@ -65,6 +68,8 @@
   static constexpr bool bias = M & DG_EPF_BIAS, affine = M & DG_EPF_AFFINE, film = M & DG_EPF_FILM, relu = M & DG_EPF_RELU,
                         pre = M & DG_EPF_PRE, res = M & DG_EPF_RES, msk = M & DG_EPF_MASK, pool = M & DG_EPF_POOL,
                         head = M & DG_EPF_HEAD;
+  static constexpr bool unpool = EC == WN_UNPOOL_CLASS || EC == WN_UNPOOL_SKIP_CLASS;
+  static constexpr int uskip = EC == WN_UNPOOL_SKIP_CLASS ? 1 : 0;
 };
 
 template <int MT, bool PERS, bool HEAD, bool GATH = false, int ABL = 0, int EC = 0>
@@ -337,7 +342,9 @@
   }
 #define EPI_HEAD HEAD
 #define EPI_CLASS WnEpi<EC>
+#define EPI_UNPOOL WnEpi<EC>::unpool
 #include "igemm_epilogue.inc"
+#undef EPI_UNPOOL
 #undef EPI_CLASS
 #undef EPI_HEAD
 #undef EPI_FETCH
@@ -387,6 +394,12 @@
     {{reinterpret_cast<const void*>(&wino_conv_head_kernel<false, WN_HEAD_CLASS>), "wino_conv_head_kernel<false,10>"},
      {reinterpret_cast<const void*>(&wino_conv_head_kernel<true, WN_HEAD_CLASS>), "wino_conv_head_kernel<true,10>"}}};
 static_assert(WN_HEAD_CLASS == 10, "the names above");
+const WnKern kWnUnpool[2][2] = {
+    {{reinterpret_cast<const void*>(&wino_conv_kernel<1, false, WN_UNPOOL_CLASS>), "wino_conv_kernel<1,false,11>"},
+     {reinterpret_cast<const void*>(&wino_conv_kernel<1, true, WN_UNPOOL_CLASS>), "wino_conv_kernel<1,true,11>"}},
+    {{reinterpret_cast<const void*>(&wino_conv_kernel<1, false, WN_UNPOOL_SKIP_CLASS>), "wino_conv_kernel<1,false,12>"},
+     {reinterpret_cast<const void*>(&wino_conv_kernel<1, true, WN_UNPOOL_SKIP_CLASS>), "wino_conv_kernel<1,true,12>"}}};
+static_assert(WN_UNPOOL_CLASS == 11 && WN_UNPOOL_SKIP_CLASS == 12, "the names above");
 const WnKern kWnGath[2][2] = {
     {{reinterpret_cast<const void*>(&wino_conv_gathered_kernel<1, false>), "wino_conv_gathered_kernel<1,false>"},
      {reinterpret_cast<const void*>(&wino_conv_gathered_kernel<1, true>), "wino_conv_gathered_kernel<1,true>"}},
@@ -458,8 +471,14 @@
   *G = *pers ? cap : *total;
 }
 
+bool dg_conv_wino_unpool_supported(const ConvArgs& a) {
+  return a.ep.unpool_out.p && a.ep.unpool_act.p && dg_get_epi_classes() && wino_mt(a) == 1 && a.cpt <= 0 &&
+         dg_epilogue_flags(a.ep) == 0;
+}
+
 static const WnKern* wino_pick(const ConvArgs& a, int mt, bool pers) {
   const int form = a.ep.head_out ? 1 : (a.cpt > 0 ? 3 : (mt == 2 ? 2 : 0));
+  if (a.ep.unpool_out.p) return &kWnUnpool[a.ep.unpool_skip.p ? 1 : 0][pers];
   const int ec = dg_wino_epi_class(dg_epilogue_flags(a.ep), form);
   if (form == 1) return &kWnHead[ec ? 1 : 0][pers];
   if (form == 3) return &kWnGath[mt - 1][pers];
@@ -490,6 +509,8 @@
       HIPCHECK(hipFuncSetAttribute(own[i].fn, hipFuncAttributeMaxDynamicSharedMemorySize, (int)LDS));
     for (int i = 0; i < 2; ++i)
       HIPCHECK(hipFuncSetAttribute(kWnGath[MT - 1][i].fn, hipFuncAttributeMaxDynamicSharedMemorySize, (int)LDS));
+    for (int i = 0; MT == 1 && i < 4; ++i)
+      HIPCHECK(hipFuncSetAttribute(kWnUnpool[i >> 1][i & 1].fn, hipFuncAttributeMaxDynamicSharedMemorySize, (int)LDS));
     for (int i = 0; MT == 2 && i < 4; ++i)
       HIPCHECK(hipFuncSetAttribute(kWnHead[i >> 1][i & 1].fn, hipFuncAttributeMaxDynamicSharedMemorySize, (int)LDS));
   }
@@ -529,5 +550,9 @@
     dg_set_error("dg_conv_wino: shape not covered (3x3, Cin %% 8, Cout %% 32, even H and W, no groups, a halo tile of the input view within 2 GiB)");
     return DG_ERR_UNSUPPORTED;
   }
+  if (a.ep.unpool_out.p && !dg_conv_wino_unpool_supported(a)) {
+    dg_set_error("dg_conv_wino: the fused un-pool rides on the 8-row kernel's own classes: no other epilogue operand, no gathered K, epilogue classes on");
+    return DG_ERR_UNSUPPORTED;
+  }
   return wino_mt(a) == 2 ? wino_launch<2>(a, st) : wino_launch<1>(a, st);
 }
diff --git a/dep_gan_im_amd/csrc/igemm_wp.hip b/dep_gan_im_amd/csrc/igemm_wp.hip
--- a/dep_gan_im_amd/csrc/igemm_wp.hip
+++ b/dep_gan_im_amd/csrc/igemm_wp.hip
@@ -1,4 +1,6 @@
 #include <stdlib.h>
+
+#include <type_traits>
 
 #include "common.h"
 #include "epilogue.h"
@@ -40,7 +42,7 @@
   static __device__ __forceinline__ acc_t run(float w, float x, acc_t c) { return __builtin_amdgcn_mfma_f32_16x16x4f32(w, x, c, 0, 0, 0); }
 };
 
-template <int MF, int KS, int CK, int ABL>
+template <int MF, int KS, int CK, int ABL, bool UNP = false>
 static __device__ __forceinline__ void igemm_wp_body(const ConvArgs& a) {
   typedef WpGeo<MF, KS, CK> G;
   constexpr int NT = G::NT, MT = G::MT, TW = G::TWX, PAD = G::PAD, NTAPS = G::NTAPS, CKP = G::CKP;
@@ -211,6 +213,8 @@
 #define EPI_ES_BASE wbuf
 #define EPI_OYW ty0
 #define EPI_FULL ((ty0 + 4 <= a.H) && (tx0 + 16 <= a.W))
+#define EPI_UNPOOL UNP
+#define EPI_CLASS std::conditional_t<UNP, EpiUnpoolOnly, EpiRunTime>
         if constexpr (MF == 32) {
 #define EPI_PHASED
 #include "igemm_epilogue.inc"
@@ -222,6 +226,8 @@
 #undef EPI_ES_BASE
 #undef EPI_OYW
 #undef EPI_FULL
+#undef EPI_CLASS
+#undef EPI_UNPOOL
       }
     }
     id += gridDim.x;
@@ -238,6 +244,10 @@
 template <int MF, int CK>
 __global__ __launch_bounds__(ws5_nwmax(MF) * 64, 1) void igemm_ws5_kernel(const ConvArgs a) {
   igemm_wp_body<MF, 5, CK, 0>(a);
+}
+template <int MF, int CK>
+__global__ __launch_bounds__(ws5_nwmax(MF) * 64, 1) void igemm_ws5_unpool_kernel(const ConvArgs a) {
+  igemm_wp_body<MF, 5, CK, 0, true>(a);
 }
 
 }
@@ -343,21 +353,28 @@
 }
 
 const char* dg_conv_igemm_ws5_name(const ConvPlan& pl) { return pl.MF == 32 ? "igemm_ws5_kernel<32,8>" : "igemm_ws5_kernel<16,16>"; }
+const char* dg_conv_igemm_ws5_unpool_name(const ConvPlan& pl) {
+  return pl.MF == 32 ? "igemm_ws5_unpool_kernel<32,8>" : "igemm_ws5_unpool_kernel<16,16>";
+}
 
 template <int MF, int CK>
 static int ws5_launch(ConvArgs& a, hipStream_t st) {
   const int nw = ws5_waves<MF, CK>(a.Cin);
   const size_t lds = ((size_t)a.Cin * 25 * MF + (size_t)nw * WpGeo<MF, 5, CK>::WAVE_FLOATS) * sizeof(float);
   static DgOncePerDevice once;
-  if (once.need())
+  if (once.need()) {
     HIPCHECK(hipFuncSetAttribute(reinterpret_cast<const void*>(&igemm_ws5_kernel<MF, CK>),
                                  hipFuncAttributeMaxDynamicSharedMemorySize, 160 * 1024));
+    HIPCHECK(hipFuncSetAttribute(reinterpret_cast<const void*>(&igemm_ws5_unpool_kernel<MF, CK>),
+                                 hipFuncAttributeMaxDynamicSharedMemorySize, 160 * 1024));
+  }
   a.lgx = (int)wp_groups(a, nw);
   a.lgy = 1;
   long G = dg_cu_count();
   if ((a.lgx & 7) == 0) G -= G % 8;
   if (G > a.lgx || G < 1) G = a.lgx;
-  hipLaunchKernelGGL((igemm_ws5_kernel<MF, CK>), dim3((unsigned)G), dim3(nw * 64), lds, st, a);
+  if (a.ep.unpool_out.p) hipLaunchKernelGGL((igemm_ws5_unpool_kernel<MF, CK>), dim3((unsigned)G), dim3(nw * 64), lds, st, a);
+  else hipLaunchKernelGGL((igemm_ws5_kernel<MF, CK>), dim3((unsigned)G), dim3(nw * 64), lds, st, a);
   HIPCHECK(hipGetLastError());
   return DG_OK;
 }
diff --git a/dep_gan_im_amd/csrc/model.h b/dep_gan_im_amd/csrc/model.h
--- a/dep_gan_im_amd/csrc/model.h
+++ b/dep_gan_im_amd/csrc/model.h
@@ -159,6 +159,7 @@
   long rccl_issued = 0;
   int device = 0;
   bool winograd = true;
+  bool fused_unpool = true;
   bool head_fused = true;
   bool wgrad_bf16 = true;
   float* host_stats = nullptr;
diff --git a/dep_gan_im_amd/csrc/model.hip b/dep_gan_im_amd/csrc/model.hip
--- a/dep_gan_im_amd/csrc/model.hip
+++ b/dep_gan_im_amd/csrc/model.hip
@@ -115,7 +115,8 @@
   const double px = 4.0 * a.B * a.H * a.W;
   const double by = px * a.Cin + ng * (px * a.Cout * (1 + (a.ep.res.p ? 1 : 0) + (a.ep.mask.p ? 1 : 0) +
                                                       (a.ep.out_pre.p ? 1 : 0) + (a.ep.accumulate ? 1 : 0) +
-                                                      (a.ep.pool.p ? 0.25 : 0) - (a.ep.head_skip_out ? 1 : 0)) +
+                                                      (a.ep.pool.p ? 0.25 : 0) - (a.ep.head_skip_out ? 1 : 0) +
+                                                      (a.ep.unpool_out.p ? 7 + (a.ep.unpool_skip.p ? 4 : 0) : 0)) +
                                           4.0 * KS * KS * a.Cin * a.Cout) +
                     (a.ep.head_out ? px + 4.0 * a.Cout : 0.0);
   if (dg_plan_mfma(pl)) {
@@ -210,7 +211,7 @@
 
 void zero_ep(Epilogue* e) {
   memset(e, 0, sizeof(*e));
-  e->out_pre = e->res = e->mask = e->pool = null_view();
+  e->out_pre = e->res = e->mask = e->pool = e->unpool_act = e->unpool_out = e->unpool_skip = null_view();
 }
 
 TView view_offset(TView v, long samples) {
@@ -779,7 +780,8 @@
   return DG_OK;
 }
 
-static int g_conv_bn_bwd(depgan_ctx* c, GLayer& L, size_t li, const float* x_user, TView dy, TView res, int n) {
+static int g_conv_bn_bwd(depgan_ctx* c, GLayer& L, size_t li, const float* x_user, TView dy, TView res, int n,
+                         bool* unpooled = nullptr) {
   TView xin = (li == 0) ? make_view(const_cast<float*>(x_user), L.H, L.W, L.Cin) : L.in;
   const ColSum cs = {n, L.s, L.db, L.dbeta};
   DGCHECK(wgrad_full(c, 3, xin, dy, n, L.H, L.W, L.Cin, L.Cout, L.s, L.dW, c->raw_all + (L.dW - c->g.G), 0, 0, &cs));
@@ -788,10 +790,20 @@
   a.w = L.wpb[0];
   a.ep.res = res;
   a.ep.mask = L.in_mask;
+  const GLayer& P = c->gl[li - 1];
+  if (unpooled && c->fused_unpool && P.kind == G_POOL && L.din.p == P.pool_dsrc.p && P.H == 2 * L.H && P.W == 2 * L.W) {
+    a.ep.unpool_act = c->gl[P.skip_of].out;
+    a.ep.unpool_out = P.pool_dst;
+    a.ep.unpool_skip = P.pool_skipgrad;
+    *unpooled = dg_conv_igemm_unpool_supported(L.pb, a);
+    if (*unpooled) a.out = null_view();
+    else a.ep.unpool_act = a.ep.unpool_out = a.ep.unpool_skip = null_view();
+  }
   return conv_launch(c, L.pb, a, 3);
 }
 
 int g_backward(depgan_ctx* c, const float* x, const float* z, int n) {
+  bool unpooled_by_conv = false;
   for (int i = (int)c->gl.size() - 1; i >= 0; --i) {
     GLayer& L = c->gl[i];
     if (L.kind == G_HEAD) {
@@ -801,8 +813,10 @@
       DGCHECK(dg_sum(c->dpre, (size_t)P, L.db, c->scratch, c->scratchFloats, c->st));
       DGCHECK(dg_head_bwd(c->dpre, L.Wt, L.in.p, L.din.p, P, L.Cin, c->st));
     } else if (L.kind == G_CONV) {
-      DGCHECK(g_conv_bn_bwd(c, L, (size_t)i, x, L.dout, null_view(), n));
+      unpooled_by_conv = false;
+      DGCHECK(g_conv_bn_bwd(c, L, (size_t)i, x, L.dout, null_view(), n, &unpooled_by_conv));
     } else if (L.kind == G_FILM) {
+      unpooled_by_conv = false;
       TView du = make_view(c->du_tmp.p, L.H, L.W, L.Cout);
       {
         ProfScope ps(c, 2, 0.0, "film bwd");
@@ -810,8 +824,9 @@
                             c->dheads + L.col_mul, c->dheads + L.col_add, n, (long)L.H * L.W, L.Cout, c->scratch,
                             c->scratchFloats, c->st));
       }
-      DGCHECK(g_conv_bn_bwd(c, L, (size_t)i, x, du, L.dout, n));
+      DGCHECK(g_conv_bn_bwd(c, L, (size_t)i, x, du, L.dout, n, &unpooled_by_conv));
     } else if (L.kind == G_POOL) {
+      if (unpooled_by_conv) { unpooled_by_conv = false; continue; }
       ProfScope ps(c, 2, 0.0, "unpool+mask");
       DGCHECK(dg_unpool_mask(L.pool_dsrc, c->gl[L.skip_of].out, L.pool_skipgrad, L.pool_dst, n, L.H / 2, L.W / 2,
                              L.Cout, c->st));
@@ -904,14 +919,22 @@
     const DLayer& Pv = c->dl[l - 1];
     ConvArgs a = conv_args(view_offset(c->d_dz[l].view(), s0), null_view(), N, L.H, L.W, L.Cout, L.Cin);
     a.w = d_panel_b(c, D, l);
+    bool unpooled = false;
     if (Pv.pool) {
       a.out = view_offset(c->d_dpool[l - 1].view(), s0);
+      if (c->fused_unpool && Pv.H == 2 * L.H && Pv.W == 2 * L.W) {
+        a.ep.unpool_act = view_offset(c->d_act[l - 1].view(), s0);
+        a.ep.unpool_out = view_offset(c->d_dz[l - 1].view(), s0);
+        unpooled = dg_conv_igemm_unpool_supported(d_plan_b(c, l), a);
+        if (unpooled) a.out = null_view();
+        else a.ep.unpool_act = a.ep.unpool_out = null_view();
+      }
     } else {
       a.out = view_offset(c->d_dz[l - 1].view(), s0);
       a.ep.mask = view_offset(c->d_act[l - 1].view(), s0);
     }
     DGCHECK(conv_launch(c, d_plan_b(c, l), a, L.KS));
-    if (Pv.pool) {
+    if (Pv.pool && !unpooled) {
       ProfScope ps(c, 2, 0.0, "unpool+mask");
       DGCHECK(dg_unpool_mask(a.out, view_offset(c->d_act[l - 1].view(), s0), null_view(),
                              view_offset(c->d_dz[l - 1].view(), s0), N, Pv.H / 2, Pv.W / 2, Pv.Cout, c->st));
@@ -1242,6 +1265,8 @@
     c->bf16s_head_fused = !(hfs && atoi(hfs) == 0);
     const char* wn = getenv("DEPGAN_WINOGRAD");
     c->winograd = !(wn && atoi(wn) == 0);
+    const char* fu = getenv("DEPGAN_FUSED_UNPOOL");
+    c->fused_unpool = !(fu && atoi(fu) == 0);
   }
   if (c->cfg.nc_out == 0) c->cfg.nc_out = 1;
   if (c->cfg.nc_out < 1 || c->cfg.nc_out > DEPGAN_MAX_HEAD_CLASSES) {
diff --git a/dep_gan_im_amd/csrc/op_entries.hip b/dep_gan_im_amd/csrc/op_entries.hip
--- a/dep_gan_im_amd/csrc/op_entries.hip
+++ b/dep_gan_im_amd/csrc/op_entries.hip
@@ -67,6 +67,10 @@
   if (path == 9 && KS != 5) { dg_set_error("op_conv: path 9 is the weight-stationary 5x5 kernel, KS must be 5"); return DG_ERR_ARG; }
   if (path == 9 && !dg_conv_igemm_ws5_supported(pl, a, true)) { dg_set_error("op_conv: the weight-stationary 5x5 kernel does not cover this shape"); return DG_ERR_UNSUPPORTED; }
   if (path == 1 && !dg_plan_mfma(pl)) { dg_set_error("op_conv: MFMA path not available for this shape"); return DG_ERR_UNSUPPORTED; }
+  if (a.ep.unpool_out.p) {
+    if (path == 2 || !dg_plan_mfma(pl)) { dg_set_error("op_conv: no fused un-pool on the direct kernels"); return DG_ERR_UNSUPPORTED; }
+    DGCHECK(dg_conv_igemm_check(pl, a));
+  }
   if (path != 2 && dg_plan_mfma(pl)) {
     DevTmp wp(st);
     DGCHECK(wp.alloc(pl.packedFloats * sizeof(float)));
@@ -246,6 +250,22 @@
   return op_conv_run(a, w_hwio, Cin, Cout, KS, path, bwd ? 1 : 0, (hipStream_t)stream);
 }
 
+int depgan_op_conv2d_unpool(const float* in, long isB, long isY, long isX, const float* w_hwio, const float* act, long asB,
+                            long asY, long asX, float* out, long osB, long osY, long osX, const float* skip, long ssB,
+                            long ssY, long ssX, int B, int H, int W, int Cin, int Cout, int KS, int path, int bwd) {
+  if (op_view_bad_batched(in, isB, isY, isX) || op_view_bad_batched(act, asB, asY, asX) || op_view_bad_batched(out, osB, osY, osX) ||
+      (skip && op_view_bad_batched(skip, ssB, ssY, ssX)) || !w_hwio || B < 1 || H < 1 || W < 1 || Cin < 1 || Cout < 1 ||
+      (KS != 1 && KS != 3 && KS != 5)) {
+    dg_set_error("op_conv2d_unpool: null or non-positive argument");
+    return DG_ERR_ARG;
+  }
+  if (path < 1 || path > 10) { dg_set_error("op_conv2d_unpool: path must be 1 ... 10"); return DG_ERR_ARG; }
+  ConvArgs a = conv_args(op_view(in, isB, isY, isX), null_view(), B, H, W, bwd ? Cout : Cin, bwd ? Cin : Cout);
+  a.ep.unpool_act = op_view(act, asB, asY, asX);
+  a.ep.unpool_out = op_view(out, osB, osY, osX);
+  a.ep.unpool_skip = op_view_or_null(skip, ssB, ssY, ssX);
+  return op_conv_run(a, w_hwio, Cin, Cout, KS, path, bwd ? 1 : 0, (hipStream_t)nullptr);
+}
 
 int depgan_op_conv3x3_wino_gathered(const float* in, long isB, long isY, long isX, const long* run_off, int runs,
                                     const float* w_hwio, const float* bias, float* out, long osB, long osY, long osX,
diff --git a/dep_gan_im_amd/csrc/ops.hip b/dep_gan_im_amd/csrc/ops.hip
--- a/dep_gan_im_amd/csrc/ops.hip
+++ b/dep_gan_im_amd/csrc/ops.hip
@@ -25,15 +25,6 @@
   if (need <= have) return 1;
   dg_set_error("%s: scratch holds %zu floats, the launch needs %zu", who, have, need);
   return 0;
-}
-
-__device__ __forceinline__ int first_argmax4(float a0, float a1, float a2, float a3) {
-  int k = 0;
-  float m = a0;
-  if (a1 > m) { m = a1; k = 1; }
-  if (a2 > m) { m = a2; k = 2; }
-  if (a3 > m) { m = a3; k = 3; }
-  return k;
 }
 
 __global__ void maxpool_kernel(TView in, TView out, int B, int Ho, int Wo, int C4) {
diff --git a/include/depgan.h b/include/depgan.h
--- a/include/depgan.h
+++ b/include/depgan.h
@@ -278,6 +278,9 @@
                            long msY, long msX, float* pool, long qsB, long qsY, long qsX, const float* head_w,
                            const float* head_b, float* head_out, int head_tanh, int head_skip_out, int B, int H, int W,
                            int Cin, int Cout, int KS, int relu, int accumulate, int path, int bwd, void* hip_stream);
+int depgan_op_conv2d_unpool(const float* in, long isB, long isY, long isX, const float* w_hwio, const float* act, long asB,
+                            long asY, long asX, float* out, long osB, long osY, long osX, const float* skip, long ssB,
+                            long ssY, long ssX, int B, int H, int W, int Cin, int Cout, int KS, int path, int bwd);
 int depgan_op_conv3x3_wino_gathered(const float* in, long isB, long isY, long isX, const long* run_off, int runs,
                                     const float* w_hwio, const float* bias, float* out, long osB, long osY, long osX,
                                     int B, int H, int W, int Cin, int Cout, void* hip_stream);
```

New measurement: 718.5 slices/s, median of 6. No clear change (+0.8%).
